# CurryChen77/RIFT

Hardware: AMD Instinct MI355X
Metric: policy-update scenes/sec (256-scene RIFT update steps on a 4096-scene replay) (higher is better)
Workload: dtype bf16; 1 GPU; BASELINE configs[2]/[3]: full rift_pluto CBV policy, 4096-scene synthetic replay (64 agents x 21 steps, 20 polygons x 3 x 20 pts, R~U{1..6} x 120 ref pts, 12 modes), RIFT loss, pi_head trainable; per_gpu_batch=256, global_batch=256, replay_scenes_per_gpu=4096, parallelism=dp1, train_mode=dropout+droppath+state-dropout, BN batch stats

## Files before the change

### include/rift_hip.h

```cpp
#ifndef RIFT_HIP_H
#define RIFT_HIP_H

#include <stdint.h>

#ifdef __cplusplus
extern "C" {
#endif

typedef struct RiftCtx RiftCtx;

enum { RIFT_OK = 0, RIFT_ERR_ARG = -1, RIFT_ERR_HIP = -2, RIFT_ERR_STATE = -3, RIFT_ERR_NONFINITE = -4 };

enum {
  RIFT_F_TRAIN      = 1,
  RIFT_F_NEED_TRAJ  = 2,
  RIFT_F_FP32       = 4,
  RIFT_F_NO_DROP    = 8,
  RIFT_F_NO_BN_UPDATE = 16,
  RIFT_F_DEFER_HEAD = 32
};
#define RIFT_DEFER_SLOTS 4

enum { RIFT_LOSS_RIFT = 0, RIFT_LOSS_GRPO = 1, RIFT_LOSS_PPO = 2, RIFT_LOSS_REINFORCE = 3,
       RIFT_LOSS_SFT = 4  };
// ... 8 lines not shown

typedef struct RiftFeatureBatch {
  int32_t bs, A, Mp, R, S;
  int32_t T;
  const float*   agent_position;
  const float*   agent_heading;
  const float*   agent_velocity;
  const float*   agent_shape;
  const int8_t*  agent_category;
  const uint8_t* agent_valid_mask;
  const float*   map_point_position;
  const float*   map_point_vector;
  const float*   map_point_orientation;
  const float*   map_polygon_center;
  const int8_t*  map_polygon_type;
  const uint8_t* map_polygon_on_route;
  const int8_t*  map_polygon_tl_status;
  const uint8_t* map_polygon_has_speed_limit;
  const float*   map_polygon_speed_limit;
  const uint8_t* map_valid_mask;
  const float*   ref_position;
  const float*   ref_vector;
  const float*   ref_orientation;
  const uint8_t* ref_valid_mask;
  const float*   static_position;
  const float*   static_heading;
  const float*   static_shape;
  const int8_t*  static_category;
  const uint8_t* static_valid_mask;
  const float*   current_state;
  int32_t cs_ld;
} RiftFeatureBatch;

typedef struct RiftOutputs {
  float* probability;
  float* hidden;
  float* trajectory;
  float* prediction;
  float* ref_free_trajectory;
} RiftOutputs;

typedef struct RiftLossIn {
  const float*   old_group_logits;
  const float*   ref_group_logits;
  const double*  group_advantage;
  const uint8_t* group_valid_mask;
  const int64_t* action_mode;
  const float*   advantage;
  const float*   old_log_prob;
  const float*   returns;
  float clip_epsilon;
  float lambda_entropy;
} RiftLossIn;

typedef struct RiftLossOut {
  double* loss;
  double* stats;
  float*  flat_grad_sum;
  float*  grad_w1;  float* grad_b1;
  float*  grad_ln_w; float* grad_ln_b;
  float*  grad_w2;  float* grad_b2;
  int64_t* argmax_rm;
  double* exchange;
} RiftLossOut;

enum { RIFT_OPERANDS_BF16 = 0, RIFT_OPERANDS_FP16 = 1 };
// ... 128 lines not shown
  double  bbox_inflation_ratio;
  double  resolution;
} RiftEvalParams;
int rift_eval_params_default(RiftCtx* ctx, RiftEvalParams* out);

int rift_rollout_return_ex(RiftCtx* ctx, const float* delta_dis, const float* delta_angle, const float* speed,
                           const float* acc, const float* ang_vel, const float* ang_acc, const uint8_t* collision,
                           int collision_ld, const uint8_t* off_road, int off_road_ld, int G, int Ts, const RiftEvalParams* params,
                           double* returns, double* terms, void* stream);

int rift_group_advantage_tick_ex(RiftCtx* ctx, const float* trajectory, int Rb, int Tfull, const RiftTickCBV* cbvs, int K,
                                 float* turn_buf, int32_t* turn_ptr, int32_t* turn_len, float* speed_buf, int32_t* speed_ptr, int32_t* speed_len,
                                 const RiftEvalParams* params, double* advantage, double* returns, double* terms, void* stream);

typedef struct RiftControlCBV {
  int32_t batch_index;
  int32_t slot;
  double x, y, heading;
  double speed;
} RiftControlCBV;
int rift_control_tick(RiftCtx* ctx, const float* trajectory , const float* probability ,
                      const float* ref_free_trajectory , int Rb, int Tfull,
                      const RiftControlCBV* cbvs, int K, int topk, int sample_interval, double* pid_state ,
                      int n_slots, double* decision , void* stream);

typedef struct RiftReplayArena {
  int32_t n_scenes, A, Mp, Rcap, S, T, cs_ld;
  RiftFeatureBatch scenes;
  const int32_t* r_count;
  const float*   old_group_logits;
  const float*   ref_group_logits;
  const double*  group_advantage;
  const uint8_t* group_valid_mask;
} RiftReplayArena;

int rift_collate(RiftCtx* ctx, const RiftReplayArena* arena, const int32_t* scene_idx , int bs,
                 int R_out, const RiftFeatureBatch* out_batch , float* out_old_logits,
                 float* out_ref_logits, double* out_advantage, uint8_t* out_valid_mask, void* stream);

int rift_clip_grad_norm(RiftCtx* ctx, float* const* grads , const int64_t* numels ,
                        int n_tensors , float max_norm, float* total_norm, void* stream);

int rift_adamw_step(RiftCtx* ctx, int n_tensors , float* const* params, const float* const* grads, float* const* exp_avg,
                    float* const* exp_avg_sq, float* const* steps, const int64_t* numels , const double* lr ,
                    const double* weight_decay , double step_new, double beta1, double beta2, double eps, void* stream);

int rift_update_tail(RiftCtx* ctx, const RiftLossOut* out, int accumulate, float max_norm, float* total_norm, int n_tensors ,
                     float* const* params, const float* const* grads, float* const* exp_avg, float* const* exp_avg_sq, float* const* steps,
                     const double* lr , const double* weight_decay , double step_new, double beta1, double beta2, double eps,
                     void* stream);

typedef struct RiftCritic {
  const float *w0, *b0, *w1, *b1, *w2, *b2;
  const float *state_avg, *state_std, *value_avg, *value_std;
} RiftCritic;
#define RIFT_CRITIC_NPARAM_C 99331

int rift_critic_forward(RiftCtx* ctx, const RiftCritic* w, const float* state , int n, float* value , void* stream);

int rift_critic_loss_backward(RiftCtx* ctx, const RiftCritic* w, const float* state , const float* reward_sum ,
                              int n, double* stats , float* flat_grad_sum, void* stream);

int rift_critic_finalize(RiftCtx* ctx, const float* flat_grad_sum, const double* stats, float* g_w0, float* g_b0, float* g_w1,
                         float* g_b1, float* g_w2, float* g_b2, float* g_state_avg, float* g_state_std, float* g_value_avg,
                         float* g_value_std, void* stream);

int rift_critic_backward(RiftCtx* ctx, const RiftCritic* w, const float* state , const float* dvalue , int n,
// ... 7 lines not shown
```

### rift_amd/_ffi.py

```python
import ctypes as C
import threading
import os
from typing import Dict, Optional

import numpy as np
import torch

_HERE = os.path.dirname(os.path.abspath(__file__))
LIB_PATH = os.path.join(_HERE, "librift_hip.so")

F_TRAIN, F_NEED_TRAJ, F_FP32, F_NO_DROP, F_NO_BN_UPDATE, F_DEFER_HEAD = 1, 2, 4, 8, 16, 32
DEFER_SLOTS = 4
LOSS_KINDS = {"rift": 0, "grpo": 1, "ppo": 2, "reinforce": 3, "sft": 4}
PI_NPARAM = 16897

vp = C.c_void_p


class RiftTensorDesc(C.Structure):
    _fields_ = [("name", C.c_char_p), ("data", vp), ("numel", C.c_int64), ("ndim", C.c_int32),
                ("shape", C.c_int64 * 4)]


_FB_PTRS = [
    "agent_position", "agent_heading", "agent_velocity", "agent_shape", "agent_category", "agent_valid_mask",
    "map_point_position", "map_point_vector", "map_point_orientation", "map_polygon_center", "map_polygon_type",
    "map_polygon_on_route", "map_polygon_tl_status", "map_polygon_has_speed_limit", "map_polygon_speed_limit",
    "map_valid_mask", "ref_position", "ref_vector", "ref_orientation", "ref_valid_mask", "static_position",
    "static_heading", "static_shape", "static_category", "static_valid_mask", "current_state",
]


class RiftFeatureBatch(C.Structure):
    _fields_ = ([(n, C.c_int32) for n in ("bs", "A", "Mp", "R", "S", "T")] + [(n, vp) for n in _FB_PTRS]
                + [("cs_ld", C.c_int32)])


class RiftOutputs(C.Structure):
    _fields_ = [(n, vp) for n in ("probability", "hidden", "trajectory", "prediction", "ref_free_trajectory")]


class RiftLossIn(C.Structure):
    _fields_ = [(n, vp) for n in ("old_group_logits", "ref_group_logits", "group_advantage", "group_valid_mask",
                                  "action_mode", "advantage", "old_log_prob", "returns")] + \
               [("clip_epsilon", C.c_float), ("lambda_entropy", C.c_float)]


class RiftLossOut(C.Structure):
    _fields_ = [(n, vp) for n in ("loss", "stats", "flat_grad_sum", "grad_w1", "grad_b1", "grad_ln_w", "grad_ln_b",
                                  "grad_w2", "grad_b2", "argmax_rm", "exchange")]


class RiftCritic(C.Structure):
    _fields_ = [(n, vp) for n in ("w0", "b0", "w1", "b1", "w2", "b2", "state_avg", "state_std", "value_avg", "value_std")]


class RiftReplayArena(C.Structure):
    _fields_ = [(n, C.c_int32) for n in ("n_scenes", "A", "Mp", "Rcap", "S", "T", "cs_ld")] + \
               [("scenes", RiftFeatureBatch)] + \
               [(n, vp) for n in ("r_count", "old_group_logits", "ref_group_logits", "group_advantage",
                                  "group_valid_mask")]


EXCHANGE_FN = C.CFUNCTYPE(C.c_int, C.c_void_p, C.c_int64, C.c_int64, C.c_void_p)


class RiftDp(C.Structure):
    _fields_ = [("scene_offset", C.c_int32), ("global_bs", C.c_int32), ("xchg", vp), ("xchg_len", C.c_int64),
                ("exchange", EXCHANGE_FN), ("user", vp)]


class RiftRolloutIO(C.Structure):
    _fields_ = [("trajectories", vp), ("G", C.c_int32), ("Tfull", C.c_int32), ("G_per_group", C.c_int32), ("center_state", vp),
                ("turn_buf", vp), ("turn_ptr", vp), ("turn_len", vp), ("speed_buf", vp), ("speed_ptr", vp), ("speed_len", vp),
                ("center", vp), ("angle", vp), ("speed", vp), ("acc", vp), ("ang_vel", vp), ("ang_acc", vp), ("vertices", vp),
                ("closest_index", vp), ("aim_idx", vp)]


class RiftTickCBV(C.Structure):
    _fields_ = [("batch_index", C.c_int32), ("R", C.c_int32), ("Pmax", C.c_int32), ("n_actors", C.c_int32), ("center_state", vp),
                ("ref_pos", vp), ("ref_angle", vp), ("ref_len", vp), ("actors", vp), ("off_road_mask", vp), ("H", C.c_int32), ("W", C.c_int32),
                ("pose", C.c_double * 3)]


class RiftControlCBV(C.Structure):
    _fields_ = [("batch_index", C.c_int32), ("slot", C.c_int32), ("x", C.c_double), ("y", C.c_double), ("heading", C.c_double),
                ("speed", C.c_double)]


class RiftEvalParams(C.Structure):
    _fields_ = [("reward_model", C.c_int32), ("near_lane_change", C.c_int32), ("gamma", C.c_double)] + \
               [(n, C.c_double) for n in ("alpha_collision", "alpha_boundary", "alpha_comfort", "alpha_l_align", "alpha_vel_align", "alpha_l_center",
                                          "alpha_center_bias", "alpha_velocity", "alpha_timestep", "bbox_inflation_ratio", "resolution")]


REWARD_MODELS = {"dense": 0, "sparse": 1}


def eval_params(reward_model=None, gamma: float = 0.98, bbox_inflation_ratio: float = 1.1, resolution: float = 0.5,
                near_lane_change: bool = True) -> RiftEvalParams:
    from rift_amd.gym_carla.reward.reward_model import DenseRewardModel
    p = RiftEvalParams()
    weights = DenseRewardModel().get_params()
    kind = "dense"
    if reward_model is not None:
        kind = reward_model.kind
        unknown = sorted(set(reward_model.get_params()) - set(weights))
        if kind not in REWARD_MODELS or unknown:
            raise ValueError(f"reward model {kind!r} with parameter(s) {unknown}: known models {sorted(REWARD_MODELS)}, known parameters {sorted(weights)}")
        weights.update(reward_model.get_params())
    p.reward_model, p.near_lane_change, p.gamma = REWARD_MODELS[kind], 1 if near_lane_change else 0, float(gamma)
    for k, v in weights.items():
        setattr(p, k, float(v))
    p.bbox_inflation_ratio, p.resolution = float(bbox_inflation_ratio), float(resolution)
    return p


CONTROL_STATE = 44
OPERANDS = {"bf16": 0, "fp16": 1}
EXPORTS = [
    "rift_ctx_create", "rift_ctx_create_ex", "rift_ctx_operand_format", "rift_ctx_destroy", "rift_last_error", "rift_model_load", "rift_forward", "rift_forward_head", "rift_forward_head_back", "rift_loss_backward",
    "rift_loss_finalize", "rift_loss_finalize_clip", "rift_set_param_event", "rift_tap", "rift_op_linear", "rift_gae", "rift_discounted_return",
    "rift_normalize_advantage", "rift_group_advantage", "rift_rollout_return", "rift_collate",
    "rift_prof_enable", "rift_prof_report", "rift_op_linear_bench", "rift_ref_line_info", "rift_rollout",
    "rift_critic_forward", "rift_critic_loss_backward", "rift_critic_finalize", "rift_clip_grad_norm", "rift_adamw_step", "rift_update_tail", "rift_collision_matrix", "rift_off_road_matrix", "rift_other_vehicle_rollout", "rift_sft_teacher_mode",
    "rift_check_finite", "rift_set_dp", "rift_set_prepare_stream", "rift_set_side_stream",
    "rift_comm_unique_id", "rift_comm_init", "rift_comm_all_reduce", "rift_comm_destroy", "rift_group_advantage_tick",
    "rift_control_tick", "rift_head_backward", "rift_critic_backward",
    "rift_eval_params_default", "rift_rollout_return_ex", "rift_group_advantage_tick_ex",
]
CRITIC_NPARAM = 99331
PI_KEYS = ("mlp.0.weight", "mlp.0.bias", "mlp.1.weight", "mlp.1.bias", "mlp.3.weight", "mlp.3.bias")
PI_SIZES = (128 * 128, 128, 128, 128, 128, 1)
CRITIC_SIZES = (256 * 128, 256, 256 * 256, 256, 256, 1, 128, 128, 1, 1)
CRITIC_KEYS = ("net.0.weight", "net.0.bias", "net.2.weight", "net.2.bias", "net.4.weight", "net.4.bias",
               "state_avg", "state_std", "value_avg", "value_std")

_libs = {}


def load_library(variant: str = "") -> C.CDLL:
    if variant in _libs:
        return _libs[variant]
    path = LIB_PATH if not variant else LIB_PATH.replace("librift_hip.so", f"librift_hip_{variant}.so")
    if not variant and os.environ.get("RIFT_LIB"):
        path = os.environ["RIFT_LIB"]
    if not os.path.exists(path):
        raise RuntimeError(
            f"{path} is missing: build it with `python -c 'import __graft_entry__ as g; g.build()'` "
            "(hipcc --offload-arch=gfx950). rift_amd has no CPU fallback.")
    lib = C.CDLL(path)
    for name in EXPORTS:
        if not hasattr(lib, name):
            raise RuntimeError(f"librift_hip.so does not export {name}")
    lib.rift_ctx_create.argtypes = [C.c_int, C.POINTER(vp)]
    lib.rift_ctx_create_ex.argtypes = [C.c_int, C.c_int, C.POINTER(vp)]
# ... 17 lines not shown
    lib.rift_set_side_stream.argtypes = [vp, vp]
    lib.rift_comm_unique_id.argtypes = [vp, vp]
    lib.rift_comm_init.argtypes = [vp, vp, C.c_int, C.c_int]
    lib.rift_comm_all_reduce.argtypes = [vp, vp, C.c_int64, vp]
    lib.rift_group_advantage_tick.argtypes = [vp, vp, C.c_int, C.c_int, C.POINTER(RiftTickCBV), C.c_int, vp, vp, vp, vp, vp, vp, C.c_double, vp, vp]
    lib.rift_group_advantage_tick_ex.argtypes = [vp, vp, C.c_int, C.c_int, C.POINTER(RiftTickCBV), C.c_int, vp, vp, vp, vp, vp, vp, C.POINTER(RiftEvalParams),
                                                 vp, vp, vp, vp]
    lib.rift_eval_params_default.argtypes = [vp, C.POINTER(RiftEvalParams)]
    lib.rift_rollout_return_ex.argtypes = [vp, vp, vp, vp, vp, vp, vp, vp, C.c_int, vp, C.c_int, C.c_int, C.c_int, C.POINTER(RiftEvalParams), vp, vp, vp]
    lib.rift_control_tick.argtypes = [vp, vp, vp, vp, C.c_int, C.c_int, C.POINTER(RiftControlCBV), C.c_int, C.c_int, C.c_int, vp, C.c_int, vp, vp]
    lib.rift_comm_destroy.argtypes = [vp]
    lib.rift_loss_finalize_clip.argtypes = [vp, C.POINTER(RiftLossOut), C.c_int, C.c_float, vp, vp]
    lib.rift_tap.argtypes = [vp, C.c_char_p, vp, C.POINTER(C.c_int64), vp]
    lib.rift_critic_forward.argtypes = [vp, C.POINTER(RiftCritic), vp, C.c_int, vp, vp]
    lib.rift_critic_loss_backward.argtypes = [vp, C.POINTER(RiftCritic), vp, vp, C.c_int, vp, vp, vp]
    lib.rift_critic_finalize.argtypes = [vp] * 14
    lib.rift_clip_grad_norm.argtypes = [vp, C.POINTER(vp), C.POINTER(C.c_int64), C.c_int, C.c_float, vp, vp]
    lib.rift_update_tail.argtypes = [vp, C.POINTER(RiftLossOut), C.c_int, C.c_float, vp, C.c_int, C.POINTER(vp), C.POINTER(vp), C.POINTER(vp), C.POINTER(vp),
                                     C.POINTER(vp), C.POINTER(C.c_double), C.POINTER(C.c_double), C.c_double, C.c_double, C.c_double, C.c_double, vp]
    lib.rift_adamw_step.argtypes = [vp, C.c_int, C.POINTER(vp), C.POINTER(vp), C.POINTER(vp), C.POINTER(vp), C.POINTER(vp),
                                    C.POINTER(C.c_int64), C.POINTER(C.c_double), C.POINTER(C.c_double), C.c_double, C.c_double,
                                    C.c_double, C.c_double, vp]
    lib.rift_sft_teacher_mode.argtypes = [vp, vp, vp, C.c_int, C.c_int, C.c_int, C.c_int, C.c_int, vp, vp]
    lib.rift_other_vehicle_rollout.argtypes = [vp, vp, vp, vp, vp, vp, C.c_int, C.c_int, C.c_int, C.c_double, vp, vp]
    lib.rift_collision_matrix.argtypes = [vp, vp, C.c_int, C.c_int, vp, C.c_int, C.c_int, vp, vp]
    lib.rift_off_road_matrix.argtypes = [vp, vp, C.c_int, vp, C.c_int, C.c_int] + [C.c_double] * 7 + [vp, vp]
    lib.rift_op_linear.argtypes = [vp, vp, C.c_int, C.c_int, vp, vp, C.c_int, vp, vp, C.c_int, C.c_int, vp, vp]
    lib.rift_gae.argtypes = [vp, vp, vp, vp, vp, vp, C.c_float, C.c_float, C.c_int, vp, vp]
    lib.rift_discounted_return.argtypes = [vp, vp, vp, C.c_double, C.c_int, vp, vp]
    lib.rift_normalize_advantage.argtypes = [vp, vp, C.c_int, vp]
    lib.rift_group_advantage.argtypes = [vp, vp, C.c_int, C.c_int, vp, vp]
    lib.rift_rollout_return.argtypes = [vp, vp, vp, vp, vp, vp, vp, vp, C.c_int, vp, C.c_int, C.c_int, C.c_int,
                                        C.c_double, vp, vp]
    lib.rift_collate.argtypes = [vp, C.POINTER(RiftReplayArena), vp, C.c_int, C.c_int, C.POINTER(RiftFeatureBatch),
                                 vp, vp, vp, vp, vp]
    lib.rift_op_linear_bench.argtypes = [vp, vp, C.c_int, C.c_int, vp, vp, C.c_int, vp, vp, C.c_int, vp, vp, C.c_int,
                                         C.POINTER(C.c_float), vp]
    lib.rift_ref_line_info.argtypes = [vp, vp, C.c_int, C.c_int, C.c_int, C.c_int, vp, vp, vp, C.c_int, vp, vp, vp, vp]
    lib.rift_rollout.argtypes = [vp, C.POINTER(RiftRolloutIO), vp]
    lib.rift_prof_enable.argtypes = [vp, C.c_int]
    lib.rift_prof_report.argtypes = [vp, C.c_char_p, C.c_int]
    for name in EXPORTS:
        if name not in ("rift_ctx_destroy", "rift_last_error"):
            getattr(lib, name).restype = C.c_int
    _libs[variant] = lib
    return lib


def _ptr(t: Optional[torch.Tensor]):
    return None if t is None else C.c_void_p(t.data_ptr())


class _KnownStreams(threading.local):
    def __init__(self):
        self.stack = []


_KNOWN_STREAM = _KnownStreams()


def _stream():
    st = _KNOWN_STREAM.stack
    if st:
        return st[-1]
    return C.c_void_p(torch.cuda.current_stream().cuda_stream)

# ... 36 lines not shown

    fb = RiftFeatureBatch()
    pos = put(ag["position"], f32)
    bs, A, T = pos.shape[:3]
    Mp = mp["point_position"].shape[1]
    R = rl["position"].shape[1]
    S = so["position"].shape[1] if so is not None else 0
    fb.bs, fb.A, fb.Mp, fb.R, fb.S, fb.T = bs, A, Mp, R, S, T
    t = {
        "agent_position": pos, "agent_heading": put(ag["heading"], f32), "agent_velocity": put(ag["velocity"], f32),
        "agent_shape": put(ag["shape"], f32), "agent_category": put(ag["category"], i8),
        "agent_valid_mask": put(ag["valid_mask"], u8),
        "map_point_position": put(mp["point_position"], f32), "map_point_vector": put(mp["point_vector"], f32),
        "map_point_orientation": put(mp["point_orientation"], f32), "map_polygon_center": put(mp["polygon_center"], f32),
        "map_polygon_type": put(mp["polygon_type"], i8), "map_polygon_on_route": put(mp["polygon_on_route"], u8),
        "map_polygon_tl_status": put(mp["polygon_tl_status"], i8),
        "map_polygon_has_speed_limit": put(mp["polygon_has_speed_limit"], u8),
        "map_polygon_speed_limit": put(mp["polygon_speed_limit"], f32), "map_valid_mask": put(mp["valid_mask"], u8),
        "ref_position": put(rl["position"], f32), "ref_vector": put(rl["vector"], f32),
        "ref_orientation": put(rl["orientation"], f32), "ref_valid_mask": put(rl["valid_mask"], u8),
        "current_state": put(data["current_state"], f32),
    }
    if S > 0:
        t.update({"static_position": put(so["position"], f32), "static_heading": put(so["heading"], f32),
                  "static_shape": put(so["shape"], f32), "static_category": put(so["category"], i8),
                  "static_valid_mask": put(so["valid_mask"], u8)})
    for name in _FB_PTRS:
        setattr(fb, name, t[name].data_ptr() if name in t else None)
    fb.cs_ld = t["current_state"].shape[1]
    return fb, keep


class Engine:

    def __init__(self, device=None, operands: str = "bf16", variant: str = ""):
        if operands not in OPERANDS:
            raise ValueError(f"operands must be one of {sorted(OPERANDS)}, got {operands!r}")
        if not torch.cuda.is_available():
            raise RuntimeError("rift_amd.Engine needs a HIP device (torch.cuda.is_available() is False); "
                               "there is no CPU fallback")
        self.lib = load_library(variant)
        self.device = torch.device(device if device is not None else f"cuda:{torch.cuda.current_device()}")
        self.ctx = vp()
        self.operands = operands
        rc = self.lib.rift_ctx_create_ex(self.device.index or 0, OPERANDS[operands], C.byref(self.ctx))
        if rc != 0:
            raise RuntimeError(f"rift_ctx_create_ex failed ({rc})")
        self._params = None
        self._names = None
        self._keep = []
        self._stage_host = self._stage_dev = None
        self._stage_off = 0
        self._ctl_state = None
        self.generation = 0

    _STAGE_BYTES = 8 << 20
    _NP_OF = {torch.float32: np.float32, torch.float64: np.float64, torch.int32: np.int32, torch.int64: np.int64, torch.uint8: np.uint8,
              torch.int8: np.int8, torch.bool: np.bool_}

    def stage_tree(self, data):
        leaves = []

        def walk(d):
            if isinstance(d, dict):
                return {k: walk(v) for k, v in d.items()}
            if torch.is_tensor(d):
                leaves.append(d)
                return len(leaves) - 1
            raise NotImplementedError(type(d))

        shape = walk(data)
        out = self.stage_many(leaves)

        def build(d):
            return {k: build(v) for k, v in d.items()} if isinstance(d, dict) else out[d]
        return build(shape)

    def stage_many(self, tensors):
        if self._stage_host is None:
            self._stage_host = torch.empty(self._STAGE_BYTES, dtype=torch.uint8).pin_memory()
            self._stage_dev = torch.empty(self._STAGE_BYTES, dtype=torch.uint8, device=self.device)
        plan, total = [], 0
        for t in tensors:
            if t.is_cuda or t.dtype not in self._NP_OF or t.numel() == 0 or t.numel() * t.element_size() > self._STAGE_BYTES // 4:
                plan.append(None)
                continue
            a = np.ascontiguousarray(t.detach().numpy())
# ... 77 lines not shown
            descs[i].data = v.data_ptr()
            descs[i].numel = v.numel()
            descs[i].ndim = min(v.dim(), 4)
            shp = list(v.shape)[-4:] if v.dim() > 4 else list(v.shape)
            for d in range(4):
                descs[i].shape[d] = shp[d] if d < len(shp) else 1
        self._params, self._names = params, names
        self._check(self.lib.rift_model_load(self.ctx, descs, len(params), _stream()), "rift_model_load")
        return params

    def forward(self, data: Dict, train=False, need_traj=False, fp32=False, no_drop=False, bn_update=True,
                seed: int = 0) -> Dict[str, torch.Tensor]:
        fb, keep = feature_batch(data, self.device)
        bs, A, R = fb.bs, fb.A, fb.R
        o = RiftOutputs()
        out = {"probability": torch.empty(bs, R, 12, device=self.device),
               "hidden": torch.empty(bs, 128, device=self.device)}
        if need_traj:
            out["trajectory"] = torch.empty(bs, R, 12, 80, 6, device=self.device)
            out["prediction"] = torch.empty(bs, max(A - 1, 0), 80, 6, device=self.device)
            out["ref_free_trajectory"] = torch.empty(bs, 80, 4, device=self.device)
        for k, v in out.items():
            setattr(o, k, v.data_ptr())
        flags = (F_TRAIN if train else 0) | (F_NEED_TRAJ if need_traj else 0) | (F_FP32 if fp32 else 0) | \
                (F_NO_DROP if no_drop else 0) | (0 if bn_update else F_NO_BN_UPDATE)
        self._check(self.lib.rift_forward(self.ctx, C.byref(fb), C.byref(o), flags, C.c_uint32(seed & 0xFFFFFFFF),
                                          _stream()), "rift_forward")
        self.generation += 1
        self._keep = keep + list(out.values())
        self._bs = bs
        return out

    def forward_raw(self, fb: RiftFeatureBatch, out: RiftOutputs, flags: int, seed: int):
        rc = self.lib.rift_forward(self.ctx, C.byref(fb), C.byref(out), flags, C.c_uint32(seed & 0xFFFFFFFF), _stream())
        self.generation += 1
        if rc != 0:
            self._check(rc, "rift_forward")
        self._bs = fb.bs

    def set_side_stream(self, stream: Optional["torch.cuda.Stream"]):
        self._side_stream = stream
        rc = self.lib.rift_set_side_stream(self.ctx, C.c_void_p(stream.cuda_stream if stream is not None else 0))
        if rc != 0:
            self._check(rc, "rift_set_side_stream")

    def set_prepare_stream(self, stream: Optional["torch.cuda.Stream"]):
        self._prep_stream = stream
        rc = self.lib.rift_set_prepare_stream(self.ctx, C.c_void_p(stream.cuda_stream if stream is not None else 0))
        if rc != 0:
            self._check(rc, "rift_set_prepare_stream")

    def forward_head(self, back: int = 0):
        rc = self.lib.rift_forward_head_back(self.ctx, back, _stream())
        self.generation += 1
        if rc != 0:
            self._check(rc, "rift_forward_head")

    def loss_backward_raw(self, kind: int, li: RiftLossIn, lo: RiftLossOut):
        rc = self.lib.rift_loss_backward(self.ctx, kind, C.byref(li), C.byref(lo), _stream())
        if rc != 0:
            self._check(rc, "rift_loss_backward")

    def loss_finalize_raw(self, lo: RiftLossOut, accumulate: int = 0):
        rc = self.lib.rift_loss_finalize(self.ctx, C.byref(lo), accumulate, _stream())
        if rc != 0:
            self._check(rc, "rift_loss_finalize")

# ... 538 lines not shown
```

### rift_amd/csrc/abi.cpp

```cpp
#include <stdlib.h>
#include <string.h>

#include "abi_table.h"

extern "C" const RiftVTable rift_vtable_bf16;
#if defined(RIFT_ABI_BF16_ONLY)
#define RIFT_VT_FP16 (static_cast<const RiftVTable*>(nullptr))
#else
extern "C" const RiftVTable rift_vtable_fp16;
#define RIFT_VT_FP16 (&rift_vtable_fp16)
#endif

static inline const RiftVTable& vt(const RiftCtx* ctx) {
  return (*reinterpret_cast<const int*>(ctx) == RIFT_OPERANDS_FP16 && RIFT_VT_FP16) ? *RIFT_VT_FP16 : rift_vtable_bf16;
}

extern "C" {

int rift_ctx_create_ex(int device, int operand_format, RiftCtx** ctx) {
  if (operand_format == RIFT_OPERANDS_BF16) return rift_vtable_bf16.rift_ctx_create(device, ctx);
  if (operand_format == RIFT_OPERANDS_FP16 && RIFT_VT_FP16) return RIFT_VT_FP16->rift_ctx_create(device, ctx);
  return RIFT_ERR_ARG;
}

// ... 168 lines not shown
  return vt(ctx).rift_ref_line_info(ctx, trajectories, G, Tfull, Ts, M, ref_pos, ref_angle, ref_len, Pmax, delta_dis, delta_angle, closest_idx, stream);
}

int rift_rollout(RiftCtx* ctx, const RiftRolloutIO* io, void* stream) {
  if (!ctx) return RIFT_ERR_ARG;
  return vt(ctx).rift_rollout(ctx, io, stream);
}

int rift_group_advantage_tick(RiftCtx* ctx, const float* trajectory, int Rb, int Tfull, const RiftTickCBV* cbvs, int K, float* turn_buf, int32_t* turn_ptr, int32_t* turn_len, float* speed_buf, int32_t* speed_ptr, int32_t* speed_len, double gamma, double* advantage, void* stream) {
  if (!ctx) return RIFT_ERR_ARG;
  return vt(ctx).rift_group_advantage_tick(ctx, trajectory, Rb, Tfull, cbvs, K, turn_buf, turn_ptr, turn_len, speed_buf, speed_ptr, speed_len, gamma, advantage, stream);
}

int rift_eval_params_default(RiftCtx* ctx, RiftEvalParams* out) {
  if (!ctx) return RIFT_ERR_ARG;
  return vt(ctx).rift_eval_params_default(ctx, out);
}

int rift_rollout_return_ex(RiftCtx* ctx, const float* delta_dis, const float* delta_angle, const float* speed, const float* acc, const float* ang_vel, const float* ang_acc, const uint8_t* collision, int collision_ld, const uint8_t* off_road, int off_road_ld, int G, int Ts, const RiftEvalParams* params, double* returns, double* terms, void* stream) {
  if (!ctx) return RIFT_ERR_ARG;
  return vt(ctx).rift_rollout_return_ex(ctx, delta_dis, delta_angle, speed, acc, ang_vel, ang_acc, collision, collision_ld, off_road, off_road_ld, G, Ts, params, returns, terms, stream);
}

int rift_group_advantage_tick_ex(RiftCtx* ctx, const float* trajectory, int Rb, int Tfull, const RiftTickCBV* cbvs, int K, float* turn_buf, int32_t* turn_ptr, int32_t* turn_len, float* speed_buf, int32_t* speed_ptr, int32_t* speed_len, const RiftEvalParams* params, double* advantage, double* returns, double* terms, void* stream) {
  if (!ctx) return RIFT_ERR_ARG;
  return vt(ctx).rift_group_advantage_tick_ex(ctx, trajectory, Rb, Tfull, cbvs, K, turn_buf, turn_ptr, turn_len, speed_buf, speed_ptr, speed_len, params, advantage, returns, terms, stream);
}

int rift_control_tick(RiftCtx* ctx, const float* trajectory, const float* probability, const float* ref_free_trajectory, int Rb, int Tfull, const RiftControlCBV* cbvs, int K, int topk, int sample_interval, double* pid_state, int n_slots, double* decision, void* stream) {
  if (!ctx) return RIFT_ERR_ARG;
  return vt(ctx).rift_control_tick(ctx, trajectory, probability, ref_free_trajectory, Rb, Tfull, cbvs, K, topk, sample_interval, pid_state, n_slots, decision, stream);
}

int rift_collate(RiftCtx* ctx, const RiftReplayArena* arena, const int32_t* scene_idx, int bs, int R_out, const RiftFeatureBatch* out_batch, float* out_old_logits, float* out_ref_logits, double* out_advantage, uint8_t* out_valid_mask, void* stream) {
  if (!ctx) return RIFT_ERR_ARG;
  return vt(ctx).rift_collate(ctx, arena, scene_idx, bs, R_out, out_batch, out_old_logits, out_ref_logits, out_advantage, out_valid_mask, stream);
}

int rift_clip_grad_norm(RiftCtx* ctx, float* const* grads, const int64_t* numels, int n_tensors, float max_norm, float* total_norm, void* stream) {
  if (!ctx) return RIFT_ERR_ARG;
  return vt(ctx).rift_clip_grad_norm(ctx, grads, numels, n_tensors, max_norm, total_norm, stream);
}

int rift_adamw_step(RiftCtx* ctx, int n_tensors, float* const* params, const float* const* grads, float* const* exp_avg, float* const* exp_avg_sq, float* const* steps, const int64_t* numels, const double* lr, const double* weight_decay, double step_new, double beta1, double beta2, double eps, void* stream) {
  if (!ctx) return RIFT_ERR_ARG;
  return vt(ctx).rift_adamw_step(ctx, n_tensors, params, grads, exp_avg, exp_avg_sq, steps, numels, lr, weight_decay, step_new, beta1, beta2, eps, stream);
}

int rift_update_tail(RiftCtx* ctx, const RiftLossOut* out, int accumulate, float max_norm, float* total_norm, int n_tensors, float* const* params, const float* const* grads, float* const* exp_avg, float* const* exp_avg_sq, float* const* steps, const double* lr, const double* weight_decay, double step_new, double beta1, double beta2, double eps, void* stream) {
  if (!ctx) return RIFT_ERR_ARG;
  return vt(ctx).rift_update_tail(ctx, out, accumulate, max_norm, total_norm, n_tensors, params, grads, exp_avg, exp_avg_sq, steps, lr, weight_decay, step_new, beta1, beta2, eps, stream);
}

int rift_critic_forward(RiftCtx* ctx, const RiftCritic* w, const float* state, int n, float* value, void* stream) {
  if (!ctx) return RIFT_ERR_ARG;
  return vt(ctx).rift_critic_forward(ctx, w, state, n, value, stream);
}

int rift_critic_loss_backward(RiftCtx* ctx, const RiftCritic* w, const float* state, const float* reward_sum, int n, double* stats, float* flat_grad_sum, void* stream) {
  if (!ctx) return RIFT_ERR_ARG;
  return vt(ctx).rift_critic_loss_backward(ctx, w, state, reward_sum, n, stats, flat_grad_sum, stream);
}

int rift_critic_finalize(RiftCtx* ctx, const float* flat_grad_sum, const double* stats, float* g_w0, float* g_b0, float* g_w1, float* g_b1, float* g_w2, float* g_b2, float* g_state_avg, float* g_state_std, float* g_value_avg, float* g_value_std, void* stream) {
  if (!ctx) return RIFT_ERR_ARG;
  return vt(ctx).rift_critic_finalize(ctx, flat_grad_sum, stats, g_w0, g_b0, g_w1, g_b1, g_w2, g_b2, g_state_avg, g_state_std, g_value_avg, g_value_std, stream);
// ... 9 lines not shown
```

### rift_amd/csrc/abi_list.h

```cpp
RIFT_FN(rift_ctx_create)
RIFT_FN(rift_ctx_destroy)
RIFT_FN(rift_last_error)
RIFT_FN(rift_model_load)
RIFT_FN(rift_forward)
RIFT_FN(rift_forward_head)
RIFT_FN(rift_forward_head_back)
RIFT_FN(rift_set_dp)
RIFT_FN(rift_comm_unique_id)
RIFT_FN(rift_comm_init)
RIFT_FN(rift_comm_all_reduce)
RIFT_FN(rift_comm_destroy)
RIFT_FN(rift_set_prepare_stream)
RIFT_FN(rift_set_side_stream)
RIFT_FN(rift_check_finite)
RIFT_FN(rift_sft_teacher_mode)
RIFT_FN(rift_set_param_event)
RIFT_FN(rift_loss_backward)
RIFT_FN(rift_loss_finalize)
RIFT_FN(rift_loss_finalize_clip)
RIFT_FN(rift_head_backward)
RIFT_FN(rift_prof_enable)
RIFT_FN(rift_prof_report)
RIFT_FN(rift_tap)
RIFT_FN(rift_op_linear)
RIFT_FN(rift_op_linear_bench)
RIFT_FN(rift_gae)
RIFT_FN(rift_discounted_return)
RIFT_FN(rift_normalize_advantage)
RIFT_FN(rift_group_advantage)
RIFT_FN(rift_other_vehicle_rollout)
RIFT_FN(rift_collision_matrix)
RIFT_FN(rift_off_road_matrix)
RIFT_FN(rift_rollout_return)
RIFT_FN(rift_ref_line_info)
RIFT_FN(rift_rollout)
RIFT_FN(rift_group_advantage_tick)
RIFT_FN(rift_eval_params_default)
RIFT_FN(rift_rollout_return_ex)
RIFT_FN(rift_group_advantage_tick_ex)
RIFT_FN(rift_control_tick)
RIFT_FN(rift_collate)
RIFT_FN(rift_clip_grad_norm)
RIFT_FN(rift_adamw_step)
RIFT_FN(rift_update_tail)
RIFT_FN(rift_critic_forward)
RIFT_FN(rift_critic_loss_backward)
RIFT_FN(rift_critic_finalize)
RIFT_FN(rift_critic_backward)
```

### rift_amd/csrc/adv.h

```cpp
#pragma once
#include "common.h"

namespace RIFT_NS {

struct GaeCoef {
  const double* rewards; const float* undones; const float* values; const float* next_values; const float* unterminated;
  float gamma, lambda_;
  __device__ __forceinline__ void get(int t, double& a, double& b) const {
    const float t2 = (unterminated[t] * gamma) * next_values[t];
    b = rewards[t] + (double)t2 - (double)values[t];
    a = (double)((undones[t] * gamma) * lambda_);
  }
};
struct ReturnCoef {
  const double* rewards; const float* dones; double gamma;
  __device__ __forceinline__ void get(int t, double& a, double& b) const {
    b = rewards[t];
    a = (dones[t] == 1.0f) ? 0.0 : gamma;
  }
};

#define RIFT_SCAN_THREADS 1024
template <class Coef, class OutT>
__global__ __launch_bounds__(RIFT_SCAN_THREADS) void affine_scan_reverse_kernel(Coef c, int n, OutT* __restrict__ out) {
// ... 218 lines not shown
    if (!(ox0 > ex1 || ox1 < ex0 || oy0 > ey1 || oy1 < ey0)) { hit = 1; break; }
  }
  out[i] = hit;
}
__global__ __launch_bounds__(256) void collision_matrix_kernel(const float* __restrict__ cv, int G, int Tc, const double* __restrict__ ov, int N, int Ts, uint8_t* __restrict__ out) {
  collision_matrix_body(cv, G, Tc, ov, N, Ts, out);
}

__device__ __forceinline__ void off_road_body(const float* __restrict__ pts , int n, const uint8_t* __restrict__ mask, int H,
                                                       int W, double ox, double oy, double c, double s, double res_x, double res_y,
                                                       double off_x, double off_y, uint8_t* __restrict__ out) {
  const int i = blockIdx.x * 256 + threadIdx.x;
  if (i >= n) return;
  const double dx = (double)pts[2 * i] - ox, dy = (double)pts[2 * i + 1] - oy;
  const double lx = __dadd_rn(__dmul_rn(dx, c), __dmul_rn(dy, s));
  const double ly = __dadd_rn(__dmul_rn(dx, -s), __dmul_rn(dy, c));
  const double px = rint(lx / res_x + off_x), py = rint(ly / res_y + off_y);
  uint8_t off = 0;
  if (px >= 0.0 && px < (double)W && py >= 0.0 && py < (double)H) off = mask[(size_t)(int)py * W + (int)px] == 1;
  out[i] = off;
}
__global__ __launch_bounds__(256) void off_road_kernel(const float* __restrict__ pts, int n, const uint8_t* __restrict__ mask, int H, int W, double ox, double oy, double c, double s,
                                                       double res_x, double res_y, double off_x, double off_y, uint8_t* __restrict__ out) {
  off_road_body(pts, n, mask, H, W, ox, oy, c, s, res_x, res_y, off_x, off_y, out);
}

#define RIFT_COLLATE_MAXT 40
struct CollateP {
  int nt;
  const unsigned char* src[RIFT_COLLATE_MAXT];
  unsigned char* dst[RIFT_COLLATE_MAXT];
  int src_bytes[RIFT_COLLATE_MAXT];
  int dst_bytes[RIFT_COLLATE_MAXT];
};

__global__ void collate_kernel(CollateP p, const int32_t* __restrict__ scene_idx) {
  const int k = blockIdx.y, b = blockIdx.x;
  const unsigned char* s = p.src[k] + (size_t)scene_idx[b] * p.src_bytes[k];
  unsigned char* d = p.dst[k] + (size_t)b * p.dst_bytes[k];
  const int n = p.dst_bytes[k];
  if ((((uintptr_t)s | (uintptr_t)d | (uintptr_t)n) & 15) == 0) {
    const uint4* s4 = reinterpret_cast<const uint4*>(s);
    uint4* d4 = reinterpret_cast<uint4*>(d);
    for (int i = threadIdx.x; i < (n >> 4); i += blockDim.x) d4[i] = s4[i];
  } else if ((((uintptr_t)s | (uintptr_t)d | (uintptr_t)n) & 3) == 0) {
    const uint32_t* s4 = reinterpret_cast<const uint32_t*>(s);
    uint32_t* d4 = reinterpret_cast<uint32_t*>(d);
    for (int i = threadIdx.x; i < (n >> 2); i += blockDim.x) d4[i] = s4[i];
  } else {
    for (int i = threadIdx.x; i < n; i += blockDim.x) d[i] = s[i];
  }
}

}
```

### rift_amd/csrc/engine.hip

```cpp
#include <hip/hip_runtime.h>
#include <math.h>
#include <stdio.h>
#include <stdlib.h>
#include <string.h>

#include <algorithm>
#include <set>
#include <cmath>
#include <string>
#include <unordered_map>
#include <dlfcn.h>
#include <vector>

#include "../../include/rift_hip.h"
#include "adv.h"
#include "eval_params.h"
#include "gemm.h"
#include "kernels.h"
#include "loss.h"
#include "nat_l0w.h"
#include "nat_l1w.h"
#include "enc_fused.h"
#include "dec_w.h"
#include "dec_kv.h"
// ... 11 lines not shown
#include "pi_fused.h"
#include "rollout.h"
#include "tick_multi.h"
#include "control.h"

#define ENC_NW 8

using namespace RIFT_NS;

namespace {

struct Param { void* data; int64_t numel; int ndim; int64_t shape[4]; };

struct PW {
  void* bf = nullptr; float* f32 = nullptr; const float* bias = nullptr;
  int N = 0, K = 0, Kp = 0, Npad = 0;
  void* hid = nullptr;
};

struct Tap { float* p; int64_t numel; };

}

struct RiftCtx {
  int opfmt = 0;
  int device = 0;
  std::string err;
  std::unordered_map<std::string, Param> params;
  std::unordered_map<std::string, PW> pw;
  std::vector<void*> owned;
  struct WConst { float* p = nullptr; bool ready = false; };
  std::unordered_map<std::string, WConst> wconst;
  char* arena = nullptr; size_t arena_cap = 0, arena_off = 0;
  long long dry_key[11] = {}; size_t dry_need = 0;
  char* arenas[RIFT_DEFER_SLOTS] = {}; size_t arena_caps[RIFT_DEFER_SLOTS] = {}; int parity = 0;
  struct Head {
    bool valid = false, fp32 = false, need_traj = false;
    float *Q = nullptr, *x0p = nullptr, *QF = nullptr, *Hpi = nullptr, *prob = nullptr, *traj = nullptr, *o3[3] = {nullptr, nullptr, nullptr}, *oT[3] = {nullptr, nullptr, nullptr};
    uint8_t* r_kpm = nullptr; int bs = 0, R = 0, nQ = 0;
    bool dec_pending = false; DecWP dec;
  } head[RIFT_DEFER_SLOTS];
  int dec_defer_max = -1; bool dec_split = true;
  bool ro8 = true;
  float* ro_raw = nullptr; size_t ro_cap = 0;
  char* tick_scratch = nullptr; size_t tick_cap = 0;
  bool dry = false;
  hipStream_t stream = nullptr;
  std::unordered_map<std::string, Tap> taps;
  float* last_qfinal = nullptr; float* last_hpi = nullptr; float* last_prob = nullptr;
  uint8_t* last_rkpm = nullptr; int last_bs = 0, last_R = 0;
  double* l_S = nullptr; double* l_cnt = nullptr; float* l_dz = nullptr; float* l_partial = nullptr;
  size_t l_cap_bs = 0, l_cap_rows = 0, l_cap_wg = 0;
  double* l_sink = nullptr;
  float* ego_w = nullptr; float* ego_b = nullptr;
  bool nat_fused = true; int gemm_dbg = 0;
  unsigned short* l0w_img = nullptr; float* l0w_par = nullptr;
  unsigned short* encw_img = nullptr; float* encw_par = nullptr;
  unsigned short* l2w_img = nullptr; float* l2w_par = nullptr;
  unsigned short* l1w_img = nullptr; float* l1w_par = nullptr;
  unsigned short* enc_wqkv[4] = {nullptr, nullptr, nullptr, nullptr};
  float* enc_bqkv[4] = {nullptr, nullptr, nullptr, nullptr};
  int* enc_idx = nullptr; bool enc_fused = true;
  int poison_lds = -1;
  struct { std::string delay_label; long long delay_ticks = 0; int pe_ts = -1, pew_dbg = 0, pew_ts = 0, nat_ts = 0, enc_ts = 0, dec_ts = 0, dec_dbg = 0, poison_arena = -1; } dg;
  hipEvent_t param_event = nullptr;
  bool dec_fused = true;
  bool two_streams = true; bool nat_compact = true; bool pe_live = true; bool pe_pack = true;
  hipStream_t prep_stream = nullptr; bool prep_set = false; hipEvent_t ev_prep = nullptr; int side_gate = 0;
  hipEvent_t ev_join2 = nullptr; bool nat_aside = true;
  hipStream_t side = nullptr; bool side_owned = false; hipEvent_t ev_fork = nullptr, ev_join = nullptr;
  bool fo_w = true; unsigned short* fow_img[3] = {nullptr, nullptr, nullptr}; float* fow_par[3] = {nullptr, nullptr, nullptr};
  bool pe_w = true; unsigned short* pew_img[2] = {nullptr, nullptr};
  unsigned short* decw_img = nullptr; float* decw_par = nullptr;
  double* clip_part = nullptr;
  struct Dp { bool on = false; int off = 0, gbs = 0; double* xchg = nullptr; long long len = 0; RiftExchangeFn fn = nullptr; void* user = nullptr; } dp;
  int* nonfinite = nullptr;
  unsigned long long* rk_pub[RIFT_DEFER_SLOTS] = {}; int rk_cap[RIFT_DEFER_SLOTS] = {}; unsigned int rk_epoch[RIFT_DEFER_SLOTS] = {};
  bool rank_fault = false;
  bool no_skip = false;
  bool enc112 = true;
  bool rank_in_prep = true;
  void* comm = nullptr; int comm_rank = 0, comm_world = 1;
  float* cr_buf = nullptr; size_t cr_cap = 0; double* cr_part = nullptr;
  bool pe_fused = true; bool fo_fused = true; int nat_grid = 256; bool fpn_fused = true; bool ego_fused = true; bool heads_fused = true; bool pi_fused = true;
  bool loaded = false;
  bool prof_on = false; double prof_flops = 0.0; bool prof_shapes = false;
  std::set<std::string> prof_names;
  std::vector<hipEvent_t> prof_pool; size_t prof_used = 0;
  struct Rec { const char* label; hipEvent_t e0, e1; double flops; };
  std::vector<Rec> prof_recs;
};

static void prof_events(RiftCtx* c, hipEvent_t* e0, hipEvent_t* e1) {
  while (c->prof_pool.size() < c->prof_used + 2) { hipEvent_t e; (void)hipEventCreate(&e); c->prof_pool.push_back(e); }
  *e0 = c->prof_pool[c->prof_used++]; *e1 = c->prof_pool[c->prof_used++];
}
static void prof_push(RiftCtx* c, const char* label, hipEvent_t e0, hipEvent_t e1, double flops) {
  c->prof_recs.push_back(RiftCtx::Rec{label, e0, e1, flops});
}

// ... 280 lines not shown
#undef SETATTR
#define SETATTR_N(K, N) HIPCHK(c, hipFuncSetAttribute(reinterpret_cast<const void*>(&K), hipFuncAttributeMaxDynamicSharedMemorySize, (int)(N)))
  SETATTR_N(lds_poison_kernel, 160 * 1024);
  SETATTR_N(dec_kv_frag_kernel, DEC_KV_LDS);
  SETATTR_N(pe_mid_kernel, PE_MID_LDS);
  SETATTR_N(pe_out_kernel, PE_OUT_LDS);
  SETATTR_N(fourier_fused_kernel, FO_LDS);
  SETATTR_N(fpn_tail_kernel, FPN_LDS);
  SETATTR_N(heads3_fused_kernel, HD_LDS);
  SETATTR_N(pi_forward_kernel, PI_LDS);
  HIPCHK(c, (hipError_t)l0w_set_attributes());
  HIPCHK(c, (hipError_t)l1w_set_attributes());
#undef SETATTR_N
  return RIFT_OK;
}

const std::string HE = "agent_encoder.history_encoder", PD = "planning_decoder";

struct Fwd {
  RiftCtx* c; bool train, drop, fp32, need_traj, bn_update; uint32_t seed; uint32_t stream_id = 1;
  uint32_t next_stream() { return stream_id++; }
  bool dp = false, kpm_pending = false; int kb = 0; uint8_t* g_rkpm = nullptr;
  uint8_t* r_tiles = nullptr;
  const RiftFeatureBatch* B = nullptr; const RiftOutputs* out = nullptr; int flags = 0;
  StreamPlan plan; hipStream_t on[3] = {nullptr, nullptr, nullptr};
  int bs = 0, A = 0, Mp = 0, R = 0, S = 0, T = 0, N = 0, M = 12, nA = 0, nP = 0, nL = 0, nQ = 0, nT = 0;
  DropStats ds = {};
  float *F9 = nullptr, *F10 = nullptr, *F6 = nullptr, *pos = nullptr, *r_pos = nullptr;
  uint8_t *valid_agent = nullptr, *kpm = nullptr, *r_kpm = nullptr;
  bool nat_compact = false; int *nat_aidx = nullptr, *nat_cnt = nullptr;
  const uint8_t* q_kpm = nullptr; int q_bs = 0, q_off = 0;
  float *nat_out = nullptr, *x_ego = nullptr, *poly = nullptr, *r_emb = nullptr, *speed_emb = nullptr, *PEtok = nullptr, *Q = nullptr, *X = nullptr;
  bool pe_pair = false, fo3 = false, rpe_done = false;
  float* ENC = nullptr;
  unsigned short* enc_KT = nullptr;
  uint8_t* kpm_c = nullptr;
  float* enc_x0p = nullptr;
  bool enc_wide = false;
  bool dec_deferred = false; DecWP dec_later;
};

struct RcclApi {
  struct UniqueId { char internal[128]; };
  int (*GetUniqueId)(UniqueId*) = nullptr;
  int (*CommInitRank)(void**, int, UniqueId, int) = nullptr;
  int (*AllReduce)(const void*, void*, size_t, int, int, void*, hipStream_t) = nullptr;
  int (*CommDestroy)(void*) = nullptr;
  const char* (*GetErrorString)(int) = nullptr;
  bool ok = false;
};
static RcclApi& rccl_api(std::string* why) {
  static RcclApi api;
  static bool tried = false;
  static std::string err;
  if (!tried) {
    tried = true;
    void* h = nullptr;
    const char* names[] = {getenv("RIFT_RCCL_LIB"), "librccl.so", "librccl.so.1"};
    for (const char* n : names) if (n && !h) h = dlopen(n, RTLD_NOW | RTLD_NOLOAD | RTLD_GLOBAL);
    for (const char* n : names) if (n && !h) h = dlopen(n, RTLD_NOW | RTLD_GLOBAL);
    if (!h) h = dlopen("/opt/rocm/lib/librccl.so", RTLD_NOW | RTLD_GLOBAL);
    if (!h) err = std::string("librccl.so not found (set RIFT_RCCL_LIB): ") + (dlerror() ? dlerror() : "");
    else {
      api.GetUniqueId = (decltype(api.GetUniqueId))dlsym(h, "ncclGetUniqueId");
      api.CommInitRank = (decltype(api.CommInitRank))dlsym(h, "ncclCommInitRank");
      api.AllReduce = (decltype(api.AllReduce))dlsym(h, "ncclAllReduce");
// ... 87 lines not shown

void batchnorm_affine(Fwd& f, const float* X, int rows, int C, const uint8_t* valid, const std::string& name,
                      float** scale, float** shift) {
  RiftCtx* c = f.c;
  *scale = A_alloc<float>(c, C); *shift = A_alloc<float>(c, C);
  const int rows_per_blk = 128;
  const int nblk = cdiv(rows, rows_per_blk);
  double* part = A_alloc<double>(c, (size_t)nblk * 2 * C);
  int* cnt = A_alloc<int>(c, nblk);
  if (f.train) launch(c, "bn_partial_kernel", bn_partial_kernel, dim3(nblk), dim3(C), 0, X, C, rows, C, valid, part, cnt, rows_per_blk);
  const Param* nb = find(c, name + ".num_batches_tracked");
  const bool dpx = f.dp && f.train;
  double* sums = dpx ? c->dp.xchg + f.kb : nullptr;
  for (int mode = dpx ? 1 : 0; mode <= (dpx ? 2 : 0); ++mode) {
    launch(c, "bn_finalize_kernel", bn_finalize_kernel, dim3(cdiv(C, 4)), dim3(256), 0, (const double*)part, (const int*)cnt, nblk, C,
           fptr(c, name + ".weight"), fptr(c, name + ".bias"), (float*)fptr(c, name + ".running_mean"),
           (float*)fptr(c, name + ".running_var"), nb ? (long long*)nb->data : (long long*)nullptr, f.train ? 1 : 0,
           f.bn_update ? 1 : 0, 1e-5f, *scale, *shift, sums, mode);
    if (mode == 1) dp_exchange(f, 2 * C + 1);
  }
}

static void pe_fill(Fwd& f, PeP& q, const float* F, int Cin, int groups, int n, const uint8_t* valid, const std::string& p) {
  RiftCtx* c = f.c;
  memset(&q, 0, sizeof(q));
  const int rows = groups * n;
  q.F = F; q.Cin = Cin; q.valid = valid; q.rows = rows; q.ntiles = cdiv(rows, 120);
  const PW &w1 = c->pw[p + ".first_mlp.0"], &w2 = c->pw[p + ".first_mlp.3"], &w3a = c->pw[p + ".second_mlp.0.feat"],
           &w3b = c->pw[p + ".second_mlp.0.pool"], &w4 = c->pw[p + ".second_mlp.3"];
  q.w1 = (const unsigned short*)w1.bf; q.w2 = (const unsigned short*)w2.bf; q.w3a = (const unsigned short*)w3a.bf;
  q.w3b = (const unsigned short*)w3b.bf; q.w4 = (const unsigned short*)w4.bf;
  q.b1 = w1.bias; q.b2 = w2.bias; q.b3 = w3a.bias; q.b4 = w4.bias;
  q.s1 = A_alloc<float>(c, 128); q.t1 = A_alloc<float>(c, 128); q.s2 = A_alloc<float>(c, 256); q.t2 = A_alloc<float>(c, 256);
  q.part1 = A_alloc<float>(c, (size_t)2 * 128 * q.ntiles);
  q.part2 = A_alloc<float>(c, (size_t)2 * 256 * q.ntiles);
  q.cnt = A_alloc<int>(c, q.ntiles);
  q.Fmid = A_alloc<unsigned short>(c, (size_t)rows * 256);
  q.gp = A_alloc<float>(c, (size_t)groups * 256);
  q.out = A_alloc<float>(c, (size_t)groups * 128);
  q.do_stats = f.train ? 1 : 0;
  { if (c->dg.pe_ts == n) { q.ts = A_alloc<long long>(c, 64); q.ts_tile = 0; tap(c, "pe_ts", (float*)q.ts, 128); } }
}

static BnFinP bn_fin(RiftCtx* c, const PeP& q, const std::string& name, int C, const float* part, const float* sc, const float* sh,
                     double* sums = nullptr, int sums_mode = 0) {
  BnFinP b; memset(&b, 0, sizeof(b));
  b.sums = sums; b.sums_mode = sums_mode;
  const Param* nb = find(c, name + ".num_batches_tracked");
  b.part = part; b.cnt = q.cnt; b.nblk = q.ntiles; b.C = C; b.gamma = fptr(c, name + ".weight"); b.beta = fptr(c, name + ".bias");
  b.running_mean = (float*)fptr(c, name + ".running_mean"); b.running_var = (float*)fptr(c, name + ".running_var");
  b.num_batches = nb ? (long long*)nb->data : nullptr; b.scale = (float*)sc; b.shift = (float*)sh;
  return b;
}

void points_encoder_pair(Fwd& f, const float* Fm, int gm, const uint8_t* vm, const std::string& pm, const float* Fr, int gr,
                         const uint8_t* vr, const std::string& pr, float** out_m, float** out_r) {
  RiftCtx* c = f.c;
  PeP2 q;
  pe_fill(f, q.a, Fm, 10, gm, 20, vm, pm);
  pe_fill(f, q.b, Fr, 6, gr, 120, vr, pr);
  const int nt = q.a.ntiles + q.b.ntiles;
  const double rows = (double)q.a.rows + q.b.rows, groups = (double)gm + gr;
  const bool stats_p = f.train && c->pe_w;
  const bool packb = c->pe_w && c->pe_pack && gr > 0 && f.r_tiles != nullptr;
  int* pk_tab = nullptr; int* pk_hdr = nullptr;
  PePackP pk; memset(&pk, 0, sizeof(pk));
  if (packb) {
    const int maxr = cdiv(q.b.rows, PEW_ROUND_ROWS);
    pk_tab = A_alloc<int>(c, (size_t)std::max(maxr, 1) * PEW_TAB_INTS); pk_hdr = A_alloc<int>(c, 4);
    pk.tiles = f.r_tiles; pk.nlines = gr; pk.tab = pk_tab; pk.hdr = pk_hdr; pk.max_rounds = maxr;
    tap(c, "pe_pack_hdr", (float*)pk_hdr, 4); tap(c, "pe_pack_tab", (float*)pk_tab, (int64_t)std::max(maxr, 1) * PEW_TAB_INTS);
    if (!stats_p) { c->prof_flops = 0.0; launch(c, "pe_pack_lines_kernel", pe_pack_lines_kernel, dim3(1), dim3(256), (size_t)gr * 2 * sizeof(int), pk); }
  }
  if (stats_p) {
    int g = std::min(nt, 4 * c->nat_grid);
    int ga = (int)(((long long)g * q.a.ntiles + nt / 2) / nt);
    if (q.a.ntiles > 0 && ga < 1) ga = 1;
    if (q.b.ntiles > 0 && ga > g - 1) ga = g - 1;
    if (q.b.ntiles == 0) ga = g;
    ga = std::min(ga, q.a.ntiles);
    q.a.nwg1 = ga; q.b.nwg1 = std::min(g - ga, q.b.ntiles);
    PeP* sd[2] = {&q.a, &q.b};
    for (int i = 0; i < 2; ++i) { sd[i]->part1w = A_alloc<float>(c, (size_t)2 * 128 * std::max(sd[i]->nwg1, 1)); sd[i]->cnt1w = A_alloc<int>(c, std::max(sd[i]->nwg1, 1)); }
    c->prof_flops = 2.0 * 128.0 * (q.a.rows * 10.0 + q.b.rows * 6.0);
    launch(c, "pe_stats1_kernel", pe_stats1p_kernel, dim3(q.a.nwg1 + q.b.nwg1 + (packb ? 1 : 0)), dim3(256), packb ? (size_t)gr * 2 * sizeof(int) : 0, q, pk);
  } else if (f.train) {
    c->prof_flops = 2.0 * 128.0 * (q.a.rows * 10.0 + q.b.rows * 6.0);
    launch(c, "pe_stats1_kernel", pe_stats1_kernel, dim3(nt), dim3(256), 0, q);
  }
  const bool dpx = f.dp && f.train;
  double* xs = dpx ? c->dp.xchg + f.kb : nullptr;
  PeLiveP lv; memset(&lv, 0, sizeof(lv));
  const bool live = stats_p && c->pe_live;
  int pew_grid = c->nat_grid, pew_ga = 0;
  if (c->pe_w) pew_split(cdiv(q.a.rows, PEW_ROUND_ROWS), cdiv(q.b.rows, PEW_ROUND_ROWS), &pew_grid, &pew_ga);
  if (live || packb) {
    const PeP* sd[2] = {&q.a, &q.b};
    for (int i = 0; i < 2; ++i) {
      lv.cnt[i] = live ? sd[i]->cnt : nullptr; lv.nt[i] = sd[i]->ntiles; lv.nr[i] = cdiv(sd[i]->rows, PEW_ROUND_ROWS);
      lv.live[i] = A_alloc<int>(c, std::max(lv.nr[i], 1));
    }
    lv.grid = pew_grid; lv.hdr = A_alloc<int>(c, 4);
    lv.packed_b = pk_hdr;
    tap(c, "pe_live_hdr", (float*)lv.hdr, 4);
  }
  const bool lvblock = live || packb;
  for (int mode = dpx ? 1 : 0; mode <= (dpx ? 2 : 0); ++mode) {
    BnFinP f1a = bn_fin(c, q.a, pm + ".first_mlp.1", 128, q.a.part1, q.a.s1, q.a.t1, xs, mode);
    BnFinP f1b = bn_fin(c, q.b, pr + ".first_mlp.1", 128, q.b.part1, q.b.s1, q.b.t1, xs ? xs + 257 : nullptr, mode);
    if (stats_p) { f1a.part = q.a.part1w; f1a.cnt = q.a.cnt1w; f1a.nblk = q.a.nwg1; f1b.part = q.b.part1w; f1b.cnt = q.b.cnt1w; f1b.nblk = q.b.nwg1; }
    const bool with_lv = lvblock && mode == (dpx ? 2 : 0);
    PeLiveP none; memset(&none, 0, sizeof(none));
    launch(c, "bn_finalize_t_kernel", bn_finalize_t_kernel, dim3(256 + (with_lv ? 1 : 0)), dim3(256), 0, f1a, f1b, f.train ? 1 : 0, f.bn_update ? 1 : 0, 1e-5f,
           with_lv ? lv : none);
    if (mode == 1) dp_exchange(f, 2 * 257);
  }
  c->prof_flops = 2.0 * rows * (128.0 * 8 + 128.0 * 256 + (f.train ? 256.0 * 256 : 0.0)) + 2.0 * groups * 256.0 * 256;
  BnFinP fa, fb;
  if (c->pe_w) {
    PeWP w; memset(&w, 0, sizeof(w));
    const PeP* src[2] = {&q.a, &q.b};
    PeWSide* dst[2] = {&w.a, &w.b};
    const int npts[2] = {20, 120};
    const int grid = pew_grid, ga = pew_ga;
    const int nwg[2] = {lvblock ? grid : ga, lvblock ? grid : grid - ga};
    for (int i = 0; i < 2; ++i) {
      const PeP& o = *src[i]; PeWSide& d = *dst[i];
      d.F = o.F; d.Cin = o.Cin; d.valid = o.valid; d.rows = o.rows; d.npts = npts[i]; d.nrounds = cdiv(o.rows, PEW_ROUND_ROWS);
      d.img = c->pew_img[i]; d.w3b = o.w3b; d.b1 = o.b1; d.b2 = o.b2; d.b3 = o.b3; d.s1 = o.s1; d.t1 = o.t1;
      d.live = (live && !(i == 1 && packb)) ? lv.live[i] : nullptr;
      if (i == 1) { d.ptab = pk_tab; d.phdr = pk_hdr; }
      d.part2 = A_alloc<float>(c, (size_t)2 * 256 * std::max(nwg[i], 1)); d.cnt2 = A_alloc<int>(c, std::max(nwg[i], 1));
      d.Fmid = o.Fmid;
    }
    w.ga = ga; w.hdr = lvblock ? lv.hdr : nullptr;
    w.do_stats = f.train ? 1 : 0;
    w.dbg = c->dg.pew_dbg;
    { if (c->dg.pew_ts) { w.ts = A_alloc<long long>(c, 128); tap(c, "pew_ts", (float*)w.ts, 256); } }
    launch_call(c, "pe_w_kernel", [&] { pew_launch(w, grid, c->stream); });
    fa = bn_fin(c, q.a, pm + ".second_mlp.1", 256, w.a.part2, q.a.s2, q.a.t2, xs, 0); fa.cnt = w.a.cnt2; fa.nblk = nwg[0]; fa.nblk_dev = lvblock ? lv.hdr + 2 : nullptr;
    fb = bn_fin(c, q.b, pr + ".second_mlp.1", 256, w.b.part2, q.b.s2, q.b.t2, xs ? xs + 513 : nullptr, 0); fb.cnt = w.b.cnt2; fb.nblk = nwg[1]; fb.nblk_dev = lvblock ? lv.hdr + 3 : nullptr;
  } else {
    launch(c, "pe_mid_kernel", pe_mid_kernel, dim3(nt), dim3(512), (size_t)PE_MID_LDS, q);
    fa = bn_fin(c, q.a, pm + ".second_mlp.1", 256, q.a.part2, q.a.s2, q.a.t2, xs, 0);
    fb = bn_fin(c, q.b, pr + ".second_mlp.1", 256, q.b.part2, q.b.s2, q.b.t2, xs ? xs + 513 : nullptr, 0);
  }
  for (int mode = dpx ? 1 : 0; mode <= (dpx ? 2 : 0); ++mode) {
    fa.sums_mode = mode; fb.sums_mode = mode;
    PeLiveP none; memset(&none, 0, sizeof(none));
// ... 391 lines not shown
         (const float*)c->ego_w, (const float*)c->ego_b, fptr(c, EG + ".pos_embed"), bs, E);
  float* EKV = A_alloc<float>(c, (size_t)bs * 6 * 256);
  gemm(c, mk(E, 128, bs * 6, c->pw[EG + ".attn.kv"], EKV, 256), c->pw[EG + ".attn.kv"], f.fp32);
  uint8_t* edrop = nullptr;
  if (f.drop) {
    edrop = A_alloc<uint8_t>(c, (size_t)bs * 6);
    launch(c, "ego_dropmask_kernel", ego_dropmask_kernel, dim3(cdiv(bs * 6, 256)), dim3(256), 0, bs, 0.75f, f.seed, f.next_stream(), edrop);
  }
  float* EAO = A_alloc<float>(c, (size_t)bs * 128);
  {
    MhaP p; memset(&p, 0, sizeof(p));
    p.Q = eq; p.ldq = 128; p.K = EKV; p.V = EKV + 128; p.ldkv = 256; p.O = EAO; p.ldo = 128;
    p.nb_outer = bs; p.nb_inner = 1; p.H = 4; p.Lq = 1; p.Lk = 6;
    p.q_outer = 0; p.q_inner = 0; p.q_stride = 0; p.kv_outer = 6; p.kv_inner = 0; p.kv_stride = 1;
    p.o_outer = 1; p.o_inner = 0; p.o_stride = 0; p.mask = edrop; p.mask_quirk = 0; p.mask_mod = 1;
    run_mha(c, p, f.fp32);
  }
  gemm(c, mk(EAO, 128, bs, c->pw[EG + ".attn.out_proj"], f.x_ego, 128), c->pw[EG + ".attn.out_proj"], f.fp32);
  }
  tap(c, "x_ego", f.x_ego, (int64_t)bs * 128);
}

int build_q0(Fwd& f) {
  RiftCtx* c = f.c;
  const int M = f.M, nL = f.nL, nQ = f.nQ;
  bool fill;
  float* Mb = wconst_get(c, "Mb", (size_t)M * 128, f.fp32, &fill);
  if (fill) gemm(c, mk(fptr(c, PD + ".m_emb"), 128, M, c->pw[PD + ".q_proj.m"], Mb, 128), c->pw[PD + ".q_proj.m"], f.fp32);
  f.Q = A_alloc<float>(c, (size_t)nQ * 128);
  if (!f.fp32 && c->pi_fused) {
    Q0P q; memset(&q, 0, sizeof(q));
    q.r_emb = f.r_emb; q.nL = nL; q.M = M; q.wr = (const unsigned short*)c->pw[PD + ".q_proj.r"].bf; q.br = c->pw[PD + ".q_proj.r"].bias;
    q.Mb = Mb; q.Q = f.Q;
    c->prof_flops = 2.0 * nL * 128.0 * 128;
    launch(c, "q0_fused_kernel", q0_fused_kernel, dim3(cdiv(nL, 16)), dim3(256), 0, q);
  } else {
    float* Ra = A_alloc<float>(c, (size_t)nL * 128);
    gemm(c, mk(f.r_emb, 128, nL, c->pw[PD + ".q_proj.r"], Ra, 128), c->pw[PD + ".q_proj.r"], f.fp32);
    launch(c, "build_q0_kernel", build_q0_kernel, dim3(cdiv((long long)nQ * 128, 256)), dim3(256), 0, (const float*)Ra, (const float*)Mb, nL, M, f.Q);
  }
  return RIFT_OK;
}

int map_and_embeddings(Fwd& f) {
  RiftCtx* c = f.c;
  const RiftFeatureBatch* B = f.B;
  const int S = f.S, nP = f.nP, nL = f.nL, nT = f.nT;
  f.pe_pair = !f.fp32 && c->pe_fused;
  if (f.pe_pair) points_encoder_pair(f, f.F10, nP, B->map_valid_mask, "map_encoder.polygon_encoder", f.F6, nL, B->ref_valid_mask, PD + ".r_encoder", &f.poly, &f.r_emb);
  else f.poly = points_encoder(f, f.F10, 10, nP, 20, B->map_valid_mask, "map_encoder.polygon_encoder");
  tap(c, "poly_pe", f.poly, (int64_t)nP * 128);
  f.fo3 = f.pe_pair && !f.fp32 && c->fo_fused && S == 0;
  if (f.fo3) {
    tap(c, "r_pe", f.r_emb, (int64_t)nL * 128);
    FourierP3 q3; memset(&q3, 0, sizeof(q3));
    q3.e[0] = fourier_desc(f, f.pos, 3, nT, 3, "pos_emb", 2, nullptr);
    q3.e[1] = fourier_desc(f, B->map_polygon_speed_limit, 1, nP, 1, "map_encoder.speed_limit_emb", -1, nullptr);
    q3.e[2] = fourier_desc(f, f.r_pos, 3, nL, 3, PD + ".r_pos_emb", -1, f.r_emb);
    q3.nblk[0] = cdiv(nT, FO_ROWS); q3.nblk[1] = cdiv(nP, FO_ROWS); q3.nblk[2] = cdiv(nL, FO_ROWS); q3.count = 3;
    c->prof_flops = 2.0 * 128.0 * ((nT + nL) * (3 * 257.0 + 128.0) + nP * (257.0 + 128.0));
    if (c->fo_w) {
      FoWP w; memset(&w, 0, sizeof(w));
      w.count = 3;
      for (int i = 0; i < 3; ++i) {
        const FourierP& o = q3.e[i]; FoWSide& d = w.e[i];
        d.in = o.in; d.in_ld = o.in_ld; d.rows = o.rows; d.D = o.D; d.wrap_dim = o.wrap_dim; d.img = c->fow_img[i]; d.par = c->fow_par[i];
        d.Y = o.Y; d.accumulate = o.accumulate; d.rep = o.D == 1 ? 2 : 1; d.nwg = cdiv(cdiv(o.rows, 16), 8 * d.rep);
      }
      launch_call(c, "fo_w_kernel", [&] { fow_launch(w, c->stream); });
    } else
    launch(c, "fourier_fused_kernel", fourier_fused_kernel, dim3(q3.nblk[0] + q3.nblk[1] + q3.nblk[2]), dim3(256), (size_t)FO_LDS, q3);
    f.PEtok = q3.e[0].Y; f.speed_emb = q3.e[1].Y; f.rpe_done = true;
  } else {
    f.speed_emb = fourier(f, B->map_polygon_speed_limit, 1, nP, 1, "map_encoder.speed_limit_emb", -1);
  }
  if (f.plan.forked && f.rpe_done) TRY(build_q0(f));
  return RIFT_OK;
}

void assemble_tokens(Fwd& f) {
  RiftCtx* c = f.c;
  const RiftFeatureBatch* B = f.B;
  const int bs = f.bs, A = f.A, Mp = f.Mp, S = f.S, N = f.N, nA = f.nA, nP = f.nP, nT = f.nT;
  f.X = A_alloc<float>(c, (size_t)nT * 128);
  TokenP q; memset(&q, 0, sizeof(q));
  q.nat = f.nat_out; q.x_ego = f.x_ego; q.valid_agent = (const uint8_t*)f.valid_agent; q.category = B->agent_category; q.a_type_emb = fptr(c, "agent_encoder.type_emb.weight");
  q.pooled = f.poly; q.ptype = B->map_polygon_type; q.on_route = B->map_polygon_on_route; q.tl = B->map_polygon_tl_status; q.has_sl = B->map_polygon_has_speed_limit;
  q.speed_emb = f.speed_emb; q.p_type_emb = fptr(c, "map_encoder.type_emb.weight"); q.route_emb = fptr(c, "map_encoder.on_route_emb.weight");
  q.tl_emb = fptr(c, "map_encoder.traffic_light_emb.weight"); q.unk_emb = fptr(c, "map_encoder.unknown_speed_emb.weight");
  q.bs = bs; q.A = A; q.Mp = Mp; q.N = N; q.X = f.X; q.pe = f.PEtok;
  q.nblk_a = cdiv((long long)nA * 32, 256);
  launch(c, "token_kernel", token_kernel, dim3(q.nblk_a + cdiv((long long)nP * 32, 256)), dim3(256), 0, q);
  if (S > 0) {
    float* semb = fourier(f, B->static_shape, 2, bs * S, 2, "static_objects_encoder.obj_encoder", -1);
    launch(c, "static_token_kernel", static_token_kernel, dim3(cdiv((long long)bs * S * 128, 256)), dim3(256), 0, (const float*)semb, B->static_category,
           B->static_valid_mask, fptr(c, "static_objects_encoder.type_emb.weight"), bs, A, Mp, S, N, f.X);
  }
  if (!f.fo3) fourier(f, f.pos, 3, nT, 3, "pos_emb", 2, f.X);
  tap(c, "x_tokens", f.X, (int64_t)nT * 128);
}

void scene_encoder(Fwd& f) {
  RiftCtx* c = f.c;
  const int bs = f.bs, R = f.R, N = f.N, nT = f.nT;
  static const float edpr[4] = {0.f, 0.2f / 3.f, 0.4f / 3.f, 0.2f};
  f.ENC = A_alloc<float>(c, (size_t)nT * 128);
  f.enc_wide = N > 96 && N <= 112 && c->enc112 && c->dec_fused && R <= 8 && ENC_NW == 8;
  if (c->enc_fused && !f.fp32 && (N <= 96 || f.enc_wide)) {
    EncFusedP ep; memset(&ep, 0, sizeof(ep));
    ep.X = f.X; ep.Y = f.ENC; ep.kpm = f.kpm; ep.bs = bs; ep.N = N; ep.seed = f.seed; ep.stream = f.next_stream(); f.stream_id += 8;
    for (int i = 0; i < 4; ++i) {
      const std::string p = "encoder_blocks." + std::to_string(i);
      EncBlockW& w = ep.blk[i];
      w.ln1_g = fptr(c, p + ".norm1.weight"); w.ln1_b = fptr(c, p + ".norm1.bias");
      w.ln2_g = fptr(c, p + ".norm2.weight"); w.ln2_b = fptr(c, p + ".norm2.bias");
      w.wqkv = c->enc_wqkv[i]; w.bqkv = c->enc_bqkv[i];
      w.wo = (const unsigned short*)c->pw[p + ".attn.out_proj"].bf; w.bo = c->pw[p + ".attn.out_proj"].bias;
      w.w1 = (const unsigned short*)c->pw[p + ".mlp.fc1"].bf; w.b1 = c->pw[p + ".mlp.fc1"].bias;
      w.w2 = (const unsigned short*)c->pw[p + ".mlp.fc2"].hid; w.b2 = c->pw[p + ".mlp.fc2"].bias;
      w.droppath = f.drop ? edpr[i] : 0.f;
    }
    ep.norm_g = fptr(c, "norm.weight"); ep.norm_b = fptr(c, "norm.bias"); ep.nonfinite = c->nonfinite;
    ep.ds = f.ds; ep.dbg = c->no_skip ? 1 : 0;
// ... 310 lines not shown

  c->stream = f.on[ON_CALLER];
  assemble_tokens(f);
  scene_encoder(f);
  agent_predictor(f);
  TRY(planning_decoder(f));
  return policy_and_ego_heads(f);
}

}

namespace RIFT_NS { namespace abi {

static bool env_is(const char* name, char ch) { const char* ev = getenv(name); return ev && ev[0] == ch; }
static void env_flag(const char* name, bool* v) { const char* ev = getenv(name); if (ev) *v = atoi(ev) != 0; }
static bool env_int(const char* name, int* v, int base = 10) { const char* ev = getenv(name); if (ev) *v = (int)strtol(ev, nullptr, base); return ev != nullptr; }

static void read_switches(RiftCtx* c) {
  c->nat_fused = !env_is("RIFT_NAT_UNFUSED", '1');
  c->dec_fused = !env_is("RIFT_DEC_UNFUSED", '1');
  c->enc_fused = !env_is("RIFT_ENC_UNFUSED", '1');
  c->pe_fused = !env_is("RIFT_PE_UNFUSED", '1');
  c->fpn_fused = !env_is("RIFT_FPN_UNFUSED", '1');
  c->ego_fused = !env_is("RIFT_EGO_UNFUSED", '1');
  c->heads_fused = !env_is("RIFT_HEADS_UNFUSED", '1');
  c->pi_fused = !env_is("RIFT_PI_UNFUSED", '1');
  c->fo_fused = !env_is("RIFT_FOURIER_UNFUSED", '1');
  c->pe_w = !env_is("RIFT_PE_W", '0');
  c->fo_w = !env_is("RIFT_FO_W", '0');
  c->two_streams = !env_is("RIFT_TWO_STREAMS", '0');
  { int g = 0; env_int("RIFT_NAT_GRID", &g); if (g > 0) c->nat_grid = g; }
  env_flag("RIFT_NAT_COMPACT", &c->nat_compact);
  env_flag("RIFT_PE_LIVE", &c->pe_live);
  env_flag("RIFT_PE_PACK", &c->pe_pack);
  env_flag("RIFT_RANK_IN_PREP", &c->rank_in_prep);
  env_flag("RIFT_NO_SKIP", &c->no_skip);
  env_flag("RIFT_ENC112", &c->enc112);
  env_flag("RIFT_RANK_FAULT", &c->rank_fault);
  env_int("RIFT_SIDE_GATE", &c->side_gate);
  env_flag("RIFT_NAT_ASIDE", &c->nat_aside);
  env_int("RIFT_DEC_DEFER", &c->dec_defer_max);
  env_flag("RIFT_DEC_SPLIT", &c->dec_split);
  env_flag("RIFT_RO8", &c->ro8);
  if (env_int("RIFT_POISON_LDS", &c->poison_lds, 0)) c->poison_lds &= 0xff;
  if (env_int("RIFT_POISON_ARENA", &c->dg.poison_arena, 0)) c->dg.poison_arena &= 0xff;
  { const char* ev = getenv("RIFT_DELAY"); const char* col = ev ? strrchr(ev, ':') : nullptr;
    if (col) { c->dg.delay_label.assign(ev, col - ev); c->dg.delay_ticks = (long long)(atof(col + 1) * 100.0); } }
  env_int("RIFT_PE_TS", &c->dg.pe_ts);
  c->dg.pew_ts = env_is("RIFT_PEW_TS", '1');
  env_int("RIFT_NAT_TS", &c->dg.nat_ts);
  c->dg.enc_ts = getenv("RIFT_ENC_TS") != nullptr;
  c->dg.dec_ts = getenv("RIFT_DEC_TS") != nullptr;
  env_int("RIFT_PEW_DBG", &c->dg.pew_dbg);
  env_int("RIFT_DEC_DBG", &c->dg.dec_dbg);
  env_int("RIFT_GEMM_DBG", &c->gemm_dbg);
}

int rift_ctx_create(int device, RiftCtx** ctx) {
  if (!ctx) return RIFT_ERR_ARG;
  RiftCtx* c = new RiftCtx();
  c->opfmt = RIFT_OP_F16;
  c->device = device;
  if (hipSetDevice(device) != hipSuccess) { delete c; return RIFT_ERR_HIP; }
  read_switches(c);
  if (hipMalloc((void**)&c->nonfinite, sizeof(int)) != hipSuccess || hipMemset(c->nonfinite, 0, sizeof(int)) != hipSuccess) { delete c; return RIFT_ERR_HIP; }
  for (int i = 0; i < RIFT_DEFER_SLOTS; ++i) {
// ... 148 lines not shown
      PeWSrc q; q.Cin = cin[i];
      q.w1 = fptr(c, enc[i] + ".first_mlp.0.weight"); q.w2 = fptr(c, enc[i] + ".first_mlp.3.weight"); q.w3 = fptr(c, enc[i] + ".second_mlp.0.weight");
      if (!c->err.empty()) return RIFT_ERR_ARG;
      if (!c->pew_img[i]) HIPCHK(c, hipMalloc((void**)&c->pew_img[i], (size_t)PEW_FRAGS * 1024));
      pew_pack(q, c->pew_img[i], c->stream);
    }
  }
  {
    DecWSrc q; memset(&q, 0, sizeof(q));
    for (int i = 0; i < 4; ++i) {
      const std::string p = PD + ".decoder_blocks." + std::to_string(i);
      DecWSrc::L& k = q.l[i];
      for (int n = 0; n < 4; ++n) { k.ln[2 * n] = fptr(c, p + ".norm" + std::to_string(n + 1) + ".weight"); k.ln[2 * n + 1] = fptr(c, p + ".norm" + std::to_string(n + 1) + ".bias"); }
      k.r2r_w = fptr(c, p + ".r2r_attn.in_proj_weight"); k.r2r_b = fptr(c, p + ".r2r_attn.in_proj_bias");
      k.r2ro_w = fptr(c, p + ".r2r_attn.out_proj.weight"); k.r2ro_b = fptr(c, p + ".r2r_attn.out_proj.bias");
      k.m2m_w = fptr(c, p + ".m2m_attn.in_proj_weight"); k.m2m_b = fptr(c, p + ".m2m_attn.in_proj_bias");
      k.m2mo_w = fptr(c, p + ".m2m_attn.out_proj.weight"); k.m2mo_b = fptr(c, p + ".m2m_attn.out_proj.bias");
      k.c_w = fptr(c, p + ".cross_attn.in_proj_weight"); k.c_b = fptr(c, p + ".cross_attn.in_proj_bias");
      k.co_w = fptr(c, p + ".cross_attn.out_proj.weight"); k.co_b = fptr(c, p + ".cross_attn.out_proj.bias");
      k.f1_w = fptr(c, p + ".ffn.0.weight"); k.f1_b = fptr(c, p + ".ffn.0.bias"); k.f2_w = fptr(c, p + ".ffn.3.weight"); k.f2_b = fptr(c, p + ".ffn.3.bias");
    }
    q.m_pos = fptr(c, PD + ".m_pos");
    if (!c->err.empty()) return RIFT_ERR_ARG;
    if (!c->decw_img) { HIPCHK(c, hipMalloc((void**)&c->decw_img, (size_t)4 * DECW_LAYER_FRAGS * 1024)); HIPCHK(c, hipMalloc((void**)&c->decw_par, (size_t)4 * DECW_PAR_LAYER * 4)); }
    decw_pack(q, c->decw_img, c->decw_par, c->stream);
  }
  return RIFT_OK;
}

int rift_model_load(RiftCtx* c, const RiftTensorDesc* params, int n, void* stream) {
  if (!c || !params) return RIFT_ERR_ARG;
  c->err.clear();
  c->stream = (hipStream_t)stream;
  HIPCHK(c, hipSetDevice(c->device));
  for (void* p : c->owned) (void)hipFree(p);
  c->owned.clear(); c->pw.clear(); c->params.clear(); c->wconst.clear();
  c->dry_need = 0;
  for (int i = 0; i < n; ++i) {
    Param p; p.data = params[i].data; p.numel = params[i].numel; p.ndim = params[i].ndim;
    for (int d = 0; d < 4; ++d) p.shape[d] = params[i].shape[d];
    c->params[params[i].name] = p;
  }
  TRY(pack_history_encoder(c));
  const std::string EG = "agent_encoder.ego_state_emb";
  TRY(pack_rows(c, EG + ".attn.q", EG + ".attn.in_proj_weight", EG + ".attn.in_proj_bias", 0, 128, 128));
  TRY(pack_rows(c, EG + ".attn.kv", EG + ".attn.in_proj_weight", EG + ".attn.in_proj_bias", 128, 256, 256));
  TRY(pack_linear(c, EG + ".attn.out_proj"));
  if (!c->ego_w) { HIPCHK(c, hipMalloc((void**)&c->ego_w, 6 * 128 * 4)); HIPCHK(c, hipMalloc((void**)&c->ego_b, 6 * 128 * 4)); }
  for (int i = 0; i < 6; ++i) {
    const float* w = fptr(c, EG + ".linears." + std::to_string(i) + ".weight");
    const float* b = fptr(c, EG + ".linears." + std::to_string(i) + ".bias");
    if (!w || !b) return RIFT_ERR_ARG;
    HIPCHK(c, hipMemcpyAsync(c->ego_w + i * 128, w, 128 * 4, hipMemcpyDeviceToDevice, c->stream));
    HIPCHK(c, hipMemcpyAsync(c->ego_b + i * 128, b, 128 * 4, hipMemcpyDeviceToDevice, c->stream));
  }
  TRY(pack_points_encoder(c, "map_encoder.polygon_encoder"));
  TRY(pack_fourier(c, "map_encoder.speed_limit_emb", 1));
  TRY(pack_fourier(c, "static_objects_encoder.obj_encoder", 2));
  TRY(pack_fourier(c, "pos_emb", 3));
  for (int i = 0; i < 4; ++i) {
    const std::string p = "encoder_blocks." + std::to_string(i);
    TRY(pack_self_mha(c, p + ".attn"));
    TRY(pack_linear(c, p + ".mlp.fc1")); TRY(pack_linear(c, p + ".mlp.fc2")); TRY(pack_hid(c, p + ".mlp.fc2"));
  }
  {
    int idx[384];
// ... 36 lines not shown
    for (int i = 0; i < 4; ++i) {
      wn.push_back(PD + ".decoder_blocks." + std::to_string(i) + ".cross_attn.in_proj_weight");
      bn.push_back(PD + ".decoder_blocks." + std::to_string(i) + ".cross_attn.in_proj_bias");
    }
    TRY(pack_stacked_rows(c, PD + ".kv_all", wn, bn, 128, 256));
  }
  TRY(pack_streamed_images(c));
  TRY(pack_cols(c, PD + ".cat_x_proj.q", PD + ".cat_x_proj", 0, 128, true));
  TRY(pack_cols(c, PD + ".cat_x_proj.x", PD + ".cat_x_proj", 128, 128, false));
  const char* hd[3] = {"loc_head", "yaw_head", "vel_head"};
  for (int i = 0; i < 3; ++i) TRY(pack_mlp_layer(c, PD + "." + hd[i]));
  TRY(pack_linear(c, "hidden_proj.0")); TRY(pack_linear(c, "hidden_proj.2"));
  TRY(pack_mlp_layer(c, "ref_free_decoder"));
  const char* need[] = {"norm.weight", "agent_encoder.type_emb.weight", "map_encoder.type_emb.weight",
                        "planning_decoder.m_emb", "planning_decoder.m_pos", "planning_decoder.pi_head.mlp.0.weight",
                        "planning_decoder.pi_head.mlp.3.weight", "agent_encoder.ego_state_emb.query"};
  for (const char* nme : need) if (!fptr(c, nme)) return RIFT_ERR_ARG;
  HIPCHK(c, hipGetLastError());
  c->loaded = true;
  return RIFT_OK;
}

int rift_forward(RiftCtx* c, const RiftFeatureBatch* B, const RiftOutputs* out, int flags, uint32_t seed, void* stream) {
  if (!c || !B || !out) return RIFT_ERR_ARG;
  c->err.clear();
  if (!c->loaded) { c->err = "rift_forward before rift_model_load"; return RIFT_ERR_STATE; }
  if (B->bs <= 0 || B->A <= 0 || B->Mp <= 0 || B->R <= 0 || B->S < 0 || B->T < 21) { c->err = "bad batch dims"; return RIFT_ERR_ARG; }
  HIPCHK(c, hipSetDevice(c->device));
  c->stream = (hipStream_t)stream;
  c->parity = (flags & RIFT_F_DEFER_HEAD) ? (c->parity + 1) % RIFT_DEFER_SLOTS : 0;
  c->arena = c->arenas[c->parity]; c->arena_cap = c->arena_caps[c->parity];
  long long omask = 0;
  { const void* const* op = reinterpret_cast<const void* const*>(out); for (size_t i = 0; i < sizeof(RiftOutputs) / sizeof(void*); ++i) omask |= (long long)(op[i] != nullptr) << i; }
  const long long dkey[11] = {B->bs, B->A, B->Mp, B->R, B->S, B->T, flags, c->dp.on ? 1 : 0, c->dp.on ? c->dp.gbs : 0, omask, c->prof_on ? 1 : 0};
  int rc = RIFT_OK;
  if (c->dry_need == 0 || memcmp(dkey, c->dry_key, sizeof(dkey)) != 0) {
    c->dry = true; c->arena_off = 0; c->dry_need = 0;
    rc = forward_impl(c, B, out, flags, seed);
    c->stream = (hipStream_t)stream;
    if (rc != RIFT_OK) { c->dry = false; return rc; }
    memcpy(c->dry_key, dkey, sizeof(dkey)); c->dry_need = c->arena_off;
  }
  const size_t need = c->dry_need;
  if (need > c->arena_cap) {
    HIPCHK(c, hipDeviceSynchronize());
    if (c->arena) HIPCHK(c, hipFree(c->arena));
    c->arena = nullptr; c->arena_cap = 0;
    const size_t cap = need + (need >> 3);
    HIPCHK(c, hipMalloc((void**)&c->arena, cap));
    c->arena_cap = cap;
  }
  c->arenas[c->parity] = c->arena; c->arena_caps[c->parity] = c->arena_cap;
  c->dry = false; c->arena_off = 0; c->taps.clear();
  if (c->dg.poison_arena >= 0 && c->arena) { HIPCHK(c, hipMemsetAsync(c->arena, c->dg.poison_arena, c->arena_cap, plan_of(c, (flags & RIFT_F_FP32) != 0, B->bs).prefetched ? c->prep_stream : c->stream)); }
  rc = forward_impl(c, B, out, flags, seed);
  c->stream = (hipStream_t)stream;
  if (rc != RIFT_OK) return rc;
  if (!c->err.empty()) return RIFT_ERR_ARG;
  if (c->arena_off > c->arena_cap) {
    c->dry_need = 0;
    c->err = "activation arena overrun: the forward allocated " + std::to_string(c->arena_off) + " B of a " + std::to_string(c->arena_cap) + " B arena (stale sizing pass)";
    (void)hipDeviceSynchronize();
    return RIFT_ERR_STATE;
  }
  HIPCHK(c, hipGetLastError());
  return RIFT_OK;
}
// ... 738 lines not shown
  std::vector<int> slots((size_t)K);
  for (int k = 0; k < K; ++k) {
    if (cbvs[k].batch_index < 0) return refuse("batch_index < 0");
    if (cbvs[k].slot < 0 || cbvs[k].slot >= n_slots) return refuse("slot outside [0, n_slots)");
    slots[(size_t)k] = cbvs[k].slot;
  }
  std::sort(slots.begin(), slots.end());
  if (std::adjacent_find(slots.begin(), slots.end()) != slots.end()) return refuse("two CBVs with the same slot");
  c->err.clear();
  if (K == 0) return RIFT_OK;
  HIPCHK(c, hipSetDevice(c->device));
  const hipStream_t st = (hipStream_t)stream;
  for (int k0 = 0; k0 < K; k0 += RIFT_CTL_CHUNK) {
    CtlArr a; memset(&a, 0, sizeof(a));
    a.K = std::min(RIFT_CTL_CHUNK, K - k0); a.G = (int)G; a.Tfull = Tfull; a.topk = topk; a.interval = sample_interval;
    for (int j = 0; j < a.K; ++j) {
      const RiftControlCBV& v = cbvs[k0 + j];
      CtlK& d = a.d[j];
      d.traj = trajectory + (size_t)v.batch_index * (size_t)G * Tfull * 6;
      d.prob = probability + (size_t)v.batch_index * (size_t)G;
      d.rf = ref_free_trajectory ? ref_free_trajectory + (size_t)v.batch_index * Tfull * 4 : nullptr;
      d.state = pid_state + (size_t)v.slot * RIFT_CTL_STATE;
      d.dec = decision + (size_t)(k0 + j) * 8;
      d.ox = v.x; d.oy = v.y; d.ch = std::cos(v.heading); d.sh = std::sin(v.heading); d.speed = v.speed;
    }
    if (G <= 64 * 2) hipLaunchKernelGGL(control_tick_kernel<2>, dim3(a.K), dim3(64), 0, st, a);
    else if (G <= 64 * 4) hipLaunchKernelGGL(control_tick_kernel<4>, dim3(a.K), dim3(64), 0, st, a);
    else hipLaunchKernelGGL(control_tick_kernel<16>, dim3(a.K), dim3(64), 0, st, a);
    HIPCHK(c, hipGetLastError());
  }
  return RIFT_OK;
}

int rift_collate(RiftCtx* c, const RiftReplayArena* ar, const int32_t* scene_idx, int bs, int R_out,
                 const RiftFeatureBatch* ob, float* out_old_logits, float* out_ref_logits, double* out_advantage,
                 uint8_t* out_valid_mask, void* stream) {
  if (!c || !ar || !scene_idx || !ob || bs <= 0 || R_out <= 0 || R_out > ar->Rcap) return RIFT_ERR_ARG;
  if (ob->A > ar->A || ob->Mp > ar->Mp || ob->S > ar->S || ob->A <= 0 || ob->T != ar->T) return RIFT_ERR_ARG;
  const RiftFeatureBatch& s = ar->scenes;
  const int A = ar->A, Mp = ar->Mp, Rc = ar->Rcap, S = ar->S, T = ar->T;
  const int oA = ob->A, oMp = ob->Mp, oS = ob->S;
  CollateP p; memset(&p, 0, sizeof(p));
  int k = 0;
  auto add = [&](const void* src, void* dst, long long src_bytes, long long dst_bytes) {
    if (!src || !dst || dst_bytes <= 0) return;
    p.src[k] = (const unsigned char*)src; p.dst[k] = (unsigned char*)dst; p.src_bytes[k] = (int)src_bytes; p.dst_bytes[k] = (int)dst_bytes; ++k;
  };
#define FIX(field, n_src, n_dst, per) add(s.field, (void*)ob->field, (long long)(n_src) * (per), (long long)(n_dst) * (per))
  FIX(agent_position, A, oA, T * 8); FIX(agent_heading, A, oA, T * 4); FIX(agent_velocity, A, oA, T * 8);
  FIX(agent_shape, A, oA, T * 8); FIX(agent_category, A, oA, 1); FIX(agent_valid_mask, A, oA, T);
  FIX(map_point_position, Mp, oMp, 3 * 20 * 8); FIX(map_point_vector, Mp, oMp, 3 * 20 * 8);
  FIX(map_point_orientation, Mp, oMp, 3 * 20 * 4); FIX(map_polygon_center, Mp, oMp, 12);
  FIX(map_polygon_type, Mp, oMp, 1); FIX(map_polygon_on_route, Mp, oMp, 1); FIX(map_polygon_tl_status, Mp, oMp, 1);
  FIX(map_polygon_has_speed_limit, Mp, oMp, 1); FIX(map_polygon_speed_limit, Mp, oMp, 4); FIX(map_valid_mask, Mp, oMp, 20);
  FIX(static_position, S, oS, 8); FIX(static_heading, S, oS, 4); FIX(static_shape, S, oS, 8);
  FIX(static_category, S, oS, 1); FIX(static_valid_mask, S, oS, 1); FIX(current_state, 1, 1, ar->cs_ld * 4);
#undef FIX
#define RAG(srcp, dstp, per_line) add((srcp), (void*)(dstp), (long long)Rc * (per_line), (long long)R_out * (per_line))
  RAG(s.ref_position, ob->ref_position, 120 * 8); RAG(s.ref_vector, ob->ref_vector, 120 * 8);
  RAG(s.ref_orientation, ob->ref_orientation, 120 * 4); RAG(s.ref_valid_mask, ob->ref_valid_mask, 120);
  RAG(ar->old_group_logits, out_old_logits, 12 * 4); RAG(ar->ref_group_logits, out_ref_logits, 12 * 4);
  RAG(ar->group_advantage, out_advantage, 12 * 8); RAG(ar->group_valid_mask, out_valid_mask, 12);
#undef RAG
  p.nt = k;
  hipLaunchKernelGGL(collate_kernel, dim3(bs, k), dim3(256), 0, (hipStream_t)stream, p, scene_idx);
  HIPCHK(c, hipGetLastError());
  return RIFT_OK;
}

}}

#include "abi_table.h"
#if RIFT_OP_F16
#define RIFT_VT_SYM rift_vtable_fp16
#else
#define RIFT_VT_SYM rift_vtable_bf16
#endif
#if !defined(__HIP_DEVICE_COMPILE__)
extern "C" const RiftVTable RIFT_VT_SYM = {
#define RIFT_FN(name) &RIFT_NS::abi::name,
#include "abi_list.h"
#undef RIFT_FN
};
#endif
```

### rift_amd/csrc/kernels.h

```cpp
#pragma once
#include "common.h"
#include "token.h"

namespace RIFT_NS {

#define RIFT_PI 3.14159265358979323846f

template <bool BF16>
__global__ void pack_weight_kernel(const float* __restrict__ src, void* dst, int N, int K, int Npad, int Kp,
                                   int conv_C, int tap_lo, int tap_n, int src_row_off, int src_ld) {
  const int idx = blockIdx.x * blockDim.x + threadIdx.x;
  if (idx >= Npad * Kp) return;
  const int n = idx / Kp, k = idx - n * Kp;
  float v = 0.f;
  if (n < N && k < K) {
    if (conv_C > 0) {
      const int j = k / conv_C, c = k - j * conv_C;
      if (j < tap_n) v = src[((size_t)n * conv_C + c) * 3 + tap_lo + j];
    } else {
      v = src[(size_t)(n + src_row_off) * src_ld + k];
    }
  }
  if (BF16) reinterpret_cast<unsigned short*>(dst)[fm_index(n, k, Kp)] = f2h(v);
  else reinterpret_cast<float*>(dst)[idx] = v;
// ... 451 lines not shown
}

__global__ void fpn_merge_kernel(const float* __restrict__ lat0, const float* __restrict__ lat1,
                                 const float* __restrict__ lat2, int nA, float* __restrict__ Z) {
  const int idx = blockIdx.x * blockDim.x + threadIdx.x;
  if (idx >= nA * 128) return;
  const int c = idx & 127, a = idx >> 7;
  const float l2a = lat2[((size_t)a * 2 + 0) * 128 + c], l2b = lat2[((size_t)a * 2 + 1) * 128 + c];
  const float l1a = lat1[((size_t)a * 2 + 0) * 128 + c] + (0.25f * l2a + 0.75f * l2b);
  const float l1b = lat1[((size_t)a * 2 + 1) * 128 + c] + l2b;
  Z[(size_t)a * 256 + c] = lat0[((size_t)a * 2 + 0) * 128 + c] + (0.25f * l1a + 0.75f * l1b);
  Z[(size_t)a * 256 + 128 + c] = lat0[((size_t)a * 2 + 1) * 128 + c] + l1b;
}

__global__ void ego_token_kernel(const float* __restrict__ cs, int cs_ld, const float* __restrict__ lw ,
                                 const float* __restrict__ lb , const float* __restrict__ pos_embed, int bs,
                                 float* __restrict__ E) {
  const int idx = blockIdx.x * blockDim.x + threadIdx.x;
  if (idx >= bs * 6 * 128) return;
  const int c = idx & 127, i = (idx >> 7) % 6, b = idx / (6 * 128);
  E[idx] = (cs[(size_t)b * cs_ld + i] * lw[i * 128 + c] + lb[i * 128 + c]) + pos_embed[i * 128 + c];
}

__global__ void ego_dropmask_kernel(int bs, float p, uint32_t seed, uint32_t stream, uint8_t* __restrict__ mask) {
  const int idx = blockIdx.x * blockDim.x + threadIdx.x;
  if (idx >= bs * 6) return;
  const int i = idx % 6;
  mask[idx] = (i >= 3 && uniform01(seed, stream, (uint32_t)idx) < p) ? 1 : 0;
}

__device__ __forceinline__ void agent_token_body(const int idx, const float* __restrict__ nat, const float* __restrict__ x_ego,
                                                 const uint8_t* __restrict__ valid_agent, const int8_t* __restrict__ category,
                                                 const float* __restrict__ type_emb, int bs, int A, int N, float* __restrict__ X,
                                                 const float* __restrict__ pe ) {
  if (idx >= bs * A * 32) return;
  const int c = (idx & 31) * 4, a = (idx >> 5) % A, b = idx / (A * 32);
  *reinterpret_cast<float4*>(X + ((size_t)b * N + a) * 128 + c) = agent_token_value(b, a, c, nat, x_ego, valid_agent, category, type_emb, A, N, pe);
}

__device__ __forceinline__ void polygon_token_body(const int idx, const float* __restrict__ pooled, const int8_t* __restrict__ ptype,
                                                   const uint8_t* __restrict__ on_route, const int8_t* __restrict__ tl,
                                                   const uint8_t* __restrict__ has_sl, const float* __restrict__ speed_emb,
                                                   const float* __restrict__ type_emb, const float* __restrict__ route_emb,
                                                   const float* __restrict__ tl_emb, const float* __restrict__ unk_emb, int bs,
                                                   int A, int Mp, int N, float* __restrict__ X, const float* __restrict__ pe) {
  if (idx >= bs * Mp * 32) return;
  const int c = (idx & 31) * 4, m = (idx >> 5) % Mp, b = idx / (Mp * 32);
  *reinterpret_cast<float4*>(X + ((size_t)b * N + A + m) * 128 + c) =
      polygon_token_value(b, m, c, pooled, ptype, on_route, tl, has_sl, speed_emb, type_emb, route_emb, tl_emb, unk_emb, A, Mp, N, pe);
}

__global__ void token_kernel(TokenP p) {
  if ((int)blockIdx.x < p.nblk_a)
    agent_token_body(blockIdx.x * blockDim.x + threadIdx.x, p.nat, p.x_ego, p.valid_agent, p.category, p.a_type_emb, p.bs, p.A, p.N, p.X, p.pe);
  else
    polygon_token_body((blockIdx.x - p.nblk_a) * blockDim.x + threadIdx.x, p.pooled, p.ptype, p.on_route, p.tl, p.has_sl, p.speed_emb, p.p_type_emb,
                       p.route_emb, p.tl_emb, p.unk_emb, p.bs, p.A, p.Mp, p.N, p.X, p.pe);
}

__global__ void static_token_kernel(const float* __restrict__ emb, const int8_t* __restrict__ cat,
                                    const uint8_t* __restrict__ valid, const float* __restrict__ type_emb, int bs,
                                    int A, int Mp, int S, int N, float* __restrict__ X) {
  const int idx = blockIdx.x * blockDim.x + threadIdx.x;
  if (idx >= bs * S * 128) return;
  const int c = idx & 127, s = (idx >> 7) % S, b = idx / (S * 128);
  const int o = b * S + s;
  X[((size_t)b * N + A + Mp + s) * 128 + c] = valid[o] ? emb[(size_t)o * 128 + c] + type_emb[(int)cat[o] * 128 + c] : 0.f;
}

__global__ void add_inplace_kernel(float* __restrict__ Y, const float* __restrict__ Z, size_t n) {
  const size_t idx = (size_t)blockIdx.x * blockDim.x + threadIdx.x;
  if (idx < n) Y[idx] += Z[idx];
}

__global__ void build_q0_kernel(const float* __restrict__ Ra, const float* __restrict__ Mb, int nLine, int M,
                                float* __restrict__ Q) {
  const int idx = blockIdx.x * blockDim.x + threadIdx.x;
  if (idx >= nLine * M * 128) return;
  const int c = idx & 127, m = (idx >> 7) % M, l = idx / (M * 128);
  Q[idx] = Ra[(size_t)l * 128 + c] + Mb[(size_t)m * 128 + c];
}

__device__ __forceinline__ void refline_pos_body(const float* __restrict__ rp, const float* __restrict__ ro, int nLine,
                                   float* __restrict__ pos, const int vblk) {
  const int l = vblk * (int)blockDim.x + (int)threadIdx.x;
  if (l >= nLine) return;
  pos[l * 3] = rp[(size_t)l * 240]; pos[l * 3 + 1] = rp[(size_t)l * 240 + 1]; pos[l * 3 + 2] = ro[(size_t)l * 120];
}

__global__ void gather_rows_kernel(const float* __restrict__ X, int ldx, float* __restrict__ Y, int ldy, int rows,
// ... 68 lines not shown
  if (mark) {
    const int c = (wbase[wave] + lane) % 3;
    int r = (int)((base >> (21 * c)) & 0x1fffffull);
#pragma unroll
    for (int w = 0; w < 4; ++w) {
      if (w > wave) break;
      const unsigned long long sel = s_mask[w] & rk_class_mask((c - wbase[w] + 3) % 3);
      r += __builtin_popcountll(w < wave ? sel : (sel & ((1ull << lane) - 1ull)));
    }
    q.aidx[3 * r + c] = b * A + tid;
  }
  if (b == q.nrk - 1 && tid < 3) q.cnt[tid] = (int)((base >> (21 * tid)) & 0x1fffffull) + own[tid];
}

__device__ __forceinline__ void prep_body(const PrepP& q, int blk) {
  if (blk < q.nrk) { rank_scene_body(q, blk); return; }
  blk -= q.nrk;
  if (blk < q.nb[0]) { agent_feature_body(q.agent_pos, q.agent_head, q.agent_vel, q.agent_shape, q.agent_valid, q.nA, q.Tfull, q.F9, q.valid_agent, blk, q.hist_agent, q.A); return; }
  blk -= q.nb[0];
  if (blk < q.nb[1]) { map_feature_body(q.map_pp, q.map_pv, q.map_po, q.map_center, q.nPoly, q.F10, blk); return; }
  blk -= q.nb[1];
  if (blk < q.nb[2]) { ref_feature_body(q.ref_pos, q.ref_vec, q.ref_ori, q.nLine, q.F6, blk); return; }
  blk -= q.nb[2];
  if (blk < q.nb[3]) { refline_pos_body(q.ref_pos, q.ref_ori, q.nLine, q.r_pos, blk); return; }
  blk -= q.nb[3];
  if (blk < q.nb[4]) { refline_mask_body(q.ref_valid, q.nLine, q.r_kpm, blk, q.r_tiles); return; }
  blk -= q.nb[4];
  if (blk < q.nb[5]) { token_mask_body(nullptr, q.map_valid, q.static_valid, q.bs, q.A, q.Mp, q.S, q.kpm, blk, q.agent_valid, q.Tfull); return; }
  blk -= q.nb[5];
  token_pos_body(q.agent_pos, q.agent_head, q.Tfull, q.map_center, q.st_pos, q.st_head, q.bs, q.A, q.Mp, q.S, q.pos, blk);
}
__global__ __launch_bounds__(256) void prep_kernel(PrepP q) { prep_body(q, blockIdx.x); }

}
```

### rift_amd/csrc/pe_fused.h

```cpp
#pragma once
#include <hip/hip_fp16.h>
#include "common.h"

namespace RIFT_NS {

struct PeP {
  const float* F; int Cin;
  const uint8_t* valid;
  int rows, ntiles;
  const unsigned short *w1, *w2, *w3a, *w3b, *w4;
  const float *b1, *b2, *b3, *b4;
  const float *s1, *t1, *s2, *t2;
  float* part1;
  float* part2;
  int* cnt;
  float* part1w; int* cnt1w; int nwg1;
  unsigned short* Fmid;
  float* gp;
  float* out;
  int do_stats;
  long long* ts;
  int ts_tile;
};

#define PEW_TAB_INTS 32
struct PePackP {
  const uint8_t* tiles; int nlines;
  int* tab;
  int* hdr;
  int max_rounds;
};
struct PeLiveP {
  const int* cnt[2]; int nt[2];
  int nr[2];
  int grid;
  int* live[2];
  int* hdr;
  const int* packed_b;
};

#define PEW_PACK_SEGS 32
__device__ __forceinline__ void pe_pack_body(const PePackP& q, int* __restrict__ pk_lds, int* __restrict__ seg_rounds ) {
  const int tid = threadIdx.x, NT = blockDim.x;
  int* const enc = pk_lds + q.nlines;
  for (int l = tid; l < q.nlines; l += NT) pk_lds[l] = q.tiles[l];
  __syncthreads();
  const int nseg = min(PEW_PACK_SEGS, max(1, q.nlines / 32));
  const int per = (q.nlines + nseg - 1) / nseg;
  if (tid < PEW_PACK_SEGS) {
// ... 131 lines not shown
template <int MT, int NTW, int NW, class F>
__device__ __forceinline__ void pe_tile_stats(const f32x4 (&acc)[MT][NTW], const unsigned char* sval, F&& addend, float* part, int C,
                                              int ntiles, int tile, int wave, int l15, int l4) {
  f32x2_t okf[MT];
#pragma unroll
  for (int mt = 0; mt < MT; ++mt) okf[mt] = (f32x2_t)(sval[mt * 16 + l15] == 1 ? 1.0f : 0.0f);
#pragma unroll
  for (int j = 0; j < NTW; ++j) {
    const int col = (j * NW + wave) * 16 + l4 * 4;
    f32x2_t s01 = (f32x2_t)0.f, s23 = s01, q01 = s01, q23 = s01;
#pragma unroll
    for (int mt = 0; mt < MT; ++mt) {
      const float4 a = addend(mt * 16 + l15, col);
      f32x2_t v01, v23, a01, a23;
      v01.x = acc[mt][j][0]; v01.y = acc[mt][j][1]; v23.x = acc[mt][j][2]; v23.y = acc[mt][j][3];
      a01.x = a.x; a01.y = a.y; a23.x = a.z; a23.y = a.w;
      v01 = (v01 + a01) * okf[mt]; v23 = (v23 + a23) * okf[mt];
      s01 += v01; s23 += v23;
      q01 = __builtin_elementwise_fma(v01, v01, q01); q23 = __builtin_elementwise_fma(v23, v23, q23);
    }
    float s[4] = {s01.x, s01.y, s23.x, s23.y}, q[4] = {q01.x, q01.y, q23.x, q23.y};
#pragma unroll
    for (int r = 0; r < 4; ++r) { s[r] = sum16(s[r]); q[r] = sum16(q[r]); }
    if (l15 == 0) {
#pragma unroll
      for (int r = 0; r < 4; ++r) {
        part[(size_t)(col + r) * ntiles + tile] = s[r];
        part[(size_t)(C + col + r) * ntiles + tile] = q[r];
      }
    }
  }
}

__device__ __forceinline__ void pe_stats1_body(const PeP& p, const int tile) {
  __shared__ __attribute__((aligned(16))) unsigned short xin[PE_ROWS * PE_XS];
  __shared__ unsigned char sval[PE_ROWS];
  __shared__ __attribute__((aligned(16))) float b1s[128];
  const int tid = threadIdx.x, lane = tid & 63, wave = tid >> 6, l15 = lane & 15, l4 = lane >> 4;
  PFrags<1, 2> W1;
  p_load_w<4, 1, 2>(W1, p.w1, 32, 0, wave, l15, l4);
  if (tid < 128) b1s[tid] = p.b1[tid];
  const int nv = pe_stage_x<256>(p, tile, xin, sval, tid);
  if (tid == 0) p.cnt[tile] = nv;
  if (nv == 0) {
    for (int i = tid; i < 256; i += 256) p.part1[(size_t)i * p.ntiles + tile] = 0.f;
    return;
  }
  f32x4 acc[8][2];
  p_zero(acc);
  p_mma<8, 1, 2>(acc, xin, PE_XS, 0, W1, l15, l4);
  pe_tile_stats<8, 2, 4>(acc, sval, [&](int, int c) { return *reinterpret_cast<const float4*>(b1s + c); }, p.part1, 128, p.ntiles, tile, wave, l15, l4);
}

struct PeP2 { PeP a, b; };

__device__ __forceinline__ void pe_stats1p_body(const PeP& p, const int wg, const int G) {
  __shared__ __attribute__((aligned(16))) unsigned short xin[PE_ROWS * PE_XS];
  __shared__ unsigned char sval[PE_ROWS];
  __shared__ __attribute__((aligned(16))) float b1s[128];
  const int tid = threadIdx.x, lane = tid & 63, wave = tid >> 6, l15 = lane & 15, l4 = lane >> 4;
  PFrags<1, 2> W1;
  p_load_w<4, 1, 2>(W1, p.w1, 32, 0, wave, l15, l4);
  if (tid < 128) b1s[tid] = p.b1[tid];
  f32x2_t s01[2], s23[2], q01[2], q23[2];
#pragma unroll
  for (int j = 0; j < 2; ++j) { s01[j] = (f32x2_t)0.f; s23[j] = s01[j]; q01[j] = s01[j]; q23[j] = s01[j]; }
  int nvw = 0;
  constexpr int NXL = (PE_USED * 10 + 255) / 256;
  const int Cin = p.Cin;
  const float rcin = 1.0f / (float)Cin;
  float xv[NXL];
  unsigned char fl = 0;
  auto request = [&](int tile) {
    const int row0 = tile * PE_USED;
    const int nfl = tile < p.ntiles ? min(PE_USED, p.rows - row0) * Cin : 0;
    fl = 0;
    if (tile < p.ntiles && tid < PE_USED && row0 + tid < p.rows) fl = p.valid[row0 + tid] ? 1 : 2;
#pragma unroll
    for (int u = 0; u < NXL; ++u) { const int i = tid + u * 256; xv[u] = i < nfl ? p.F[(size_t)row0 * Cin + i] : 0.f; }
  };
  for (int i = tid; i < PE_ROWS * PE_XS / 2; i += 256) reinterpret_cast<unsigned int*>(xin)[i] = 0u;
  request(wg);
  __syncthreads();
  for (int tile = wg; tile < p.ntiles; tile += G) {
    if (tid < PE_ROWS) sval[tid] = fl;
#pragma unroll
    for (int u = 0; u < NXL; ++u) {
      const int i = tid + u * 256;
      if (i < PE_USED * Cin) {
        const int r = (int)(((float)i + 0.5f) * rcin), k = i - r * Cin;
        xin[r * PE_XS + k] = f2h(xv[u]);
      }
    }
    const int nv = __syncthreads_count(fl == 1);
    request(tile + G);
    if (tid == 0) p.cnt[tile] = nv;
    nvw += nv;
    if (nv) {
      f32x4 acc[8][2];
      p_zero(acc);
      p_mma<8, 1, 2>(acc, xin, PE_XS, 0, W1, l15, l4);
#pragma unroll
      for (int j = 0; j < 2; ++j) {
        const float4 b = *reinterpret_cast<const float4*>(b1s + (j * 4 + wave) * 16 + l4 * 4);
        f32x2_t b01, b23;
        b01.x = b.x; b01.y = b.y; b23.x = b.z; b23.y = b.w;
#pragma unroll
        for (int mt = 0; mt < 8; ++mt) {
          const f32x2_t ok = (f32x2_t)(sval[mt * 16 + l15] == 1 ? 1.0f : 0.0f);
          f32x2_t v01, v23;
          v01.x = acc[mt][j][0]; v01.y = acc[mt][j][1]; v23.x = acc[mt][j][2]; v23.y = acc[mt][j][3];
          v01 = (v01 + b01) * ok; v23 = (v23 + b23) * ok;
          s01[j] += v01; s23[j] += v23;
          q01[j] = __builtin_elementwise_fma(v01, v01, q01[j]); q23[j] = __builtin_elementwise_fma(v23, v23, q23[j]);
        }
      }
    }
    __syncthreads();
  }
#pragma unroll
  for (int j = 0; j < 2; ++j) {
    const int col = (j * 4 + wave) * 16 + l4 * 4;
    float sv[4] = {s01[j].x, s01[j].y, s23[j].x, s23[j].y}, qv[4] = {q01[j].x, q01[j].y, q23[j].x, q23[j].y};
#pragma unroll
    for (int r = 0; r < 4; ++r) { sv[r] = sum16(sv[r]); qv[r] = sum16(qv[r]); }
    if (l15 == 0) {
#pragma unroll
      for (int r = 0; r < 4; ++r) {
        p.part1w[(size_t)(col + r) * G + wg] = sv[r];
        p.part1w[(size_t)(128 + col + r) * G + wg] = qv[r];
      }
    }
  }
  if (tid == 0) p.cnt1w[wg] = nvw;
}

__global__ __launch_bounds__(256) void pe_stats1p_kernel(PeP2 q, PePackP pk) {
  const int blk = (int)blockIdx.x - (pk.tiles ? 1 : 0);
  if (blk < 0) {
    extern __shared__ int pack_dyn[];
    __shared__ int seg_rounds[PEW_PACK_SEGS + 1];
    pe_pack_body(pk, pack_dyn, seg_rounds);
    return;
  }
  if (blk < q.a.nwg1) pe_stats1p_body(q.a, blk, q.a.nwg1);
  else pe_stats1p_body(q.b, blk - q.a.nwg1, q.b.nwg1);
}

__global__ __launch_bounds__(256) void pe_stats1_kernel(PeP2 q) {
  if ((int)blockIdx.x < q.a.ntiles) pe_stats1_body(q.a, blockIdx.x);
  else pe_stats1_body(q.b, blockIdx.x - q.a.ntiles);
}

#define PE_MID_LDS (PE_ROWS * PE_XS * 2 + PE_ROWS * PE_HS * 2 + PE_ROWS * PE_FS * 2 + 16 * PE_FS * 2 + 8 * 256 * 4 + 1024 * 4 + PE_ROWS)

template <int NPTS>
__device__ __forceinline__ void pe_mid_body(const PeP& p, const int tile) {
  constexpr int MT = 8, GPT = PE_USED / NPTS, NW = 8;
  constexpr int SPL = GPT >= 4 ? 1 : 4;
  constexpr int UNITS = GPT * SPL, RPU = NPTS / SPL;
  extern __shared__ __attribute__((aligned(16))) unsigned char smem_raw[];
  unsigned short* xin = reinterpret_cast<unsigned short*>(smem_raw);
  unsigned short* h1 = xin + PE_ROWS * PE_XS;
  unsigned short* fl = h1 + PE_ROWS * PE_HS;
  unsigned short* pool = fl + PE_ROWS * PE_FS;
  float* gpl = reinterpret_cast<float*>(pool + 16 * PE_FS);
  float* par = gpl + 8 * 256;
  unsigned char* sval = reinterpret_cast<unsigned char*>(par + 1024);
  constexpr int P_B1 = 0, P_S1 = 128, P_T1 = 256, P_B2 = 384, P_B3 = 640;
  const int tid = threadIdx.x, lane = tid & 63, wave = tid >> 6, l15 = lane & 15, l4 = lane >> 4;
  const int row0 = tile * PE_USED;
  int tsn = 0;
#define PTS() do { if (p.ts && tile == p.ts_tile && tid == 0) p.ts[tsn++] = clock64(); } while (0)
  PTS();

  PFrags<1, 1> W1;
  PFrags<4, 2> Wa, Wb;
  p_load_w<NW, 1, 1>(W1, p.w1, 32, 0, wave, l15, l4);
  p_load_w<NW, 4, 2>(Wa, p.w2, 128, 0, wave, l15, l4);
  {
    float pv[2];
#pragma unroll
    for (int u = 0; u < 2; ++u) {
      const int e = tid + u * 512;
// ... 232 lines not shown
      for (int r = r0; r < r0 + RPU; ++r) m = fmaxf(m, ol[r * OS + c]);
      if (SPL == 1) {
        const int grp = tile * GPT + g;
        if ((size_t)grp * NPTS < (size_t)p.rows) p.out[(size_t)grp * 128 + c] = m;
      } else pm[u * 128 + c] = m;
    }
  }
  if (SPL > 1) {
    __syncthreads();
    if (tid < 128) {
#pragma unroll
      for (int g = 0; g < GPT; ++g) {
        float m = pm[g * SPL * 128 + tid];
#pragma unroll
        for (int s = 1; s < SPL; ++s) m = fmaxf(m, pm[(g * SPL + s) * 128 + tid]);
        const int grp = tile * GPT + g;
        if ((size_t)grp * NPTS < (size_t)p.rows) p.out[(size_t)grp * 128 + tid] = m;
      }
    }
  }
}

__global__ __launch_bounds__(512) void pe_out_kernel(PeP2 q) {
  if ((int)blockIdx.x < q.a.ntiles) pe_out_body<20>(q.a, blockIdx.x);
  else pe_out_body<120>(q.b, blockIdx.x - q.a.ntiles);
}

struct BnFinP {
  const float* part; const int* cnt; int nblk, C;
  const int* nblk_dev;
  const float* gamma; const float* beta; float* running_mean; float* running_var; long long* num_batches;
  float* scale; float* shift;
  double* sums; int sums_mode;
};

__device__ __forceinline__ void bn_finalize_t_body(const BnFinP& p, int train, int update_running, float eps, int c) {
  constexpr int NT = 256, MAXU = 8;
  const int tid = threadIdx.x;
  const int nblk = p.nblk_dev ? *p.nblk_dev : p.nblk;
  float mean, var;
  if (train) {
    double s = 0.0, q = 0.0;
    long long n = 0;
    for (int b0 = 0; b0 < (p.sums_mode == 2 ? 0 : nblk); b0 += NT * MAXU) {
      float sv[MAXU], qv[MAXU]; int nv[MAXU];
#pragma unroll
      for (int u = 0; u < MAXU; ++u) {
        const int b = b0 + tid + u * NT;
        const bool ok = b < nblk;
        sv[u] = ok ? p.part[(size_t)c * nblk + b] : 0.f;
        qv[u] = ok ? p.part[(size_t)(p.C + c) * nblk + b] : 0.f;
        nv[u] = ok ? p.cnt[b] : 0;
      }
#pragma unroll
      for (int u = 0; u < MAXU; ++u) { s += (double)sv[u]; q += (double)qv[u]; n += nv[u]; }
    }
    s = wave_sum_d(s); q = wave_sum_d(q);
    double nd = wave_sum_d((double)n);
    __shared__ double red[3][4];
    if ((tid & 63) == 0) { red[0][tid >> 6] = s; red[1][tid >> 6] = q; red[2][tid >> 6] = nd; }
    __syncthreads();
    s = (red[0][0] + red[0][1]) + (red[0][2] + red[0][3]);
    q = (red[1][0] + red[1][1]) + (red[1][2] + red[1][3]);
    nd = (red[2][0] + red[2][1]) + (red[2][2] + red[2][3]);
    if (p.sums_mode == 1) {
      if (tid == 0) { p.sums[c] = s; p.sums[p.C + c] = q; if (c == 0) p.sums[2 * p.C] = nd; }
      return;
    }
    if (p.sums_mode == 2) { s = p.sums[c]; q = p.sums[p.C + c]; nd = p.sums[2 * p.C]; }
    const double mu = s / nd;
    double v = q / nd - mu * mu;
    v = v < 0.0 ? 0.0 : v;
    mean = (float)mu; var = (float)v;
    if (update_running && tid == 0) {
      const double unb = nd > 1.0 ? v * nd / (nd - 1.0) : v;
      p.running_mean[c] = 0.9f * p.running_mean[c] + 0.1f * mean;
      p.running_var[c] = 0.9f * p.running_var[c] + 0.1f * (float)unb;
      if (c == 0 && p.num_batches) *p.num_batches += 1;
    }
  } else { mean = p.running_mean[c]; var = p.running_var[c]; }
  if (tid == 0) {
    const float sc = p.gamma[c] * rsqrtf(var + eps);
    p.scale[c] = sc;
    p.shift[c] = p.beta[c] - mean * sc;
  }
}


__device__ __forceinline__ void pe_live_body(const PeLiveP& q) {
  __shared__ int sc[256];
  __shared__ int tot[2];
  const int tid = threadIdx.x;
  for (int e = 0; e < 2; ++e) {
    if (e == 1 && q.packed_b) { if (tid == 255) tot[1] = *q.packed_b; __syncthreads(); continue; }
    if (!q.cnt[e]) { if (tid == 255) tot[e] = q.nr[e]; __syncthreads(); continue; }
    const int R = q.nr[e], K = (R + 255) / 256, r0 = tid * K;
    auto is_live = [&](int r) { return r < R && (q.cnt[e][2 * r] + (2 * r + 1 < q.nt[e] ? q.cnt[e][2 * r + 1] : 0)) > 0; };
// ... 33 lines not shown
```

### rift_amd/csrc/pi_fused.h

```cpp
#pragma once
#include "common.h"
#include "pe_fused.h"

namespace RIFT_NS {

struct PiFwdP {
  const float* Q; int rows, rows_per_scene;
  const unsigned short* wq; const float* bq;
  const float* x0p;
  const float* w1; const float* b1;
  const float *lng, *lnb, *w2, *b2;
  const uint8_t* r_kpm; int M;
  float eps;
  float* QF; float* Hpi; float* prob;
  int* nonfinite;
};

#define PI_ROWS 128
#define PI_QS 144
#define PI_FS 132
#define PI_LDS (PI_ROWS * PI_QS * 2 + PI_ROWS * PI_FS * 4 + 8 * PI_ROWS * 2 * 4 + 8 * PI_ROWS * 4)

__global__ __launch_bounds__(512) void pi_forward_kernel(PiFwdP p) {
  constexpr int MT = 8, NW = 8;
// ... 78 lines not shown
    const int row = mt * 16 + l15;
    float s = 0.f;
#pragma unroll
    for (int w = 0; w < 8; ++w) s += wpart[(w * PI_ROWS + row) * 2];
    mean[mt] = s * (1.0f / 128.0f);
    const float d0 = h[mt][0] - mean[mt], d1 = h[mt][1] - mean[mt], d2 = h[mt][2] - mean[mt], d3 = h[mt][3] - mean[mt];
    float q = (d0 * d0 + d1 * d1) + (d2 * d2 + d3 * d3);
    q = rows_sum(q);
    if (l4 == 0) wpart[(wave * PI_ROWS + row) * 2 + 1] = q;
  }
  __syncthreads();
#pragma unroll
  for (int mt = 0; mt < MT; ++mt) {
    const int row = mt * 16 + l15;
    float q = 0.f;
#pragma unroll
    for (int w = 0; w < 8; ++w) q += wpart[(w * PI_ROWS + row) * 2 + 1];
    const float rstd = rsqrtf(q * (1.0f / 128.0f) + p.eps);
    float z = fmaxf((h[mt][0] - mean[mt]) * rstd * g4.x + e4.x, 0.f) * w24.x + fmaxf((h[mt][1] - mean[mt]) * rstd * g4.y + e4.y, 0.f) * w24.y +
              fmaxf((h[mt][2] - mean[mt]) * rstd * g4.z + e4.z, 0.f) * w24.z + fmaxf((h[mt][3] - mean[mt]) * rstd * g4.w + e4.w, 0.f) * w24.w;
    z = rows_sum(z);
    if (l4 == 0) zpart[wave * PI_ROWS + row] = z;
  }
  __syncthreads();
  if (tid < PI_ROWS && row0 + tid < p.rows) {
    float z = b2;
#pragma unroll
    for (int w = 0; w < 8; ++w) z += zpart[w * PI_ROWS + tid];
    const int gr = row0 + tid;
    p.prob[gr] = p.r_kpm[gr / p.M] ? -1e6f : z;
  }
}

struct Q0P { const float* r_emb; int nL, M; const unsigned short* wr; const float* br; const float* Mb; float* Q; };

__global__ __launch_bounds__(256) void q0_fused_kernel(Q0P p) {
  __shared__ __attribute__((aligned(16))) unsigned short xb[16 * 136];
  __shared__ __attribute__((aligned(16))) float ra[16 * 132];
  const int tid = threadIdx.x, lane = tid & 63, wave = tid >> 6, l15 = lane & 15, l4 = lane >> 4;
  const int l0 = blockIdx.x * 16;
  PFrags<4, 2> W;
  p_load_w<4, 4, 2>(W, p.wr, 128, 0, wave, l15, l4);
  {
    const int r = tid >> 4, c8 = (tid & 15) * 8;
    float4 v0 = make_float4(0.f, 0.f, 0.f, 0.f), v1 = v0;
    if (l0 + r < p.nL) { v0 = *reinterpret_cast<const float4*>(p.r_emb + (size_t)(l0 + r) * 128 + c8); v1 = *reinterpret_cast<const float4*>(p.r_emb + (size_t)(l0 + r) * 128 + c8 + 4); }
    uint4 o; o.x = pack_h2(v0.x, v0.y); o.y = pack_h2(v0.z, v0.w); o.z = pack_h2(v1.x, v1.y); o.w = pack_h2(v1.z, v1.w);
    *reinterpret_cast<uint4*>(xb + r * 136 + c8) = o;
  }
  __syncthreads();
  f32x4 acc[1][2];
  p_zero(acc);
  p_mma<1, 4, 2>(acc, xb, 136, 0, W, l15, l4);
#pragma unroll
  for (int j = 0; j < 2; ++j) {
    const int col = (j * 4 + wave) * 16 + l4 * 4;
    const float4 b4 = *reinterpret_cast<const float4*>(p.br + col);
    *reinterpret_cast<float4*>(ra + l15 * 132 + col) = make_float4(acc[0][j][0] + b4.x, acc[0][j][1] + b4.y, acc[0][j][2] + b4.z, acc[0][j][3] + b4.w);
  }
  __syncthreads();
  for (int i = tid; i < 16 * p.M * 32; i += 256) {
    const int c4 = (i & 31) * 4, rm = i >> 5, m = rm % p.M, r = rm / p.M;
    if (l0 + r >= p.nL) continue;
    const float4 a = *reinterpret_cast<const float4*>(ra + r * 132 + c4), mb = *reinterpret_cast<const float4*>(p.Mb + (size_t)m * 128 + c4);
    *reinterpret_cast<float4*>(p.Q + ((size_t)(l0 + r) * p.M + m) * 128 + c4) = make_float4(a.x + mb.x, a.y + mb.y, a.z + mb.z, a.w + mb.w);
  }
}

}
```

### rift_amd/csrc/token.h

```cpp
#pragma once
#include "common.h"

namespace RIFT_NS {

__device__ __forceinline__ float4 agent_token_value(const int b, const int a, const int c, const float* __restrict__ nat, const float* __restrict__ x_ego,
                                                    const uint8_t* __restrict__ valid_agent, const int8_t* __restrict__ category,
                                                    const float* __restrict__ type_emb, int A, int N, const float* __restrict__ pe) {
  const int ag = b * A + a;
  float4 v = make_float4(0.f, 0.f, 0.f, 0.f);
  if (a == 0) v = *reinterpret_cast<const float4*>(x_ego + (size_t)b * 128 + c);
  else if (valid_agent[ag]) v = *reinterpret_cast<const float4*>(nat + (size_t)ag * 128 + c);
  const float4 t = *reinterpret_cast<const float4*>(type_emb + (int)category[ag] * 128 + c);
  v.x += t.x; v.y += t.y; v.z += t.z; v.w += t.w;
  if (pe) { const float4 q = *reinterpret_cast<const float4*>(pe + ((size_t)b * N + a) * 128 + c); v.x += q.x; v.y += q.y; v.z += q.z; v.w += q.w; }
  return v;
}

__device__ __forceinline__ float4 polygon_token_value(const int b, const int m, const int c, const float* __restrict__ pooled, const int8_t* __restrict__ ptype,
                                                      const uint8_t* __restrict__ on_route, const int8_t* __restrict__ tl,
                                                      const uint8_t* __restrict__ has_sl, const float* __restrict__ speed_emb,
                                                      const float* __restrict__ type_emb, const float* __restrict__ route_emb,
                                                      const float* __restrict__ tl_emb, const float* __restrict__ unk_emb,
                                                      int A, int Mp, int N, const float* __restrict__ pe) {
  const int pg = b * Mp + m;
  auto ld = [&](const float* p) { return *reinterpret_cast<const float4*>(p + c); };
  const float4 a0 = ld(pooled + (size_t)pg * 128), a1 = ld(type_emb + (int)ptype[pg] * 128), a2 = ld(route_emb + (on_route[pg] ? 1 : 0) * 128),
               a3 = ld(tl_emb + (int)tl[pg] * 128), a4 = has_sl[pg] ? ld(speed_emb + (size_t)pg * 128) : ld(unk_emb);
  float4 v = make_float4(((a0.x + a1.x) + a2.x) + a3.x, ((a0.y + a1.y) + a2.y) + a3.y, ((a0.z + a1.z) + a2.z) + a3.z, ((a0.w + a1.w) + a2.w) + a3.w);
  v.x += a4.x; v.y += a4.y; v.z += a4.z; v.w += a4.w;
  if (pe) { const float4 q = *reinterpret_cast<const float4*>(pe + ((size_t)b * N + A + m) * 128 + c); v.x += q.x; v.y += q.y; v.z += q.z; v.w += q.w; }
  return v;
}

struct TokenP {
  const float *nat, *x_ego; const uint8_t* valid_agent; const int8_t* category; const float* a_type_emb;
  const float* pooled; const int8_t* ptype; const uint8_t* on_route; const int8_t* tl; const uint8_t* has_sl;
  const float *speed_emb, *p_type_emb, *route_emb, *tl_emb, *unk_emb;
  int bs, A, Mp, N, nblk_a; float* X; const float* pe;
};

}
```

### rift_amd/replay.py

```python
import ctypes as C
from typing import Dict, List, Optional, Sequence

import numpy as np
import torch

from rift_amd import _ffi

_F32, _I8, _U8 = torch.float32, torch.int8, torch.bool

_FIELDS = [
    ("agent_position", "agent", "position", _F32, False), ("agent_heading", "agent", "heading", _F32, False),
    ("agent_velocity", "agent", "velocity", _F32, False), ("agent_shape", "agent", "shape", _F32, False),
    ("agent_category", "agent", "category", _I8, False), ("agent_valid_mask", "agent", "valid_mask", _U8, False),
    ("map_point_position", "map", "point_position", _F32, False), ("map_point_vector", "map", "point_vector", _F32, False),
    ("map_point_orientation", "map", "point_orientation", _F32, False),
    ("map_polygon_center", "map", "polygon_center", _F32, False), ("map_polygon_type", "map", "polygon_type", _I8, False),
    ("map_polygon_on_route", "map", "polygon_on_route", _U8, False),
    ("map_polygon_tl_status", "map", "polygon_tl_status", _I8, False),
    ("map_polygon_has_speed_limit", "map", "polygon_has_speed_limit", _U8, False),
    ("map_polygon_speed_limit", "map", "polygon_speed_limit", _F32, False),
    ("map_valid_mask", "map", "valid_mask", _U8, False),
    ("ref_position", "reference_line", "position", _F32, True), ("ref_vector", "reference_line", "vector", _F32, True),
    ("ref_orientation", "reference_line", "orientation", _F32, True),
    ("ref_valid_mask", "reference_line", "valid_mask", _U8, True),
    ("static_position", "static_objects", "position", _F32, False),
    ("static_heading", "static_objects", "heading", _F32, False), ("static_shape", "static_objects", "shape", _F32, False),
    ("static_category", "static_objects", "category", _I8, False),
    ("static_valid_mask", "static_objects", "valid_mask", _U8, False),
]


def _pad_stack(ts: List[torch.Tensor], n: int, dtype) -> torch.Tensor:
    out = torch.zeros((len(ts), n) + tuple(ts[0].shape[1:]), dtype=dtype)
# ... 89 lines not shown
        ex = extras or {}
        adv = ex.get("group_advantage")
        self._put(i, "group_advantage", _np(adv) if adv is not None else np.zeros((R, 12)), torch.float64, "R")
        msk = ex.get("group_advantage_mask")
        self._put(i, "group_valid_mask", _np(msk) if msk is not None else np.ones((R, 12), dtype=np.bool_), _U8, "R")
        old = ex.get("old_group_logits")
        self._put(i, "old_group_logits", _np(old) if old is not None else np.zeros((R, 12), dtype=np.float32), _F32, "R")
        ref = ex.get("ref_group_logits")
        if ref is not None:
            self.has_ref_logits = True
            self._put(i, "ref_group_logits", _np(ref), _F32, "R")
        self.version += 1

    def reset(self):
        self.dims = {"A": 0, "Mp": 0, "R": 0, "S": 0}
        self.has_ref_logits = False
        self.version += 1

    def nbytes(self) -> int:
        return sum(t.numel() * t.element_size() for t in self.t.values())


class PersistentBatch(dict):
    persistent = True


class DeviceReplay:

    def __init__(self, scenes: Optional[List[Dict]], device, rcap: Optional[int] = None):
        self.device = torch.device(device)
        self._out = {}
        self.t: Dict[str, torch.Tensor] = {}
        self._host_version = None
        if scenes is None:
            return
        feats = [s["feature"] for s in scenes]
        ex = [s["extras"] for s in scenes]
        n = len(scenes)
        self.n = n
        self.A = max(f["agent"]["position"].shape[0] for f in feats)
        self.Mp = max(f["map"]["point_position"].shape[0] for f in feats)
        self.S = max(f["static_objects"]["position"].shape[0] for f in feats) if "static_objects" in feats[0] else 0
        self.T = feats[0]["agent"]["position"].shape[1]
        self.r_count_cpu = torch.tensor([f["reference_line"]["position"].shape[0] for f in feats], dtype=torch.int32)
        self.Rcap = int(rcap or self.r_count_cpu.max())
        dims = {"agent": self.A, "map": self.Mp, "reference_line": self.Rcap, "static_objects": self.S}
        for name, grp, key, dt, _ in _FIELDS:
            if grp == "static_objects" and self.S == 0:
                continue
            self.t[name] = _pad_stack([f[grp][key] for f in feats], dims[grp], dt).to(self.device)
        self.t["current_state"] = torch.stack([f["current_state"] for f in feats]).float().to(self.device)
        self.cs_ld = self.t["current_state"].shape[1]
        self.t["old_group_logits"] = _pad_stack([e["old_group_logits"] for e in ex], self.Rcap, _F32).to(self.device)
        self.t["group_advantage"] = _pad_stack([e["group_advantage"] for e in ex], self.Rcap, torch.float64).to(self.device)
        self.t["group_valid_mask"] = _pad_stack([e["group_advantage_mask"] for e in ex], self.Rcap, _U8).to(self.device)
        if "ref_group_logits" in ex[0]:
            self.t["ref_group_logits"] = _pad_stack([e["ref_group_logits"] for e in ex], self.Rcap, _F32).to(self.device)
        self.r_count = self.r_count_cpu.to(self.device)
        self._describe(self.A, self.Mp, self.Rcap, self.S)

    def _describe(self, capA: int, capMp: int, capR: int, capS: int):
        ar = _ffi.RiftReplayArena()
        ar.n_scenes, ar.A, ar.Mp, ar.Rcap, ar.S, ar.T, ar.cs_ld = self.n, capA, capMp, capR, capS, self.T, self.cs_ld
        ar.scenes.bs, ar.scenes.A, ar.scenes.Mp, ar.scenes.R, ar.scenes.S, ar.scenes.T = self.n, capA, capMp, capR, capS, self.T
        for name, *_ in _FIELDS:
            setattr(ar.scenes, name, self.t[name].data_ptr() if name in self.t else None)
        ar.scenes.current_state = self.t["current_state"].data_ptr()
        ar.scenes.cs_ld = self.cs_ld
        ar.r_count = self.r_count.data_ptr()
        ar.old_group_logits = self.t["old_group_logits"].data_ptr()
        ar.ref_group_logits = self.t["ref_group_logits"].data_ptr() if "ref_group_logits" in self.t else None
        ar.group_advantage = self.t["group_advantage"].data_ptr()
        ar.group_valid_mask = self.t["group_valid_mask"].data_ptr()
        self.arena = ar

    @classmethod
    def from_host(cls, host: HostReplay, device, n: Optional[int] = None) -> "DeviceReplay":
        self = cls(None, device)
        self.upload(host, n)
        return self

    def upload(self, host: HostReplay, n: Optional[int] = None):
        n = host.capacity if n is None else int(n)
        if host.T is None:
            raise ValueError("the host replay is empty")
        if self._host_version == (id(host), host.version, n):
            return
        caps, dims = host.caps, host.dims
        geom = (n, caps["A"], caps["Mp"], caps["R"], caps["S"], host.T, host.cs_ld, host.has_ref_logits, dims["S"] > 0)
        if getattr(self, "_geom", None) != geom:
            self.t = {}
            for name, src in host.t.items():
                if name == "ref_group_logits" and not host.has_ref_logits:
                    continue
                if _GROUP_OF.get(name) == "static_objects" and dims["S"] == 0:
                    continue
                self.t[name] = torch.empty((n,) + tuple(src.shape[1:]), dtype=src.dtype, device=self.device)
            self.r_count = torch.empty(n, dtype=torch.int32, device=self.device)
            self._geom = geom
        out_dims = (dims["A"], dims["Mp"], dims["S"])
        if getattr(self, "_out_dims", None) != out_dims:
            self._out = {}
            self._out_dims = out_dims
        self.n, self.T, self.cs_ld = n, host.T, host.cs_ld
        self.A, self.Mp, self.S, self.Rcap = dims["A"], dims["Mp"], dims["S"], caps["R"]
        for name, dst in self.t.items():
            dst.copy_(host.t[name][:n], non_blocking=True)
        self.r_count.copy_(host.r_count[:n], non_blocking=True)
        self.r_count_cpu = host.r_count[:n].clone()
        self._describe(caps["A"], caps["Mp"], caps["R"], caps["S"] if dims["S"] else 0)
        self._host_version = (id(host), host.version, n)

    def nbytes(self) -> int:
        return sum(t.numel() * t.element_size() for t in self.t.values())

    def _buffers(self, bs: int, R: int, slot: int = 0):
        key = (bs, R, slot)
        if key in self._out:
            return self._out[key]
        dev = self.device
        shp = {"agent": self.A, "map": self.Mp, "reference_line": R, "static_objects": self.S}
        b: Dict[str, torch.Tensor] = PersistentBatch()
        for name, grp, _, dt, _ in _FIELDS:
            if name not in self.t:
                continue
            b[name] = torch.zeros((bs, shp[grp]) + tuple(self.t[name].shape[2:]), dtype=dt, device=dev)
        b["current_state"] = torch.zeros(bs, self.cs_ld, device=dev)
        b["old_group_logits"] = torch.zeros(bs, R, 12, device=dev)
        b["ref_group_logits"] = torch.zeros(bs, R, 12, device=dev) if "ref_group_logits" in self.t else None
        b["group_advantage"] = torch.zeros(bs, R, 12, dtype=torch.float64, device=dev)
        b["group_valid_mask"] = torch.zeros(bs, R, 12, dtype=torch.bool, device=dev)
        fb = _ffi.RiftFeatureBatch()
        fb.bs, fb.A, fb.Mp, fb.R, fb.S, fb.T = bs, self.A, self.Mp, R, self.S, self.T
        for name, *_ in _FIELDS:
            setattr(fb, name, b[name].data_ptr() if name in b else None)
        fb.current_state = b["current_state"].data_ptr()
        fb.cs_ld = self.cs_ld
        self._out[key] = (fb, b)
        return self._out[key]

    def collate(self, engine: "_ffi.Engine", scene_idx: torch.Tensor, R_out: Optional[int] = None, slot: int = 0,
                stream: Optional[torch.cuda.Stream] = None):
        bs = scene_idx.numel()
        if R_out is None:
            R_out = self.Rcap
        cached = self._out.get((bs, R_out, slot))
        if cached is not None:
            fb, b = cached
        elif stream is not None:
            with torch.cuda.stream(stream):
                fb, b = self._buffers(bs, R_out, slot)
        else:
            fb, b = self._buffers(bs, R_out, slot)
        rc = engine.lib.rift_collate(
            engine.ctx, C.byref(self.arena), C.c_void_p(scene_idx.data_ptr()), bs, R_out, C.byref(fb),
            _ffi._ptr(b["old_group_logits"]), _ffi._ptr(b["ref_group_logits"]), _ffi._ptr(b["group_advantage"]),
            _ffi._ptr(b["group_valid_mask"]), C.c_void_p(stream.cuda_stream) if stream is not None else _ffi._stream())
        if stream is not None:
            scene_idx.record_stream(stream)
        if rc != 0:
            engine._check(rc, "rift_collate")
        return fb, b

    def batch_dict(self, b: Dict[str, torch.Tensor]) -> Dict:
        data = {"agent": {}, "map": {}, "reference_line": {}, "static_objects": {}}
        for name, grp, key, _, _ in _FIELDS:
            if name in b:
                data[grp][key] = b[name]
        data["current_state"] = b["current_state"]
        return data


DUMP_VERSION = 1


def save_scenes(path: str, scenes: List[Dict]) -> None:
    import numpy as np
    out = {"__rift_scene_dump__": np.array([DUMP_VERSION, len(scenes)], dtype=np.int64)}
    for i, s in enumerate(scenes):
        for grp, v in s["feature"].items():
            if isinstance(v, dict):
                for k, t in v.items():
                    out[f"{i}/{grp}/{k}"] = torch.as_tensor(t).cpu().numpy()
            else:
                out[f"{i}/{grp}"] = torch.as_tensor(v).cpu().numpy()
        for k, t in s.get("extras", {}).items():
            out[f"{i}/extras/{k}"] = torch.as_tensor(t).cpu().numpy()
    np.savez_compressed(path, **out)
# ... 22 lines not shown
```

Measured before the change: 469,000 scenes/s.

## Cache per-scene positional encodings and BN moments across replay updates

Adds a per-replay constants arena with token positional encodings, speed embeddings, reference-line PE, and per-scene second-order moments for the points-encoder batch-norm. It is keyed on engine serial, model generation and upload version. Collate gathers these by scene index, and a new forward path reads them instead of recomputing PE and first-layer BN statistics every step. The BN stats are rebuilt from per-scene moment matrices, which removes the stats pass over all points. In exchange it costs extra replay memory and depends on correct invalidation when the weights that produce these values change.

```diff
diff --git a/include/rift_hip.h b/include/rift_hip.h
--- a/include/rift_hip.h
+++ b/include/rift_hip.h
@@ -64,6 +64,16 @@
   int32_t cs_ld;
 } RiftFeatureBatch;
 
+typedef struct RiftSceneConstants {
+  const float*   token_pe;
+  const float*   speed_emb;
+  const int32_t* scene_idx;
+  const float*   ref_pe;
+  const double*  mom_map;
+  const double*  mom_ref;
+  int32_t ldA, ldMp;
+} RiftSceneConstants;
+
 typedef struct RiftOutputs {
   float* probability;
   float* hidden;
@@ -258,7 +268,16 @@
   const float*   ref_group_logits;
   const double*  group_advantage;
   const uint8_t* group_valid_mask;
+  RiftSceneConstants constants;
 } RiftReplayArena;
+
+int rift_replay_constants(RiftCtx* ctx, const RiftReplayArena* arena, void* stream);
+int rift_model_generation(RiftCtx* ctx, int64_t* count);
+int rift_collate_const(RiftCtx* ctx, const RiftReplayArena* arena, const int32_t* scene_idx , int bs, int R_out,
+                       const RiftFeatureBatch* out_batch, const RiftSceneConstants* out_const , float* out_old_logits,
+                       float* out_ref_logits, double* out_advantage, uint8_t* out_valid_mask, void* stream);
+int rift_forward_const(RiftCtx* ctx, const RiftFeatureBatch* batch, const RiftSceneConstants* batch_const ,
+                       const RiftOutputs* out, int flags, uint32_t seed, void* stream);
 
 int rift_collate(RiftCtx* ctx, const RiftReplayArena* arena, const int32_t* scene_idx , int bs,
                  int R_out, const RiftFeatureBatch* out_batch , float* out_old_logits,
diff --git a/rift_amd/_ffi.py b/rift_amd/_ffi.py
--- a/rift_amd/_ffi.py
+++ b/rift_amd/_ffi.py
@@ -1,4 +1,5 @@
 import ctypes as C
+import itertools
 import threading
 import os
 from typing import Dict, Optional
@@ -36,6 +37,13 @@
                 + [("cs_ld", C.c_int32)])
 
 
+_CONST_PTRS = ["token_pe", "speed_emb", "scene_idx", "ref_pe", "mom_map", "mom_ref"]
+
+
+class RiftSceneConstants(C.Structure):
+    _fields_ = [(n, vp) for n in _CONST_PTRS] + [("ldA", C.c_int32), ("ldMp", C.c_int32)]
+
+
 class RiftOutputs(C.Structure):
     _fields_ = [(n, vp) for n in ("probability", "hidden", "trajectory", "prediction", "ref_free_trajectory")]
 
@@ -59,7 +67,8 @@
     _fields_ = [(n, C.c_int32) for n in ("n_scenes", "A", "Mp", "Rcap", "S", "T", "cs_ld")] + \
                [("scenes", RiftFeatureBatch)] + \
                [(n, vp) for n in ("r_count", "old_group_logits", "ref_group_logits", "group_advantage",
-                                  "group_valid_mask")]
+                                  "group_valid_mask")] + \
+               [("constants", RiftSceneConstants)]
 
 
 EXCHANGE_FN = C.CFUNCTYPE(C.c_int, C.c_void_p, C.c_int64, C.c_int64, C.c_void_p)
@@ -121,7 +130,7 @@
 EXPORTS = [
     "rift_ctx_create", "rift_ctx_create_ex", "rift_ctx_operand_format", "rift_ctx_destroy", "rift_last_error", "rift_model_load", "rift_forward", "rift_forward_head", "rift_forward_head_back", "rift_loss_backward",
     "rift_loss_finalize", "rift_loss_finalize_clip", "rift_set_param_event", "rift_tap", "rift_op_linear", "rift_gae", "rift_discounted_return",
-    "rift_normalize_advantage", "rift_group_advantage", "rift_rollout_return", "rift_collate",
+    "rift_normalize_advantage", "rift_group_advantage", "rift_rollout_return", "rift_collate", "rift_replay_constants", "rift_model_generation", "rift_collate_const", "rift_forward_const",
     "rift_prof_enable", "rift_prof_report", "rift_op_linear_bench", "rift_ref_line_info", "rift_rollout",
     "rift_critic_forward", "rift_critic_loss_backward", "rift_critic_finalize", "rift_clip_grad_norm", "rift_adamw_step", "rift_update_tail", "rift_collision_matrix", "rift_off_road_matrix", "rift_other_vehicle_rollout", "rift_sft_teacher_mode",
     "rift_check_finite", "rift_set_dp", "rift_set_prepare_stream", "rift_set_side_stream",
@@ -205,6 +214,12 @@
     lib.rift_group_advantage.argtypes = [vp, vp, C.c_int, C.c_int, vp, vp]
     lib.rift_rollout_return.argtypes = [vp, vp, vp, vp, vp, vp, vp, vp, C.c_int, vp, C.c_int, C.c_int, C.c_int,
                                         C.c_double, vp, vp]
+    lib.rift_replay_constants.argtypes = [vp, C.POINTER(RiftReplayArena), vp]
+    lib.rift_model_generation.argtypes = [vp, C.POINTER(C.c_int64)]
+    lib.rift_collate_const.argtypes = [vp, C.POINTER(RiftReplayArena), vp, C.c_int, C.c_int, C.POINTER(RiftFeatureBatch),
+                                       C.POINTER(RiftSceneConstants), vp, vp, vp, vp, vp]
+    lib.rift_forward_const.argtypes = [vp, C.POINTER(RiftFeatureBatch), C.POINTER(RiftSceneConstants), C.POINTER(RiftOutputs), C.c_int,
+                                       C.c_uint32, vp]
     lib.rift_collate.argtypes = [vp, C.POINTER(RiftReplayArena), vp, C.c_int, C.c_int, C.POINTER(RiftFeatureBatch),
                                  vp, vp, vp, vp, vp]
     lib.rift_op_linear_bench.argtypes = [vp, vp, C.c_int, C.c_int, vp, vp, C.c_int, vp, vp, C.c_int, vp, vp, C.c_int,
@@ -307,6 +322,7 @@
 
 
 class Engine:
+    _serials = itertools.count(1)
 
     def __init__(self, device=None, operands: str = "bf16", variant: str = ""):
         if operands not in OPERANDS:
@@ -321,6 +337,7 @@
         rc = self.lib.rift_ctx_create_ex(self.device.index or 0, OPERANDS[operands], C.byref(self.ctx))
         if rc != 0:
             raise RuntimeError(f"rift_ctx_create_ex failed ({rc})")
+        self.serial = next(Engine._serials)
         self._params = None
         self._names = None
         self._keep = []
@@ -328,6 +345,11 @@
         self._stage_off = 0
         self._ctl_state = None
         self.generation = 0
+
+    def model_generation(self) -> int:
+        n = C.c_int64(0)
+        self._check(self.lib.rift_model_generation(self.ctx, C.byref(n)), "rift_model_generation")
+        return int(n.value)
 
     _STAGE_BYTES = 8 << 20
     _NP_OF = {torch.float32: np.float32, torch.float64: np.float64, torch.int32: np.int32, torch.int64: np.int64, torch.uint8: np.uint8,
@@ -471,7 +493,11 @@
         return out
 
     def forward_raw(self, fb: RiftFeatureBatch, out: RiftOutputs, flags: int, seed: int):
-        rc = self.lib.rift_forward(self.ctx, C.byref(fb), C.byref(out), flags, C.c_uint32(seed & 0xFFFFFFFF), _stream())
+        k = getattr(fb, "scene_constants", None)
+        if k is not None:
+            rc = self.lib.rift_forward_const(self.ctx, C.byref(fb), C.byref(k), C.byref(out), flags, C.c_uint32(seed & 0xFFFFFFFF), _stream())
+        else:
+            rc = self.lib.rift_forward(self.ctx, C.byref(fb), C.byref(out), flags, C.c_uint32(seed & 0xFFFFFFFF), _stream())
         self.generation += 1
         if rc != 0:
             self._check(rc, "rift_forward")
diff --git a/rift_amd/csrc/abi.cpp b/rift_amd/csrc/abi.cpp
--- a/rift_amd/csrc/abi.cpp
+++ b/rift_amd/csrc/abi.cpp
@@ -224,6 +224,26 @@
   return vt(ctx).rift_control_tick(ctx, trajectory, probability, ref_free_trajectory, Rb, Tfull, cbvs, K, topk, sample_interval, pid_state, n_slots, decision, stream);
 }
 
+int rift_replay_constants(RiftCtx* ctx, const RiftReplayArena* arena, void* stream) {
+  if (!ctx) return RIFT_ERR_ARG;
+  return vt(ctx).rift_replay_constants(ctx, arena, stream);
+}
+
+int rift_model_generation(RiftCtx* ctx, int64_t* count) {
+  if (!ctx) return RIFT_ERR_ARG;
+  return vt(ctx).rift_model_generation(ctx, count);
+}
+
+int rift_collate_const(RiftCtx* ctx, const RiftReplayArena* arena, const int32_t* scene_idx, int bs, int R_out, const RiftFeatureBatch* out_batch, const RiftSceneConstants* out_const, float* out_old_logits, float* out_ref_logits, double* out_advantage, uint8_t* out_valid_mask, void* stream) {
+  if (!ctx) return RIFT_ERR_ARG;
+  return vt(ctx).rift_collate_const(ctx, arena, scene_idx, bs, R_out, out_batch, out_const, out_old_logits, out_ref_logits, out_advantage, out_valid_mask, stream);
+}
+
+int rift_forward_const(RiftCtx* ctx, const RiftFeatureBatch* batch, const RiftSceneConstants* batch_const, const RiftOutputs* out, int flags, uint32_t seed, void* stream) {
+  if (!ctx) return RIFT_ERR_ARG;
+  return vt(ctx).rift_forward_const(ctx, batch, batch_const, out, flags, seed, stream);
+}
+
 int rift_collate(RiftCtx* ctx, const RiftReplayArena* arena, const int32_t* scene_idx, int bs, int R_out, const RiftFeatureBatch* out_batch, float* out_old_logits, float* out_ref_logits, double* out_advantage, uint8_t* out_valid_mask, void* stream) {
   if (!ctx) return RIFT_ERR_ARG;
   return vt(ctx).rift_collate(ctx, arena, scene_idx, bs, R_out, out_batch, out_old_logits, out_ref_logits, out_advantage, out_valid_mask, stream);
diff --git a/rift_amd/csrc/abi_list.h b/rift_amd/csrc/abi_list.h
--- a/rift_amd/csrc/abi_list.h
+++ b/rift_amd/csrc/abi_list.h
@@ -39,6 +39,10 @@
 RIFT_FN(rift_rollout_return_ex)
 RIFT_FN(rift_group_advantage_tick_ex)
 RIFT_FN(rift_control_tick)
+RIFT_FN(rift_replay_constants)
+RIFT_FN(rift_model_generation)
+RIFT_FN(rift_collate_const)
+RIFT_FN(rift_forward_const)
 RIFT_FN(rift_collate)
 RIFT_FN(rift_clip_grad_norm)
 RIFT_FN(rift_adamw_step)
diff --git a/rift_amd/csrc/adv.h b/rift_amd/csrc/adv.h
--- a/rift_amd/csrc/adv.h
+++ b/rift_amd/csrc/adv.h
@@ -274,10 +274,12 @@
   unsigned char* dst[RIFT_COLLATE_MAXT];
   int src_bytes[RIFT_COLLATE_MAXT];
   int dst_bytes[RIFT_COLLATE_MAXT];
+  int32_t* idx_out;
 };
 
 __global__ void collate_kernel(CollateP p, const int32_t* __restrict__ scene_idx) {
   const int k = blockIdx.y, b = blockIdx.x;
+  if (p.idx_out && k == 0 && threadIdx.x == 0) p.idx_out[b] = scene_idx[b];
   const unsigned char* s = p.src[k] + (size_t)scene_idx[b] * p.src_bytes[k];
   unsigned char* d = p.dst[k] + (size_t)b * p.dst_bytes[k];
   const int n = p.dst_bytes[k];
diff --git a/rift_amd/csrc/bn_moments.h b/rift_amd/csrc/bn_moments.h
--- /dev/null
+++ b/rift_amd/csrc/bn_moments.h
@@ -0,0 +1,41 @@
+#pragma once
+
+#if defined(__HIPCC__)
+#define BNM_HD __host__ __device__
+#else
+#define BNM_HD
+#endif
+
+BNM_HD inline int bnm_count(int D) { return (D + 1) * (D + 2) / 2; }
+
+BNM_HD inline int bnm_index(int D, int i, int j) { return i * (D + 1) - i * (i - 1) / 2 + (j - i); }
+
+BNM_HD inline void bnm_pair(int D, int e, int* i, int* j) {
+  int r = 0;
+  while (e >= D + 1 - r) { e -= D + 1 - r; ++r; }
+  *i = r; *j = r + e;
+}
+
+BNM_HD inline void bnm_add_point(double* M, int D, const double* x) {
+  int e = 0;
+  for (int i = 0; i <= D; ++i)
+    for (int j = i; j <= D; ++j) M[e++] += (i ? x[i - 1] : 1.0) * (j ? x[j - 1] : 1.0);
+}
+
+BNM_HD inline void bnm_term(const double* M, int D, const double* wa, int e, double* s, double* q) {
+  int i, j;
+  bnm_pair(D, e, &i, &j);
+  const double m = M[e];
+  *s = i == 0 ? wa[j] * m : 0.0;
+  *q = (i == j ? 1.0 : 2.0) * (wa[i] * wa[j]) * m;
+}
+
+BNM_HD inline void bnm_sums(const double* M, int D, const double* wa, double* sum, double* sumsq) {
+  double s = 0.0, q = 0.0;
+  for (int e = 0; e < bnm_count(D); ++e) {
+    double ts, tq;
+    bnm_term(M, D, wa, e, &ts, &tq);
+    s += ts; q += tq;
+  }
+  *sum = s; *sumsq = q;
+}
diff --git a/rift_amd/csrc/engine.hip b/rift_amd/csrc/engine.hip
--- a/rift_amd/csrc/engine.hip
+++ b/rift_amd/csrc/engine.hip
@@ -67,7 +67,7 @@
   struct WConst { float* p = nullptr; bool ready = false; };
   std::unordered_map<std::string, WConst> wconst;
   char* arena = nullptr; size_t arena_cap = 0, arena_off = 0;
-  long long dry_key[11] = {}; size_t dry_need = 0;
+  long long dry_key[12] = {}; size_t dry_need = 0;
   char* arenas[RIFT_DEFER_SLOTS] = {}; size_t arena_caps[RIFT_DEFER_SLOTS] = {}; int parity = 0;
   struct Head {
     bool valid = false, fp32 = false, need_traj = false;
@@ -101,6 +101,8 @@
   hipEvent_t param_event = nullptr;
   bool dec_fused = true;
   bool two_streams = true; bool nat_compact = true; bool pe_live = true; bool pe_pack = true;
+  bool scene_const = true; long long load_count = 0;
+  const RiftSceneConstants* batch_const = nullptr;
   hipStream_t prep_stream = nullptr; bool prep_set = false; hipEvent_t ev_prep = nullptr; int side_gate = 0;
   hipEvent_t ev_join2 = nullptr; bool nat_aside = true;
   hipStream_t side = nullptr; bool side_owned = false; hipEvent_t ev_fork = nullptr, ev_join = nullptr;
@@ -447,6 +449,7 @@
   const uint8_t* q_kpm = nullptr; int q_bs = 0, q_off = 0;
   float *nat_out = nullptr, *x_ego = nullptr, *poly = nullptr, *r_emb = nullptr, *speed_emb = nullptr, *PEtok = nullptr, *Q = nullptr, *X = nullptr;
   bool pe_pair = false, fo3 = false, rpe_done = false;
+  const float* r_pe_const = nullptr;
   float* ENC = nullptr;
   unsigned short* enc_KT = nullptr;
   uint8_t* kpm_c = nullptr;
@@ -600,7 +603,6 @@
   q.w3b = (const unsigned short*)w3b.bf; q.w4 = (const unsigned short*)w4.bf;
   q.b1 = w1.bias; q.b2 = w2.bias; q.b3 = w3a.bias; q.b4 = w4.bias;
   q.s1 = A_alloc<float>(c, 128); q.t1 = A_alloc<float>(c, 128); q.s2 = A_alloc<float>(c, 256); q.t2 = A_alloc<float>(c, 256);
-  q.part1 = A_alloc<float>(c, (size_t)2 * 128 * q.ntiles);
   q.part2 = A_alloc<float>(c, (size_t)2 * 256 * q.ntiles);
   q.cnt = A_alloc<int>(c, q.ntiles);
   q.Fmid = A_alloc<unsigned short>(c, (size_t)rows * 256);
@@ -627,9 +629,9 @@
   PeP2 q;
   pe_fill(f, q.a, Fm, 10, gm, 20, vm, pm);
   pe_fill(f, q.b, Fr, 6, gr, 120, vr, pr);
+  tap(c, "pe_x_map", (float*)Fm, (int64_t)q.a.rows * 10); tap(c, "pe_x_ref", (float*)Fr, (int64_t)q.b.rows * 6);
   const int nt = q.a.ntiles + q.b.ntiles;
   const double rows = (double)q.a.rows + q.b.rows, groups = (double)gm + gr;
-  const bool stats_p = f.train && c->pe_w;
   const bool packb = c->pe_w && c->pe_pack && gr > 0 && f.r_tiles != nullptr;
   int* pk_tab = nullptr; int* pk_hdr = nullptr;
   PePackP pk; memset(&pk, 0, sizeof(pk));
@@ -638,28 +640,34 @@
     pk_tab = A_alloc<int>(c, (size_t)std::max(maxr, 1) * PEW_TAB_INTS); pk_hdr = A_alloc<int>(c, 4);
     pk.tiles = f.r_tiles; pk.nlines = gr; pk.tab = pk_tab; pk.hdr = pk_hdr; pk.max_rounds = maxr;
     tap(c, "pe_pack_hdr", (float*)pk_hdr, 4); tap(c, "pe_pack_tab", (float*)pk_tab, (int64_t)std::max(maxr, 1) * PEW_TAB_INTS);
-    if (!stats_p) { c->prof_flops = 0.0; launch(c, "pe_pack_lines_kernel", pe_pack_lines_kernel, dim3(1), dim3(256), (size_t)gr * 2 * sizeof(int), pk); }
-  }
-  if (stats_p) {
-    int g = std::min(nt, 4 * c->nat_grid);
-    int ga = (int)(((long long)g * q.a.ntiles + nt / 2) / nt);
-    if (q.a.ntiles > 0 && ga < 1) ga = 1;
-    if (q.b.ntiles > 0 && ga > g - 1) ga = g - 1;
-    if (q.b.ntiles == 0) ga = g;
-    ga = std::min(ga, q.a.ntiles);
-    q.a.nwg1 = ga; q.b.nwg1 = std::min(g - ga, q.b.ntiles);
-    PeP* sd[2] = {&q.a, &q.b};
-    for (int i = 0; i < 2; ++i) { sd[i]->part1w = A_alloc<float>(c, (size_t)2 * 128 * std::max(sd[i]->nwg1, 1)); sd[i]->cnt1w = A_alloc<int>(c, std::max(sd[i]->nwg1, 1)); }
-    c->prof_flops = 2.0 * 128.0 * (q.a.rows * 10.0 + q.b.rows * 6.0);
-    launch(c, "pe_stats1_kernel", pe_stats1p_kernel, dim3(q.a.nwg1 + q.b.nwg1 + (packb ? 1 : 0)), dim3(256), packb ? (size_t)gr * 2 * sizeof(int) : 0, q, pk);
+    if (!f.train) { c->prof_flops = 0.0; launch(c, "pe_pack_lines_kernel", pe_pack_lines_kernel, dim3(1), dim3(256), (size_t)gr * 2 * sizeof(int), pk); }
+  }
+  PeMomP mo; memset(&mo, 0, sizeof(mo));
+  const RiftSceneConstants* K = c->batch_const;
+  const double* mom_in[2] = {K ? K->mom_map : nullptr, K ? K->mom_ref : nullptr};
+  const bool mom_cached = f.train && c->scene_const && mom_in[0] && mom_in[1];
+  int mom_scenes = 0;
+  if (mom_cached) {
+    mom_scenes = f.bs; mo.ncnt = std::min(32, std::max(1, cdiv(nt, 64)));
+    mo.nsum = f.bs; mo.in[0] = mom_in[0]; mo.in[1] = mom_in[1];
+    mo.tot[0] = A_alloc<double>(c, bnm_count(10)); mo.tot[1] = A_alloc<double>(c, bnm_count(6));
+    c->prof_flops = 0.0;
+    launch(c, "pe_stats1_kernel", pe_stats1_kernel, dim3((packb ? 1 : 0) + 2 + mo.ncnt), dim3(256), packb ? (size_t)gr * 2 * sizeof(int) : 0, q, pk, mo);
+    mo.mom[0] = (double*)mom_in[0]; mo.mom[1] = (double*)mom_in[1];
   } else if (f.train) {
-    c->prof_flops = 2.0 * 128.0 * (q.a.rows * 10.0 + q.b.rows * 6.0);
-    launch(c, "pe_stats1_kernel", pe_stats1_kernel, dim3(nt), dim3(256), 0, q);
+    const int ns = f.bs; mom_scenes = ns;
+    if (ns <= 0 || gm % ns || gr % ns) { if (c->err.empty()) c->err = "points_encoder_pair: polylines are not a whole number per scene"; return; }
+    mo.nscene = ns; mo.rps[0] = gm / ns * 20; mo.rps[1] = gr / ns * 120;
+    mo.mom[0] = A_alloc<double>(c, (size_t)ns * bnm_count(10)); mo.mom[1] = A_alloc<double>(c, (size_t)ns * bnm_count(6));
+    mo.ncnt = std::min(32, std::max(1, cdiv(nt, 64)));
+    tap(c, "pe_mom_map", (float*)mo.mom[0], (int64_t)ns * bnm_count(10) * 2); tap(c, "pe_mom_ref", (float*)mo.mom[1], (int64_t)ns * bnm_count(6) * 2);
+    c->prof_flops = 2.0 * (q.a.rows * (double)bnm_count(10) + q.b.rows * (double)bnm_count(6));
+    launch(c, "pe_stats1_kernel", pe_stats1_kernel, dim3((packb ? 1 : 0) + 2 * ns + mo.ncnt), dim3(256), packb ? (size_t)gr * 2 * sizeof(int) : 0, q, pk, mo);
   }
   const bool dpx = f.dp && f.train;
   double* xs = dpx ? c->dp.xchg + f.kb : nullptr;
   PeLiveP lv; memset(&lv, 0, sizeof(lv));
-  const bool live = stats_p && c->pe_live;
+  const bool live = f.train && c->pe_w && c->pe_live;
   int pew_grid = c->nat_grid, pew_ga = 0;
   if (c->pe_w) pew_split(cdiv(q.a.rows, PEW_ROUND_ROWS), cdiv(q.b.rows, PEW_ROUND_ROWS), &pew_grid, &pew_ga);
   if (live || packb) {
@@ -674,15 +682,19 @@
   }
   const bool lvblock = live || packb;
   for (int mode = dpx ? 1 : 0; mode <= (dpx ? 2 : 0); ++mode) {
-    BnFinP f1a = bn_fin(c, q.a, pm + ".first_mlp.1", 128, q.a.part1, q.a.s1, q.a.t1, xs, mode);
-    BnFinP f1b = bn_fin(c, q.b, pr + ".first_mlp.1", 128, q.b.part1, q.b.s1, q.b.t1, xs ? xs + 257 : nullptr, mode);
-    if (stats_p) { f1a.part = q.a.part1w; f1a.cnt = q.a.cnt1w; f1a.nblk = q.a.nwg1; f1b.part = q.b.part1w; f1b.cnt = q.b.cnt1w; f1b.nblk = q.b.nwg1; }
+    BnFinP f1a = bn_fin(c, q.a, pm + ".first_mlp.1", 128, nullptr, q.a.s1, q.a.t1, xs, mode);
+    BnFinP f1b = bn_fin(c, q.b, pr + ".first_mlp.1", 128, nullptr, q.b.s1, q.b.t1, xs ? xs + 257 : nullptr, mode);
+    f1a.mom = mo.mom[0]; f1a.nscene = mom_scenes; f1a.D = 10; f1a.w1 = q.a.w1; f1a.b1 = q.a.b1;
+    f1b.mom = mo.mom[1]; f1b.nscene = mom_scenes; f1b.D = 6; f1b.w1 = q.b.w1; f1b.b1 = q.b.b1;
+    f1a.mtot = mo.tot[0]; f1b.mtot = mo.tot[1];
     const bool with_lv = lvblock && mode == (dpx ? 2 : 0);
     PeLiveP none; memset(&none, 0, sizeof(none));
     launch(c, "bn_finalize_t_kernel", bn_finalize_t_kernel, dim3(256 + (with_lv ? 1 : 0)), dim3(256), 0, f1a, f1b, f.train ? 1 : 0, f.bn_update ? 1 : 0, 1e-5f,
            with_lv ? lv : none);
     if (mode == 1) dp_exchange(f, 2 * 257);
   }
+  tap(c, "pe_bn1_scale_map", (float*)q.a.s1, 128); tap(c, "pe_bn1_shift_map", (float*)q.a.t1, 128);
+  tap(c, "pe_bn1_scale_ref", (float*)q.b.s1, 128); tap(c, "pe_bn1_shift_ref", (float*)q.b.t1, 128);
   c->prof_flops = 2.0 * rows * (128.0 * 8 + 128.0 * 256 + (f.train ? 256.0 * 256 : 0.0)) + 2.0 * groups * 256.0 * 256;
   BnFinP fa, fb;
   if (c->pe_w) {
@@ -1140,6 +1152,7 @@
     Q0P q; memset(&q, 0, sizeof(q));
     q.r_emb = f.r_emb; q.nL = nL; q.M = M; q.wr = (const unsigned short*)c->pw[PD + ".q_proj.r"].bf; q.br = c->pw[PD + ".q_proj.r"].bias;
     q.Mb = Mb; q.Q = f.Q;
+    if (f.r_pe_const) { q.r_pe = f.r_pe_const; q.r_sum = f.r_emb; }
     c->prof_flops = 2.0 * nL * 128.0 * 128;
     launch(c, "q0_fused_kernel", q0_fused_kernel, dim3(cdiv(nL, 16)), dim3(256), 0, q);
   } else {
@@ -1159,7 +1172,12 @@
   else f.poly = points_encoder(f, f.F10, 10, nP, 20, B->map_valid_mask, "map_encoder.polygon_encoder");
   tap(c, "poly_pe", f.poly, (int64_t)nP * 128);
   f.fo3 = f.pe_pair && !f.fp32 && c->fo_fused && S == 0;
-  if (f.fo3) {
+  const RiftSceneConstants* K = c->batch_const;
+  const bool fo_const = f.fo3 && c->scene_const && c->fo_w && c->pi_fused && K && K->token_pe && K->speed_emb && K->ref_pe && K->scene_idx;
+  if (fo_const) {
+    tap(c, "r_pe", f.r_emb, (int64_t)nL * 128);
+    f.PEtok = (float*)K->token_pe; f.speed_emb = (float*)K->speed_emb; f.r_pe_const = K->ref_pe; f.rpe_done = true;
+  } else if (f.fo3) {
     tap(c, "r_pe", f.r_emb, (int64_t)nL * 128);
     FourierP3 q3; memset(&q3, 0, sizeof(q3));
     q3.e[0] = fourier_desc(f, f.pos, 3, nT, 3, "pos_emb", 2, nullptr);
@@ -1197,6 +1215,7 @@
   q.speed_emb = f.speed_emb; q.p_type_emb = fptr(c, "map_encoder.type_emb.weight"); q.route_emb = fptr(c, "map_encoder.on_route_emb.weight");
   q.tl_emb = fptr(c, "map_encoder.traffic_light_emb.weight"); q.unk_emb = fptr(c, "map_encoder.unknown_speed_emb.weight");
   q.bs = bs; q.A = A; q.Mp = Mp; q.N = N; q.X = f.X; q.pe = f.PEtok;
+  if (f.r_pe_const) { q.sidx = c->batch_const->scene_idx; q.ldA = c->batch_const->ldA; q.ldMp = c->batch_const->ldMp; }
   q.nblk_a = cdiv((long long)nA * 32, 256);
   launch(c, "token_kernel", token_kernel, dim3(q.nblk_a + cdiv((long long)nP * 32, 256)), dim3(256), 0, q);
   if (S > 0) {
@@ -1573,6 +1592,7 @@
   { int g = 0; env_int("RIFT_NAT_GRID", &g); if (g > 0) c->nat_grid = g; }
   env_flag("RIFT_NAT_COMPACT", &c->nat_compact);
   env_flag("RIFT_PE_LIVE", &c->pe_live);
+  env_flag("RIFT_SCENE_CONST", &c->scene_const);
   env_flag("RIFT_PE_PACK", &c->pe_pack);
   env_flag("RIFT_RANK_IN_PREP", &c->rank_in_prep);
   env_flag("RIFT_NO_SKIP", &c->no_skip);
@@ -1787,6 +1807,7 @@
   if (!c || !params) return RIFT_ERR_ARG;
   c->err.clear();
   c->stream = (hipStream_t)stream;
+  ++c->load_count;
   HIPCHK(c, hipSetDevice(c->device));
   for (void* p : c->owned) (void)hipFree(p);
   c->owned.clear(); c->pw.clear(); c->params.clear(); c->wconst.clear();
@@ -1889,7 +1910,8 @@
   c->arena = c->arenas[c->parity]; c->arena_cap = c->arena_caps[c->parity];
   long long omask = 0;
   { const void* const* op = reinterpret_cast<const void* const*>(out); for (size_t i = 0; i < sizeof(RiftOutputs) / sizeof(void*); ++i) omask |= (long long)(op[i] != nullptr) << i; }
-  const long long dkey[11] = {B->bs, B->A, B->Mp, B->R, B->S, B->T, flags, c->dp.on ? 1 : 0, c->dp.on ? c->dp.gbs : 0, omask, c->prof_on ? 1 : 0};
+  const long long dkey[12] = {B->bs, B->A, B->Mp, B->R, B->S, B->T, flags, c->dp.on ? 1 : 0, c->dp.on ? c->dp.gbs : 0, omask, c->prof_on ? 1 : 0,
+                              c->batch_const ? 1 : 0};
   int rc = RIFT_OK;
   if (c->dry_need == 0 || memcmp(dkey, c->dry_key, sizeof(dkey)) != 0) {
     c->dry = true; c->arena_off = 0; c->dry_need = 0;
@@ -2694,9 +2716,75 @@
   return RIFT_OK;
 }
 
-int rift_collate(RiftCtx* c, const RiftReplayArena* ar, const int32_t* scene_idx, int bs, int R_out,
-                 const RiftFeatureBatch* ob, float* out_old_logits, float* out_ref_logits, double* out_advantage,
-                 uint8_t* out_valid_mask, void* stream) {
+int rift_model_generation(RiftCtx* c, int64_t* count) {
+  if (!c || !count) return RIFT_ERR_ARG;
+  *count = (int64_t)c->load_count;
+  return RIFT_OK;
+}
+
+int rift_replay_constants(RiftCtx* c, const RiftReplayArena* ar, void* stream) {
+  if (!c || !ar) return RIFT_ERR_ARG;
+  c->err.clear();
+  const RiftFeatureBatch& s = ar->scenes;
+  const RiftSceneConstants& k = ar->constants;
+  const int n = ar->n_scenes, A = ar->A, Mp = ar->Mp, Rc = ar->Rcap, T = ar->T;
+  auto refuse = [&](const char* why) { c->err = std::string("rift_replay_constants: ") + why; return (int)RIFT_ERR_ARG; };
+  if (n <= 0 || A <= 0 || Mp < 0 || Rc <= 0) return refuse("empty arena");
+  if (ar->S != 0) return refuse("static objects: nothing is cached for such a replay");
+  if (!k.token_pe || !k.speed_emb || !k.ref_pe || !k.mom_map || !k.mom_ref) return refuse("null output tensor");
+  if (!c->fo_w || !c->fow_img[0] || !c->fow_img[1] || !c->fow_img[2]) return refuse("no model loaded (or RIFT_FO_W=0)");
+  HIPCHK(c, hipSetDevice(c->device));
+  const hipStream_t st = (hipStream_t)stream;
+  const int CH = std::min(n, 256);
+  const size_t nT = (size_t)CH * (A + Mp), nP = (size_t)CH * Mp, nL = (size_t)CH * Rc;
+  const size_t need = (nT * 3 + nL * 3 + nP * 20 * 10 + nL * 120 * 6) * sizeof(float) + 4 * 256;
+  char* scratch = nullptr;
+  HIPCHK(c, hipMalloc((void**)&scratch, need));
+  auto carve = [&](size_t floats) { float* p = (float*)scratch; scratch += (floats * 4 + 255) & ~(size_t)255; return p; };
+  char* const scratch0 = scratch;
+  float* pos = carve(nT * 3); float* r_pos = carve(nL * 3); float* F10 = carve(nP * 200); float* F6 = carve(nL * 720);
+  int rc = RIFT_OK;
+  for (int s0 = 0; s0 < n && rc == RIFT_OK; s0 += CH) {
+    const int m = std::min(CH, n - s0);
+    const int tT = m * (A + Mp), tP = m * Mp, tL = m * Rc;
+    PrepP q; memset(&q, 0, sizeof(q));
+    q.agent_pos = s.agent_position + (size_t)s0 * A * T * 2; q.agent_head = s.agent_heading + (size_t)s0 * A * T; q.Tfull = T;
+    q.map_pp = s.map_point_position + (size_t)s0 * Mp * 120; q.map_pv = s.map_point_vector + (size_t)s0 * Mp * 120;
+    q.map_po = s.map_point_orientation + (size_t)s0 * Mp * 60; q.map_center = s.map_polygon_center + (size_t)s0 * Mp * 3;
+    q.nPoly = tP; q.F10 = F10;
+    q.ref_pos = s.ref_position + (size_t)s0 * Rc * 240; q.ref_vec = s.ref_vector + (size_t)s0 * Rc * 240; q.ref_ori = s.ref_orientation + (size_t)s0 * Rc * 120;
+    q.nLine = tL; q.F6 = F6; q.r_pos = r_pos;
+    q.bs = m; q.A = A; q.Mp = Mp; q.S = 0; q.pos = pos;
+    q.nb[0] = cdiv((long long)tP * 20, 256); q.nb[1] = cdiv((long long)tL * 120, 256); q.nb[2] = cdiv(tL, 256); q.nb[3] = cdiv(tT, 256);
+    hipLaunchKernelGGL(scene_const_prep_kernel, dim3(q.nb[0] + q.nb[1] + q.nb[2] + q.nb[3]), dim3(256), 0, st, q);
+    FoWP w; memset(&w, 0, sizeof(w));
+    w.count = 3;
+    const float* in[3] = {pos, s.map_polygon_speed_limit + (size_t)s0 * Mp, r_pos};
+    float* Y[3] = {(float*)k.token_pe + (size_t)s0 * (A + Mp) * 128, (float*)k.speed_emb + (size_t)s0 * Mp * 128, (float*)k.ref_pe + (size_t)s0 * Rc * 128};
+    const int rows[3] = {tT, tP, tL}, D[3] = {3, 1, 3}, wrap[3] = {2, -1, -1};
+    for (int i = 0; i < 3; ++i) {
+      FoWSide& d = w.e[i];
+      d.in = in[i]; d.in_ld = D[i]; d.rows = rows[i]; d.D = D[i]; d.wrap_dim = wrap[i]; d.img = c->fow_img[i]; d.par = c->fow_par[i];
+      d.Y = Y[i]; d.accumulate = 0; d.rep = D[i] == 1 ? 2 : 1; d.nwg = cdiv(cdiv(rows[i], 16), 8 * d.rep);
+    }
+    fow_launch(w, st);
+    PeP2 pq; memset(&pq, 0, sizeof(pq));
+    pq.a.F = F10; pq.a.Cin = 10; pq.a.valid = s.map_valid_mask + (size_t)s0 * Mp * 20; pq.a.rows = tP * 20;
+    pq.b.F = F6; pq.b.Cin = 6; pq.b.valid = s.ref_valid_mask + (size_t)s0 * Rc * 120; pq.b.rows = tL * 120;
+    PeMomP mo; memset(&mo, 0, sizeof(mo));
+    mo.nscene = m; mo.rps[0] = Mp * 20; mo.rps[1] = Rc * 120;
+    mo.mom[0] = (double*)k.mom_map + (size_t)s0 * bnm_count(10); mo.mom[1] = (double*)k.mom_ref + (size_t)s0 * bnm_count(6);
+    hipLaunchKernelGGL(pe_moments_kernel, dim3(2 * m), dim3(256), 0, st, pq, mo);
+    if (hipGetLastError() != hipSuccess) { c->err = "rift_replay_constants: launch failed"; rc = RIFT_ERR_HIP; }
+  }
+  (void)hipStreamSynchronize(st);
+  (void)hipFree(scratch0);
+  return rc;
+}
+
+int rift_collate_const(RiftCtx* c, const RiftReplayArena* ar, const int32_t* scene_idx, int bs, int R_out,
+                       const RiftFeatureBatch* ob, const RiftSceneConstants* oc, float* out_old_logits, float* out_ref_logits,
+                       double* out_advantage, uint8_t* out_valid_mask, void* stream) {
   if (!c || !ar || !scene_idx || !ob || bs <= 0 || R_out <= 0 || R_out > ar->Rcap) return RIFT_ERR_ARG;
   if (ob->A > ar->A || ob->Mp > ar->Mp || ob->S > ar->S || ob->A <= 0 || ob->T != ar->T) return RIFT_ERR_ARG;
   const RiftFeatureBatch& s = ar->scenes;
@@ -2717,17 +2805,37 @@
   FIX(map_polygon_has_speed_limit, Mp, oMp, 1); FIX(map_polygon_speed_limit, Mp, oMp, 4); FIX(map_valid_mask, Mp, oMp, 20);
   FIX(static_position, S, oS, 8); FIX(static_heading, S, oS, 4); FIX(static_shape, S, oS, 8);
   FIX(static_category, S, oS, 1); FIX(static_valid_mask, S, oS, 1); FIX(current_state, 1, 1, ar->cs_ld * 4);
-#undef FIX
 #define RAG(srcp, dstp, per_line) add((srcp), (void*)(dstp), (long long)Rc * (per_line), (long long)R_out * (per_line))
   RAG(s.ref_position, ob->ref_position, 120 * 8); RAG(s.ref_vector, ob->ref_vector, 120 * 8);
   RAG(s.ref_orientation, ob->ref_orientation, 120 * 4); RAG(s.ref_valid_mask, ob->ref_valid_mask, 120);
   RAG(ar->old_group_logits, out_old_logits, 12 * 4); RAG(ar->ref_group_logits, out_ref_logits, 12 * 4);
   RAG(ar->group_advantage, out_advantage, 12 * 8); RAG(ar->group_valid_mask, out_valid_mask, 12);
+  const RiftSceneConstants& ac = ar->constants;
+  if (c->scene_const && oc && S == 0 && oS == 0 && ac.ref_pe && oc->ref_pe && oc->scene_idx) {
+    RAG(ac.ref_pe, oc->ref_pe, 512);
+    add(ac.mom_map, (void*)oc->mom_map, 66 * 8, 66 * 8); add(ac.mom_ref, (void*)oc->mom_ref, 28 * 8, 28 * 8);
+    p.idx_out = (int32_t*)oc->scene_idx;
+  }
+#undef FIX
 #undef RAG
   p.nt = k;
   hipLaunchKernelGGL(collate_kernel, dim3(bs, k), dim3(256), 0, (hipStream_t)stream, p, scene_idx);
   HIPCHK(c, hipGetLastError());
   return RIFT_OK;
+}
+
+int rift_collate(RiftCtx* c, const RiftReplayArena* ar, const int32_t* scene_idx, int bs, int R_out,
+                 const RiftFeatureBatch* ob, float* out_old_logits, float* out_ref_logits, double* out_advantage,
+                 uint8_t* out_valid_mask, void* stream) {
+  return abi::rift_collate_const(c, ar, scene_idx, bs, R_out, ob, nullptr, out_old_logits, out_ref_logits, out_advantage, out_valid_mask, stream);
+}
+
+int rift_forward_const(RiftCtx* c, const RiftFeatureBatch* B, const RiftSceneConstants* K, const RiftOutputs* out, int flags, uint32_t seed, void* stream) {
+  if (!c) return RIFT_ERR_ARG;
+  c->batch_const = K;
+  const int rc = abi::rift_forward(c, B, out, flags, seed, stream);
+  c->batch_const = nullptr;
+  return rc;
 }
 
 }}
diff --git a/rift_amd/csrc/kernels.h b/rift_amd/csrc/kernels.h
--- a/rift_amd/csrc/kernels.h
+++ b/rift_amd/csrc/kernels.h
@@ -507,10 +507,11 @@
 __device__ __forceinline__ void agent_token_body(const int idx, const float* __restrict__ nat, const float* __restrict__ x_ego,
                                                  const uint8_t* __restrict__ valid_agent, const int8_t* __restrict__ category,
                                                  const float* __restrict__ type_emb, int bs, int A, int N, float* __restrict__ X,
-                                                 const float* __restrict__ pe ) {
+                                                 const float* __restrict__ pe ,
+                                                 const int* __restrict__ sidx = nullptr, int ldA = 0, int ldMp = 0) {
   if (idx >= bs * A * 32) return;
   const int c = (idx & 31) * 4, a = (idx >> 5) % A, b = idx / (A * 32);
-  *reinterpret_cast<float4*>(X + ((size_t)b * N + a) * 128 + c) = agent_token_value(b, a, c, nat, x_ego, valid_agent, category, type_emb, A, N, pe);
+  *reinterpret_cast<float4*>(X + ((size_t)b * N + a) * 128 + c) = agent_token_value(b, a, c, nat, x_ego, valid_agent, category, type_emb, A, N, pe, sidx, ldA, ldMp);
 }
 
 __device__ __forceinline__ void polygon_token_body(const int idx, const float* __restrict__ pooled, const int8_t* __restrict__ ptype,
@@ -518,19 +519,20 @@
                                                    const uint8_t* __restrict__ has_sl, const float* __restrict__ speed_emb,
                                                    const float* __restrict__ type_emb, const float* __restrict__ route_emb,
                                                    const float* __restrict__ tl_emb, const float* __restrict__ unk_emb, int bs,
-                                                   int A, int Mp, int N, float* __restrict__ X, const float* __restrict__ pe) {
+                                                   int A, int Mp, int N, float* __restrict__ X, const float* __restrict__ pe,
+                                                   const int* __restrict__ sidx = nullptr, int ldA = 0, int ldMp = 0) {
   if (idx >= bs * Mp * 32) return;
   const int c = (idx & 31) * 4, m = (idx >> 5) % Mp, b = idx / (Mp * 32);
   *reinterpret_cast<float4*>(X + ((size_t)b * N + A + m) * 128 + c) =
-      polygon_token_value(b, m, c, pooled, ptype, on_route, tl, has_sl, speed_emb, type_emb, route_emb, tl_emb, unk_emb, A, Mp, N, pe);
+      polygon_token_value(b, m, c, pooled, ptype, on_route, tl, has_sl, speed_emb, type_emb, route_emb, tl_emb, unk_emb, A, Mp, N, pe, sidx, ldA, ldMp);
 }
 
 __global__ void token_kernel(TokenP p) {
   if ((int)blockIdx.x < p.nblk_a)
-    agent_token_body(blockIdx.x * blockDim.x + threadIdx.x, p.nat, p.x_ego, p.valid_agent, p.category, p.a_type_emb, p.bs, p.A, p.N, p.X, p.pe);
+    agent_token_body(blockIdx.x * blockDim.x + threadIdx.x, p.nat, p.x_ego, p.valid_agent, p.category, p.a_type_emb, p.bs, p.A, p.N, p.X, p.pe, p.sidx, p.ldA, p.ldMp);
   else
     polygon_token_body((blockIdx.x - p.nblk_a) * blockDim.x + threadIdx.x, p.pooled, p.ptype, p.on_route, p.tl, p.has_sl, p.speed_emb, p.p_type_emb,
-                       p.route_emb, p.tl_emb, p.unk_emb, p.bs, p.A, p.Mp, p.N, p.X, p.pe);
+                       p.route_emb, p.tl_emb, p.unk_emb, p.bs, p.A, p.Mp, p.N, p.X, p.pe, p.sidx, p.ldA, p.ldMp);
 }
 
 __global__ void static_token_kernel(const float* __restrict__ emb, const int8_t* __restrict__ cat,
@@ -665,4 +667,15 @@
 }
 __global__ __launch_bounds__(256) void prep_kernel(PrepP q) { prep_body(q, blockIdx.x); }
 
-}
+__global__ __launch_bounds__(256) void scene_const_prep_kernel(PrepP q) {
+  int blk = blockIdx.x;
+  if (blk < q.nb[0]) { map_feature_body(q.map_pp, q.map_pv, q.map_po, q.map_center, q.nPoly, q.F10, blk); return; }
+  blk -= q.nb[0];
+  if (blk < q.nb[1]) { ref_feature_body(q.ref_pos, q.ref_vec, q.ref_ori, q.nLine, q.F6, blk); return; }
+  blk -= q.nb[1];
+  if (blk < q.nb[2]) { refline_pos_body(q.ref_pos, q.ref_ori, q.nLine, q.r_pos, blk); return; }
+  blk -= q.nb[2];
+  token_pos_body(q.agent_pos, q.agent_head, q.Tfull, q.map_center, q.st_pos, q.st_head, q.bs, q.A, q.Mp, q.S, q.pos, blk);
+}
+
+}
diff --git a/rift_amd/csrc/pe_fused.h b/rift_amd/csrc/pe_fused.h
--- a/rift_amd/csrc/pe_fused.h
+++ b/rift_amd/csrc/pe_fused.h
@@ -1,6 +1,7 @@
 #pragma once
 #include <hip/hip_fp16.h>
 #include "common.h"
+#include "bn_moments.h"
 
 namespace RIFT_NS {
 
@@ -11,10 +12,8 @@
   const unsigned short *w1, *w2, *w3a, *w3b, *w4;
   const float *b1, *b2, *b3, *b4;
   const float *s1, *t1, *s2, *t2;
-  float* part1;
   float* part2;
   int* cnt;
-  float* part1w; int* cnt1w; int nwg1;
   unsigned short* Fmid;
   float* gp;
   float* out;
@@ -212,124 +211,116 @@
   }
 }
 
-__device__ __forceinline__ void pe_stats1_body(const PeP& p, const int tile) {
-  __shared__ __attribute__((aligned(16))) unsigned short xin[PE_ROWS * PE_XS];
-  __shared__ unsigned char sval[PE_ROWS];
-  __shared__ __attribute__((aligned(16))) float b1s[128];
-  const int tid = threadIdx.x, lane = tid & 63, wave = tid >> 6, l15 = lane & 15, l4 = lane >> 4;
-  PFrags<1, 2> W1;
-  p_load_w<4, 1, 2>(W1, p.w1, 32, 0, wave, l15, l4);
-  if (tid < 128) b1s[tid] = p.b1[tid];
-  const int nv = pe_stage_x<256>(p, tile, xin, sval, tid);
-  if (tid == 0) p.cnt[tile] = nv;
-  if (nv == 0) {
-    for (int i = tid; i < 256; i += 256) p.part1[(size_t)i * p.ntiles + tile] = 0.f;
-    return;
-  }
-  f32x4 acc[8][2];
-  p_zero(acc);
-  p_mma<8, 1, 2>(acc, xin, PE_XS, 0, W1, l15, l4);
-  pe_tile_stats<8, 2, 4>(acc, sval, [&](int, int c) { return *reinterpret_cast<const float4*>(b1s + c); }, p.part1, 128, p.ntiles, tile, wave, l15, l4);
+struct PeMomP {
+  int nscene;
+  int rps[2];
+  double* mom[2];
+  int ncnt;
+  int nsum; const double* in[2]; double* tot[2];
+};
+
+#define PE_MOM_CHUNK 256
+#define PE_MOM_LDS_F (PE_MOM_CHUNK * 11)
+#define PE_MOM_LDS_D 224
+
+template <int D>
+__device__ __forceinline__ void pe_moments_body(const PeP& p, const int scene, const int rps, double* __restrict__ out, float* __restrict__ xa,
+                                                double* __restrict__ part) {
+  constexpr int DA = D + 1, NE = DA * (DA + 1) / 2;
+  constexpr int NEP = NE > 64 ? 128 : NE > 32 ? 64 : 32, SL = 256 / NEP;
+  static_assert(PE_MOM_CHUNK % SL == 0 && SL * NE <= PE_MOM_LDS_D && DA <= 11, "moment block layout");
+  const int tid = threadIdx.x, e = tid & (NEP - 1), sl = tid / NEP;
+  int mi = 0, mj = 0;
+  bnm_pair(D, e < NE ? e : 0, &mi, &mj);
+  const size_t row0 = (size_t)scene * rps;
+  double acc = 0.0;
+  for (int c0 = 0; c0 < rps; c0 += PE_MOM_CHUNK) {
+    const int n = min(PE_MOM_CHUNK, rps - c0);
+    for (int i = tid; i < n * DA; i += 256) {
+      const int r = i / DA, k = i - r * DA;
+      const size_t row = row0 + c0 + r;
+      const bool ok = p.valid[row] != 0;
+      xa[i] = !ok ? 0.f : k == 0 ? 1.f : h2f(f2h(p.F[row * D + (k - 1)]));
+    }
+    __syncthreads();
+    if (e < NE) {
+#pragma unroll 4
+      for (int r = sl; r < n; r += SL) acc = fma((double)xa[r * DA + mi], (double)xa[r * DA + mj], acc);
+    }
+    __syncthreads();
+  }
+  if (e < NE) part[sl * NE + e] = acc;
+  __syncthreads();
+  if (tid < NE) {
+    double m = part[tid];
+#pragma unroll
+    for (int s = 1; s < SL; ++s) m += part[s * NE + tid];
+    out[(size_t)scene * NE + tid] = m;
+  }
+}
+
+__device__ __forceinline__ void mom_sum_scenes(const double* __restrict__ mom, const int nscene, const int NE, double* __restrict__ mpart,
+                                               double* __restrict__ out) {
+  const int tid = threadIdx.x, SL = 256 / NE, e = tid % NE, sl = tid / NE;
+  if (sl < SL) {
+    constexpr int MAXU = 8;
+    double acc = 0.0;
+    for (int s0 = sl; s0 < nscene; s0 += SL * MAXU) {
+      double v[MAXU];
+#pragma unroll
+      for (int u = 0; u < MAXU; ++u) { const int sc = s0 + u * SL; v[u] = sc < nscene ? mom[(size_t)sc * NE + e] : 0.0; }
+#pragma unroll
+      for (int u = 0; u < MAXU; ++u) acc += v[u];
+    }
+    mpart[tid] = acc;
+  }
+  __syncthreads();
+  if (tid < NE) {
+    double m = mpart[tid];
+    for (int k = 1; k < SL; ++k) m += mpart[k * NE + tid];
+    out[tid] = m;
+  }
+}
+
+__device__ __forceinline__ void pe_tile_counts_body(const PeP& a, const PeP& b, const int blk, const int nblk) {
+  const int lane = threadIdx.x & 63, nt = a.ntiles + b.ntiles;
+  for (int t = blk * 4 + (threadIdx.x >> 6); t < nt; t += nblk * 4) {
+    const PeP& p = t < a.ntiles ? a : b;
+    const int tile = t < a.ntiles ? t : t - a.ntiles, row0 = tile * PE_USED;
+    const bool v0 = row0 + lane < p.rows && p.valid[row0 + lane] != 0;
+    const bool v1 = lane + 64 < PE_USED && row0 + lane + 64 < p.rows && p.valid[row0 + lane + 64] != 0;
+    const int n = __popcll(__ballot(v0)) + __popcll(__ballot(v1));
+    if (lane == 0) p.cnt[tile] = n;
+  }
 }
 
 struct PeP2 { PeP a, b; };
 
-__device__ __forceinline__ void pe_stats1p_body(const PeP& p, const int wg, const int G) {
-  __shared__ __attribute__((aligned(16))) unsigned short xin[PE_ROWS * PE_XS];
-  __shared__ unsigned char sval[PE_ROWS];
-  __shared__ __attribute__((aligned(16))) float b1s[128];
-  const int tid = threadIdx.x, lane = tid & 63, wave = tid >> 6, l15 = lane & 15, l4 = lane >> 4;
-  PFrags<1, 2> W1;
-  p_load_w<4, 1, 2>(W1, p.w1, 32, 0, wave, l15, l4);
-  if (tid < 128) b1s[tid] = p.b1[tid];
-  f32x2_t s01[2], s23[2], q01[2], q23[2];
-#pragma unroll
-  for (int j = 0; j < 2; ++j) { s01[j] = (f32x2_t)0.f; s23[j] = s01[j]; q01[j] = s01[j]; q23[j] = s01[j]; }
-  int nvw = 0;
-  constexpr int NXL = (PE_USED * 10 + 255) / 256;
-  const int Cin = p.Cin;
-  const float rcin = 1.0f / (float)Cin;
-  float xv[NXL];
-  unsigned char fl = 0;
-  auto request = [&](int tile) {
-    const int row0 = tile * PE_USED;
-    const int nfl = tile < p.ntiles ? min(PE_USED, p.rows - row0) * Cin : 0;
-    fl = 0;
-    if (tile < p.ntiles && tid < PE_USED && row0 + tid < p.rows) fl = p.valid[row0 + tid] ? 1 : 2;
-#pragma unroll
-    for (int u = 0; u < NXL; ++u) { const int i = tid + u * 256; xv[u] = i < nfl ? p.F[(size_t)row0 * Cin + i] : 0.f; }
-  };
-  for (int i = tid; i < PE_ROWS * PE_XS / 2; i += 256) reinterpret_cast<unsigned int*>(xin)[i] = 0u;
-  request(wg);
-  __syncthreads();
-  for (int tile = wg; tile < p.ntiles; tile += G) {
-    if (tid < PE_ROWS) sval[tid] = fl;
-#pragma unroll
-    for (int u = 0; u < NXL; ++u) {
-      const int i = tid + u * 256;
-      if (i < PE_USED * Cin) {
-        const int r = (int)(((float)i + 0.5f) * rcin), k = i - r * Cin;
-        xin[r * PE_XS + k] = f2h(xv[u]);
-      }
-    }
-    const int nv = __syncthreads_count(fl == 1);
-    request(tile + G);
-    if (tid == 0) p.cnt[tile] = nv;
-    nvw += nv;
-    if (nv) {
-      f32x4 acc[8][2];
-      p_zero(acc);
-      p_mma<8, 1, 2>(acc, xin, PE_XS, 0, W1, l15, l4);
-#pragma unroll
-      for (int j = 0; j < 2; ++j) {
-        const float4 b = *reinterpret_cast<const float4*>(b1s + (j * 4 + wave) * 16 + l4 * 4);
-        f32x2_t b01, b23;
-        b01.x = b.x; b01.y = b.y; b23.x = b.z; b23.y = b.w;
-#pragma unroll
-        for (int mt = 0; mt < 8; ++mt) {
-          const f32x2_t ok = (f32x2_t)(sval[mt * 16 + l15] == 1 ? 1.0f : 0.0f);
-          f32x2_t v01, v23;
-          v01.x = acc[mt][j][0]; v01.y = acc[mt][j][1]; v23.x = acc[mt][j][2]; v23.y = acc[mt][j][3];
-          v01 = (v01 + b01) * ok; v23 = (v23 + b23) * ok;
-          s01[j] += v01; s23[j] += v23;
-          q01[j] = __builtin_elementwise_fma(v01, v01, q01[j]); q23[j] = __builtin_elementwise_fma(v23, v23, q23[j]);
-        }
-      }
-    }
-    __syncthreads();
-  }
-#pragma unroll
-  for (int j = 0; j < 2; ++j) {
-    const int col = (j * 4 + wave) * 16 + l4 * 4;
-    float sv[4] = {s01[j].x, s01[j].y, s23[j].x, s23[j].y}, qv[4] = {q01[j].x, q01[j].y, q23[j].x, q23[j].y};
-#pragma unroll
-    for (int r = 0; r < 4; ++r) { sv[r] = sum16(sv[r]); qv[r] = sum16(qv[r]); }
-    if (l15 == 0) {
-#pragma unroll
-      for (int r = 0; r < 4; ++r) {
-        p.part1w[(size_t)(col + r) * G + wg] = sv[r];
-        p.part1w[(size_t)(128 + col + r) * G + wg] = qv[r];
-      }
-    }
-  }
-  if (tid == 0) p.cnt1w[wg] = nvw;
-}
-
-__global__ __launch_bounds__(256) void pe_stats1p_kernel(PeP2 q, PePackP pk) {
-  const int blk = (int)blockIdx.x - (pk.tiles ? 1 : 0);
+__global__ __launch_bounds__(256) void pe_stats1_kernel(PeP2 q, PePackP pk, PeMomP m) {
+  int blk = (int)blockIdx.x - (pk.tiles ? 1 : 0);
   if (blk < 0) {
     extern __shared__ int pack_dyn[];
     __shared__ int seg_rounds[PEW_PACK_SEGS + 1];
     pe_pack_body(pk, pack_dyn, seg_rounds);
     return;
   }
-  if (blk < q.a.nwg1) pe_stats1p_body(q.a, blk, q.a.nwg1);
-  else pe_stats1p_body(q.b, blk - q.a.nwg1, q.b.nwg1);
-}
-
-__global__ __launch_bounds__(256) void pe_stats1_kernel(PeP2 q) {
-  if ((int)blockIdx.x < q.a.ntiles) pe_stats1_body(q.a, blockIdx.x);
-  else pe_stats1_body(q.b, blockIdx.x - q.a.ntiles);
+  __shared__ float mom_x[PE_MOM_LDS_F];
+  __shared__ double mom_part[256];
+  if (m.nsum > 0) {
+    if (blk < 2) { mom_sum_scenes(m.in[blk], m.nsum, bnm_count(blk == 0 ? 10 : 6), mom_part, m.tot[blk]); return; }
+    blk -= 2;
+  }
+  if (blk >= 2 * m.nscene) { pe_tile_counts_body(q.a, q.b, blk - 2 * m.nscene, m.ncnt); return; }
+  if (blk < m.nscene) pe_moments_body<10>(q.a, blk, m.rps[0], m.mom[0], mom_x, mom_part);
+  else pe_moments_body<6>(q.b, blk - m.nscene, m.rps[1], m.mom[1], mom_x, mom_part);
+}
+
+__global__ __launch_bounds__(256) void pe_moments_kernel(PeP2 q, PeMomP m) {
+  __shared__ float mom_x[PE_MOM_LDS_F];
+  __shared__ double mom_part[PE_MOM_LDS_D];
+  const int blk = blockIdx.x;
+  if (blk < m.nscene) pe_moments_body<10>(q.a, blk, m.rps[0], m.mom[0], mom_x, mom_part);
+  else pe_moments_body<6>(q.b, blk - m.nscene, m.rps[1], m.mom[1], mom_x, mom_part);
 }
 
 #define PE_MID_LDS (PE_ROWS * PE_XS * 2 + PE_ROWS * PE_HS * 2 + PE_ROWS * PE_FS * 2 + 16 * PE_FS * 2 + 8 * 256 * 4 + 1024 * 4 + PE_ROWS)
@@ -628,37 +619,73 @@
   const float* gamma; const float* beta; float* running_mean; float* running_var; long long* num_batches;
   float* scale; float* shift;
   double* sums; int sums_mode;
+  const double* mom; int nscene, D;
+  const double* mtot;
+  const unsigned short* w1;
+  const float* b1;
 };
 
+__device__ __forceinline__ void bn1_moment_sums(const BnFinP& p, const int c, double* s, double* q, double* nd) {
+  __shared__ double mpart[256];
+  __shared__ double mtot[66 + 11 + 3];
+  const int tid = threadIdx.x, D = p.D, NE = bnm_count(D);
+  double* wa = mtot + 66;
+  if (tid >= 192 && tid - 192 <= D) wa[tid - 192] = tid == 192 ? (double)p.b1[c] : (double)h2f(p.w1[fm_index(c, tid - 193, 32)]);
+  if (p.mtot) { if (tid < NE) mtot[tid] = p.mtot[tid]; }
+  else mom_sum_scenes(p.mom, p.nscene, NE, mpart, mtot);
+  __syncthreads();
+  if (tid < 64) {
+    double ss = 0.0, qq = 0.0;
+    for (int e = tid; e < NE; e += 64) {
+      double ts, tq;
+      bnm_term(mtot, D, wa, e, &ts, &tq);
+      ss += ts; qq += tq;
+    }
+    ss = wave_sum_d(ss); qq = wave_sum_d(qq);
+    if (tid == 0) { mtot[77] = ss; mtot[78] = qq; mtot[79] = mtot[0]; }
+  }
+  __syncthreads();
+  *s = mtot[77]; *q = mtot[78]; *nd = mtot[79];
+}
+
+__device__ __forceinline__ void bn_partial_sums(const BnFinP& p, const int c, const int nblk, double* so, double* qo, double* no) {
+  constexpr int NT = 256, MAXU = 8;
+  const int tid = threadIdx.x;
+  double s = 0.0, q = 0.0;
+  long long n = 0;
+  for (int b0 = 0; b0 < nblk; b0 += NT * MAXU) {
+    float sv[MAXU], qv[MAXU]; int nv[MAXU];
+#pragma unroll
+    for (int u = 0; u < MAXU; ++u) {
+      const int b = b0 + tid + u * NT;
+      const bool ok = b < nblk;
+      sv[u] = ok ? p.part[(size_t)c * nblk + b] : 0.f;
+      qv[u] = ok ? p.part[(size_t)(p.C + c) * nblk + b] : 0.f;
+      nv[u] = ok ? p.cnt[b] : 0;
+    }
+#pragma unroll
+    for (int u = 0; u < MAXU; ++u) { s += (double)sv[u]; q += (double)qv[u]; n += nv[u]; }
+  }
+  s = wave_sum_d(s); q = wave_sum_d(q);
+  double nd = wave_sum_d((double)n);
+  __shared__ double red[3][4];
+  if ((tid & 63) == 0) { red[0][tid >> 6] = s; red[1][tid >> 6] = q; red[2][tid >> 6] = nd; }
+  __syncthreads();
+  *so = (red[0][0] + red[0][1]) + (red[0][2] + red[0][3]);
+  *qo = (red[1][0] + red[1][1]) + (red[1][2] + red[1][3]);
+  *no = (red[2][0] + red[2][1]) + (red[2][2] + red[2][3]);
+}
+
 __device__ __forceinline__ void bn_finalize_t_body(const BnFinP& p, int train, int update_running, float eps, int c) {
-  constexpr int NT = 256, MAXU = 8;
   const int tid = threadIdx.x;
   const int nblk = p.nblk_dev ? *p.nblk_dev : p.nblk;
   float mean, var;
   if (train) {
-    double s = 0.0, q = 0.0;
-    long long n = 0;
-    for (int b0 = 0; b0 < (p.sums_mode == 2 ? 0 : nblk); b0 += NT * MAXU) {
-      float sv[MAXU], qv[MAXU]; int nv[MAXU];
-#pragma unroll
-      for (int u = 0; u < MAXU; ++u) {
-        const int b = b0 + tid + u * NT;
-        const bool ok = b < nblk;
-        sv[u] = ok ? p.part[(size_t)c * nblk + b] : 0.f;
-        qv[u] = ok ? p.part[(size_t)(p.C + c) * nblk + b] : 0.f;
-        nv[u] = ok ? p.cnt[b] : 0;
-      }
-#pragma unroll
-      for (int u = 0; u < MAXU; ++u) { s += (double)sv[u]; q += (double)qv[u]; n += nv[u]; }
-    }
-    s = wave_sum_d(s); q = wave_sum_d(q);
-    double nd = wave_sum_d((double)n);
-    __shared__ double red[3][4];
-    if ((tid & 63) == 0) { red[0][tid >> 6] = s; red[1][tid >> 6] = q; red[2][tid >> 6] = nd; }
-    __syncthreads();
-    s = (red[0][0] + red[0][1]) + (red[0][2] + red[0][3]);
-    q = (red[1][0] + red[1][1]) + (red[1][2] + red[1][3]);
-    nd = (red[2][0] + red[2][1]) + (red[2][2] + red[2][3]);
+    double s = 0.0, q = 0.0, nd = 0.0;
+    if (p.sums_mode != 2) {
+      if (p.mom) bn1_moment_sums(p, c, &s, &q, &nd);
+      else bn_partial_sums(p, c, nblk, &s, &q, &nd);
+    }
     if (p.sums_mode == 1) {
       if (tid == 0) { p.sums[c] = s; p.sums[p.C + c] = q; if (c == 0) p.sums[2 * p.C] = nd; }
       return;
diff --git a/rift_amd/csrc/pi_fused.h b/rift_amd/csrc/pi_fused.h
--- a/rift_amd/csrc/pi_fused.h
+++ b/rift_amd/csrc/pi_fused.h
@@ -134,7 +134,7 @@
   }
 }
 
-struct Q0P { const float* r_emb; int nL, M; const unsigned short* wr; const float* br; const float* Mb; float* Q; };
+struct Q0P { const float* r_emb; int nL, M; const unsigned short* wr; const float* br; const float* Mb; float* Q; const float* r_pe; float* r_sum; };
 
 __global__ __launch_bounds__(256) void q0_fused_kernel(Q0P p) {
   __shared__ __attribute__((aligned(16))) unsigned short xb[16 * 136];
@@ -146,7 +146,15 @@
   {
     const int r = tid >> 4, c8 = (tid & 15) * 8;
     float4 v0 = make_float4(0.f, 0.f, 0.f, 0.f), v1 = v0;
-    if (l0 + r < p.nL) { v0 = *reinterpret_cast<const float4*>(p.r_emb + (size_t)(l0 + r) * 128 + c8); v1 = *reinterpret_cast<const float4*>(p.r_emb + (size_t)(l0 + r) * 128 + c8 + 4); }
+    if (l0 + r < p.nL) {
+      const size_t o = (size_t)(l0 + r) * 128 + c8;
+      v0 = *reinterpret_cast<const float4*>(p.r_emb + o); v1 = *reinterpret_cast<const float4*>(p.r_emb + o + 4);
+      if (p.r_pe) {
+        const float4 e0 = *reinterpret_cast<const float4*>(p.r_pe + o), e1 = *reinterpret_cast<const float4*>(p.r_pe + o + 4);
+        v0 = make_float4(e0.x + v0.x, e0.y + v0.y, e0.z + v0.z, e0.w + v0.w); v1 = make_float4(e1.x + v1.x, e1.y + v1.y, e1.z + v1.z, e1.w + v1.w);
+        *reinterpret_cast<float4*>(p.r_sum + o) = v0; *reinterpret_cast<float4*>(p.r_sum + o + 4) = v1;
+      }
+    }
     uint4 o; o.x = pack_h2(v0.x, v0.y); o.y = pack_h2(v0.z, v0.w); o.z = pack_h2(v1.x, v1.y); o.w = pack_h2(v1.z, v1.w);
     *reinterpret_cast<uint4*>(xb + r * 136 + c8) = o;
   }
diff --git a/rift_amd/csrc/token.h b/rift_amd/csrc/token.h
--- a/rift_amd/csrc/token.h
+++ b/rift_amd/csrc/token.h
@@ -5,14 +5,18 @@
 
 __device__ __forceinline__ float4 agent_token_value(const int b, const int a, const int c, const float* __restrict__ nat, const float* __restrict__ x_ego,
                                                     const uint8_t* __restrict__ valid_agent, const int8_t* __restrict__ category,
-                                                    const float* __restrict__ type_emb, int A, int N, const float* __restrict__ pe) {
+                                                    const float* __restrict__ type_emb, int A, int N, const float* __restrict__ pe,
+                                                    const int* __restrict__ sidx = nullptr, int ldA = 0, int ldMp = 0) {
   const int ag = b * A + a;
   float4 v = make_float4(0.f, 0.f, 0.f, 0.f);
   if (a == 0) v = *reinterpret_cast<const float4*>(x_ego + (size_t)b * 128 + c);
   else if (valid_agent[ag]) v = *reinterpret_cast<const float4*>(nat + (size_t)ag * 128 + c);
   const float4 t = *reinterpret_cast<const float4*>(type_emb + (int)category[ag] * 128 + c);
   v.x += t.x; v.y += t.y; v.z += t.z; v.w += t.w;
-  if (pe) { const float4 q = *reinterpret_cast<const float4*>(pe + ((size_t)b * N + a) * 128 + c); v.x += q.x; v.y += q.y; v.z += q.z; v.w += q.w; }
+  if (pe) {
+    const size_t row = sidx ? (size_t)sidx[b] * (ldA + ldMp) + a : (size_t)b * N + a;
+    const float4 q = *reinterpret_cast<const float4*>(pe + row * 128 + c); v.x += q.x; v.y += q.y; v.z += q.z; v.w += q.w;
+  }
   return v;
 }
 
@@ -21,14 +25,19 @@
                                                       const uint8_t* __restrict__ has_sl, const float* __restrict__ speed_emb,
                                                       const float* __restrict__ type_emb, const float* __restrict__ route_emb,
                                                       const float* __restrict__ tl_emb, const float* __restrict__ unk_emb,
-                                                      int A, int Mp, int N, const float* __restrict__ pe) {
+                                                      int A, int Mp, int N, const float* __restrict__ pe,
+                                                      const int* __restrict__ sidx = nullptr, int ldA = 0, int ldMp = 0) {
   const int pg = b * Mp + m;
+  const size_t sp = sidx ? (size_t)sidx[b] * ldMp + m : (size_t)pg;
   auto ld = [&](const float* p) { return *reinterpret_cast<const float4*>(p + c); };
   const float4 a0 = ld(pooled + (size_t)pg * 128), a1 = ld(type_emb + (int)ptype[pg] * 128), a2 = ld(route_emb + (on_route[pg] ? 1 : 0) * 128),
-               a3 = ld(tl_emb + (int)tl[pg] * 128), a4 = has_sl[pg] ? ld(speed_emb + (size_t)pg * 128) : ld(unk_emb);
+               a3 = ld(tl_emb + (int)tl[pg] * 128), a4 = has_sl[pg] ? ld(speed_emb + sp * 128) : ld(unk_emb);
   float4 v = make_float4(((a0.x + a1.x) + a2.x) + a3.x, ((a0.y + a1.y) + a2.y) + a3.y, ((a0.z + a1.z) + a2.z) + a3.z, ((a0.w + a1.w) + a2.w) + a3.w);
   v.x += a4.x; v.y += a4.y; v.z += a4.z; v.w += a4.w;
-  if (pe) { const float4 q = *reinterpret_cast<const float4*>(pe + ((size_t)b * N + A + m) * 128 + c); v.x += q.x; v.y += q.y; v.z += q.z; v.w += q.w; }
+  if (pe) {
+    const size_t row = sidx ? (size_t)sidx[b] * (ldA + ldMp) + ldA + m : (size_t)b * N + A + m;
+    const float4 q = *reinterpret_cast<const float4*>(pe + row * 128 + c); v.x += q.x; v.y += q.y; v.z += q.z; v.w += q.w;
+  }
   return v;
 }
 
@@ -37,6 +46,7 @@
   const float* pooled; const int8_t* ptype; const uint8_t* on_route; const int8_t* tl; const uint8_t* has_sl;
   const float *speed_emb, *p_type_emb, *route_emb, *tl_emb, *unk_emb;
   int bs, A, Mp, N, nblk_a; float* X; const float* pe;
+  const int* sidx; int ldA, ldMp;
 };
 
 }
diff --git a/rift_amd/replay.py b/rift_amd/replay.py
--- a/rift_amd/replay.py
+++ b/rift_amd/replay.py
@@ -1,4 +1,5 @@
 import ctypes as C
+import os
 from typing import Dict, List, Optional, Sequence
 
 import numpy as np
@@ -154,6 +155,10 @@
         self._out = {}
         self.t: Dict[str, torch.Tensor] = {}
         self._host_version = None
+        self._const: Optional[Dict[str, torch.Tensor]] = None
+        self._const_key = None
+        self._const_geom = None
+        self._upload_gen = 0
         if scenes is None:
             return
         feats = [s["feature"] for s in scenes]
@@ -195,6 +200,49 @@
         ar.group_advantage = self.t["group_advantage"].data_ptr()
         ar.group_valid_mask = self.t["group_valid_mask"].data_ptr()
         self.arena = ar
+        self._caps = (capA, capMp, capR, capS)
+        self._upload_gen += 1
+        self._const_key = None
+        self._attach_constants()
+
+    _CONST_TENSORS = ("token_pe", "speed_emb", "ref_pe", "mom_map", "mom_ref")
+
+    @staticmethod
+    def constants_enabled() -> bool:
+        return os.environ.get("RIFT_SCENE_CONST", "1") != "0"
+
+    def _attach_constants(self):
+        fit = self._const is not None and self._const_geom == (self.n,) + self._caps
+        for name in self._CONST_TENSORS:
+            setattr(self.arena.constants, name, self._const[name].data_ptr() if fit else None)
+        return fit
+
+    def nbytes_constants(self) -> int:
+        return sum(t.numel() * t.element_size() for t in self._const.values()) if self._const else 0
+
+    def _ensure_constants(self, engine: "_ffi.Engine") -> bool:
+        capA, capMp, capR, capS = self._caps
+        if not self.constants_enabled() or capS != 0 or engine._params is None:
+            if self._const_key is not None or self.arena.constants.token_pe:
+                self._const_key = None
+                for name in self._CONST_TENSORS:
+                    setattr(self.arena.constants, name, None)
+            return False
+        key = (engine.serial, engine.model_generation(), self._upload_gen)
+        if key == self._const_key:
+            return True
+        geom = (self.n,) + self._caps
+        if self._const is None or self._const_geom != geom:
+            dev, n = self.device, self.n
+            self._const = {
+                "token_pe": torch.empty(n, capA + capMp, 128, device=dev), "speed_emb": torch.empty(n, capMp, 128, device=dev),
+                "ref_pe": torch.empty(n, capR, 128, device=dev),
+                "mom_map": torch.empty(n, 66, dtype=torch.float64, device=dev), "mom_ref": torch.empty(n, 28, dtype=torch.float64, device=dev)}
+            self._const_geom = geom
+        self._attach_constants()
+        engine._check(engine.lib.rift_replay_constants(engine.ctx, C.byref(self.arena), _ffi._stream()), "rift_replay_constants")
+        self._const_key = key
+        return True
 
     @classmethod
     def from_host(cls, host: HostReplay, device, n: Optional[int] = None) -> "DeviceReplay":
@@ -258,6 +306,11 @@
             setattr(fb, name, b[name].data_ptr() if name in b else None)
         fb.current_state = b["current_state"].data_ptr()
         fb.cs_ld = self.cs_ld
+        if self.constants_enabled() and self.S == 0:
+            b["const_scene_idx"] = torch.zeros(bs, dtype=torch.int32, device=dev)
+            b["const_ref_pe"] = torch.zeros(bs, R, 128, device=dev)
+            b["const_mom_map"] = torch.zeros(bs, 66, dtype=torch.float64, device=dev)
+            b["const_mom_ref"] = torch.zeros(bs, 28, dtype=torch.float64, device=dev)
         self._out[key] = (fb, b)
         return self._out[key]
 
@@ -274,8 +327,16 @@
                 fb, b = self._buffers(bs, R_out, slot)
         else:
             fb, b = self._buffers(bs, R_out, slot)
-        rc = engine.lib.rift_collate(
-            engine.ctx, C.byref(self.arena), C.c_void_p(scene_idx.data_ptr()), bs, R_out, C.byref(fb),
+        kc = None
+        if self._ensure_constants(engine) and "const_scene_idx" in b:
+            kc = _ffi.RiftSceneConstants()
+            kc.token_pe, kc.speed_emb = self._const["token_pe"].data_ptr(), self._const["speed_emb"].data_ptr()
+            kc.scene_idx, kc.ref_pe = b["const_scene_idx"].data_ptr(), b["const_ref_pe"].data_ptr()
+            kc.mom_map, kc.mom_ref = b["const_mom_map"].data_ptr(), b["const_mom_ref"].data_ptr()
+            kc.ldA, kc.ldMp = self._caps[0], self._caps[1]
+        fb.scene_constants = kc
+        rc = engine.lib.rift_collate_const(
+            engine.ctx, C.byref(self.arena), C.c_void_p(scene_idx.data_ptr()), bs, R_out, C.byref(fb), C.byref(kc) if kc is not None else None,
             _ffi._ptr(b["old_group_logits"]), _ffi._ptr(b["ref_group_logits"]), _ffi._ptr(b["group_advantage"]),
             _ffi._ptr(b["group_valid_mask"]), C.c_void_p(stream.cuda_stream) if stream is not None else _ffi._stream())
         if stream is not None:
```

Result: no change. 468,500 scenes/s (-0.1%).
